# hyperplane-lab/RGBManip

Measured on AMD Instinct MI355X. Metric: adapose_poses_per_sec_batch256, higher is better.
Workload: dtype bf16

## Files before the change

### include/rgbm.h

```cpp
#ifndef RGBM_H_
#define RGBM_H_
#include <stddef.h>
#include <stdint.h>

#ifdef __cplusplus
extern "C" {
#endif

#define RGBM_VERSION 100
#define RGBM_F32 0
#define RGBM_BF16 1
#define RGBM_F16 2
#define RGBM_BF16X3 3

int rgbm_version(void);
const char* rgbm_last_error(void);

typedef struct rgbm_weight_desc {
  const char* name;
  const float* data;
  int ndim;
  const int64_t* shape;
} rgbm_weight_desc;

// ... 67 lines not shown
int rgbm_depth_fusion(const float* depth, const float* conf, const uint8_t* mask, const double* Kcrop, const double* E, int n, int V, int S,
                      double px_max, double rel_max, float conf_min, int n_min, float* fused, uint8_t* keep, uint8_t* nviews, uint16_t* agree,
                      void* stream);
int rgbm_cloud_pack_views(const float* fused, const uint8_t* keep, const double* Kcrop, const double* E, int n, int V, int S, int cap,
                          float* cloud, int32_t* index, int32_t* count, void* stream);
int rgbm_cloud_gather_views(const float* maps, const int32_t* index, int n, int V, int S2, int C, int cap, float* out, void* stream);

int rgbm_adapose_postprocess(int B, int P, int img_size, const float* nocs1, const float* depth1, const float* r1,
                             const int32_t* choose1, const double* Kcrop, const double* E1, double* bbox_world, double* ts,
                             int32_t* valid, void* stream);
int rgbm_adapose_postprocess_scratch_bytes(int B, size_t* bytes);
int rgbm_adapose_postprocess_ws(int B, int P, int img_size, const float* nocs1, const float* depth1, const float* r1,
                                const int32_t* choose1, const double* Kcrop, const double* E1, double* bbox_world, double* ts,
                                int32_t* valid, void* scratch, size_t scratch_bytes, void* stream);

int rgbm_adapose_postprocess_regressed(int B, int P, const float* nocs1, const float* r1, const float* t1, const float* s1,
                                       const double* E1, double* bbox_world, double* ts, int32_t* valid, void* stream);

int rgbm_adapose_postprocess_ransac(int B, int P, int img_size, uint32_t seed, const float* nocs1, const float* depth1,
                                    const int32_t* choose1, const double* Kcrop, const double* E1, double* bbox_world, double* srt,
                                    int32_t* valid, void* stream);
int rgbm_adapose_postprocess_pnp(int B, int P, uint32_t seed, const float* nocs1, const float* pts2d1, const float* nocs2,
                                 const float* pts2d2, const double* K, const double* E1, const double* E2, double* bbox_out,
                                 double* srt_out, int32_t* info_out, int32_t* valid_out, void* stream);

int rgbm_prepare_inputs(const float* rgb_dev, const uint8_t* mask_dev, const double* K_dev, int N, int H, int W, int S, int P,
                        uint32_t seed, float* img_out, int32_t* choose_out, float* pts2d_out, double* Kcrop_out,
                        int32_t* window_out, int32_t* valid_out, uint8_t* scratch, void* stream);

int rgbm_prepare_inputs_indexed(const float* rgb_dev, const uint8_t* mask_dev, const double* K_dev, const int32_t* frame_map_dev,
                                int N, int H, int W, int S, int P, uint32_t seed, float* img_out, int32_t* choose_out,
                                float* pts2d_out, double* Kcrop_out, int32_t* window_out, int32_t* valid_out, uint8_t* scratch,
                                void* stream);
int rgbm_prepare_inputs_ex(const float* rgb_dev, const uint8_t* mask_dev, const double* K_dev, const int32_t* frame_map_dev,
                           int frame0, int N, int H, int W, int S, int P, uint32_t seed, float* img_out, int32_t* choose_out,
                           float* pts2d_out, double* Kcrop_out, int32_t* window_out, int32_t* valid_out, uint8_t* scratch,
                           void* stream);
int rgbm_prepare_inputs_u8(const uint8_t* rgb_dev, const uint8_t* mask_dev, const double* K_dev, const int32_t* frame_map_dev,
                           int frame0, int N, int H, int W, int S, int P, uint32_t seed, float* img_out, int32_t* choose_out,
                           float* pts2d_out, double* Kcrop_out, int32_t* window_out, int32_t* valid_out, uint8_t* scratch,
                           void* stream);
int rgbm_prepare_inputs_opt(const void* rgb_dev, int pixel_type, int normalize, const uint8_t* mask_dev, const double* K_dev,
                            const int32_t* frame_map_dev, int frame0, int N, int H, int W, int S, int P, uint32_t seed, float* img_out,
                            int32_t* choose_out, float* pts2d_out, double* Kcrop_out, int32_t* window_out, int32_t* valid_out,
                            uint8_t* scratch, void* stream);
int rgbm_prepare_inputs_windows(const void* pix_dev, int pixel_type, int normalize, const uint8_t* mask_pix_dev, const int64_t* offset_dev,
                                const int32_t* window_dev, const int32_t* valid_in_dev, const double* K_dev, int frame0, int N, int H, int W,
                                int S, int P, uint32_t seed, float* img_out, int32_t* choose_out, float* pts2d_out, double* Kcrop_out,
                                int32_t* valid_out, uint8_t* scratch, void* stream);
int rgbm_quantize_frames(const float* src_dev, uint8_t* dst_dev, size_t n, void* stream);

int rgbm_projection(const double* Kcrop_dev, const double* E_dev, float* P_dev, int N, void* stream);
int rgbm_mask_extent(const uint8_t* mask_dev, int N, int H, int W, int32_t* ext_out, int32_t* count_out, void* stream);

int rgbm_lookat_quat(const double* dir_dev, int N, int batch_zero, double* quat_dev, void* stream);
int rgbm_control_action_to_pose(const float* action_dev, int lda, const double* pose_mid, const double* pose_min,
                                const double* pose_max, int N, double* pose_dev, void* stream);
typedef struct rgbm_control_reward_args {
  const float* action;
  const double* cam_pose;
  const double* target;
  const float* move_success;
  const double* bbox;
  const double* avail;
  const double* gt_bbox;
  const double* pred_bbox;
  const double* pose_cur;
  const double* pose_prev;
  const double* robot_pose;
  const double* success;
  double* reward;
  double* terms;
  double coef[14];
  double proper_pos[3];
  double precision2;
  int N, T, lda, pots, first;
  int pad_;
} rgbm_control_reward_args;
int rgbm_control_reward(const rgbm_control_reward_args* args, void* stream);
int rgbm_control_grasp_frame(const double* est_dev, int N, double* center_dev, double* direction_dev, void* stream);

typedef struct rgbm_synth_scene {
  const double* cam_pose;
  const double* robot_pose;
  const double* box;
  double fx, fy, cx, cy;
  int N, H, W, env0;
} rgbm_synth_scene;
int rgbm_synth_camera(const rgbm_synth_scene* scene, double* K_dev, double* E_dev, double* rays_dev, void* stream);
int rgbm_synth_render(const rgbm_synth_scene* scene, const double* rays_dev, float* color_dev, uint8_t* mask_dev, void* stream);
int rgbm_synth_render_u8(const rgbm_synth_scene* scene, const double* rays_dev, uint8_t* color_dev, uint8_t* mask_dev,
                         int32_t* extent_dev, int32_t* count_dev, void* stream);

int rgbm_gae(int T, int N, const float* rewards, const uint8_t* dones, const float* values, const float* last_values,
             float gamma, float lam, float* returns, float* adv, double* sums, void* stream);
int rgbm_adv_normalise(int64_t n_local, float* adv, const double* sums, double count_total, void* stream);

typedef struct rgbm_policy_layout {
  int dims[5];
  int log_std;
  int w[2][4];
  int b[2][4];
  int total;
} rgbm_policy_layout;
int rgbm_policy_forward(const float* params, const rgbm_policy_layout* L, int n, int mode, const float* obs, const float* noise,
                        float* actions, float* logp, float* value, float* mu, void* stream);
int rgbm_ppo_partial_floats(const rgbm_policy_layout* L, int n, size_t* count);
int rgbm_ppo_minibatch_fwd_bwd(const float* params, const rgbm_policy_layout* L, int n, const float* obs, const float* actions,
                               const float* old_logp, const float* adv, const float* returns, const float* old_values,
                               const float* old_mu, const float* old_log_std, float clip, float vcoef, float ecoef,
                               float* partial_scratch, float* grads_flat, void* stream);
int rgbm_ppo_clip_adam(float* params, const float* grads_flat, float* exp_avg, float* exp_avg_sq, void* opt_state,
                       const rgbm_policy_layout* L, float inv_world, float max_norm, float desired_kl, float lr_min,
                       float lr_max, int adaptive, void* stream);

#define RGBM_POLICY_MAX_HIDDEN 6
#define RGBM_POLICY_MAX_WIDTH 512
#define RGBM_POLICY_MAX_ACT 32
#define RGBM_ACT_ELU 0
#define RGBM_ACT_SELU 1
#define RGBM_ACT_RELU 2
#define RGBM_ACT_LRELU 3
#define RGBM_ACT_TANH 4
#define RGBM_ACT_SIGMOID 5
typedef struct rgbm_policy_desc {
  int obs_dim, state_dim, act_dim;
  int activation;
  int asymmetric;
  int n_hidden[2];
  int hidden[2][RGBM_POLICY_MAX_HIDDEN];
  int w[2][RGBM_POLICY_MAX_HIDDEN + 1];
  int b[2][RGBM_POLICY_MAX_HIDDEN + 1];
  int log_std;
  int total;
} rgbm_policy_desc;
int rgbm_policy_forward_ex(const float* params, const rgbm_policy_desc* D, int n, int mode, const float* obs, const float* states,
                           const float* noise, float* actions, float* logp, float* value, float* mu, void* stream);
int rgbm_ppo_scratch_floats_ex(const rgbm_policy_desc* D, int n, int clipped_value_loss, size_t* count);
int rgbm_ppo_minibatch_fwd_bwd_ex(const float* params, const rgbm_policy_desc* D, int n, const float* obs, const float* states,
                                  const float* actions, const float* old_logp, const float* adv, const float* returns,
                                  const float* old_values, const float* old_mu, const float* old_log_std, float clip, float vcoef,
                                  float ecoef, int clipped_value_loss, float* scratch, float* grads_flat, void* stream);
int rgbm_ppo_clip_adam_ex(float* params, const float* grads_flat, float* exp_avg, float* exp_avg_sq, void* opt_state, int total,
                          float inv_world, float max_norm, float desired_kl, float lr_min, float lr_max, int adaptive, void* stream);

int rgbm_conv_nd(int dtype, const void* in_dev, int N, int D, int H, int W, int Cin, int Cin_pad, const float* w_host,
                 int Cout, int Cout_pad, int KD, int KH, int KW, int stride_d, int stride_hw, int pad_d, int pad_hw,
                 int dil_hw, int transposed, const float* bias_host, const float* bn_scale_host, const float* bn_shift_host,
                 const void* res_dev, int res_mode, int act, float slope, void* out_dev, void* stream);
#define RGBM_CONV_PLAN_INTS 9
int rgbm_conv_plan(int dtype, int N, int D, int H, int W, int Cin, int Cin_pad, int Cout, int Cout_pad, int KD, int KH, int KW,
                   int stride_d, int stride_hw, int pad_d, int pad_hw, int dil_hw, int transposed, int has_bias, int res_mode, int act,
                   int cls, int n_cu, int32_t* plan);
int rgbm_bn_per_sample_scratch_bytes(int V, size_t* bytes);
int rgbm_bn_per_sample(int dtype, void* y_dev, const void* res_dev, const float* gamma_dev, const float* beta_dev, void* scratch_dev,
                       int V, int64_t nvox, int C, int relu, void* stream);
int rgbm_conv3d_tile(int layer, int dtype, const void* in_dev, int N, int D, int H, int W, const float* w_host,
                     const float* bn_scale_host, const float* bn_shift_host, const void* res_dev, void* out_dev, void* stream);
int rgbm_upsample_conv3x3(int dtype, const void* in_dev, int V, int h, int w, int Cin, const float* w_host, int Cout,
                          const float* bias_host, int act, float slope, void* z_scratch_dev, void* out_dev, void* stream);
int rgbm_upsample_conv3x3_final(int dtype, const void* in_dev, int V, int h, int w, const float* w3_host, const float* b3_host,
                                float slope, const float* wf_host, const float* bf_host, void* out_dev, int out_f32, void* stream);
int rgbm_stem(int dtype, const float* img1_dev, const float* img2_dev, const float* w_host, void* out_dev, int B, int S, void* stream);
int rgbm_maxpool3x3s2(int dtype, const void* in_dev, void* out_dev, int V, int H, int W, int C, void* stream);
int rgbm_resize_bilinear_ac(int dtype, const void* in_dev, void* out_dev, int V, int Hs, int Ws, int C, int Ho, int Wo,
                            void* stream);
int rgbm_adaptive_avgpool(int dtype, const void* in_dev, void* out_dev, int V, int H, int W, int C, int S, void* stream);
int rgbm_build_volume(int dtype, const void* feat_dev, const float* P_views_dev, const float* depths_dev, float* homog_scratch,
                      void* vol_dev, int V, int B, int D, int H, int W, void* stream);
int rgbm_conv0_sweep(const void* feat_dev, const float* P_views_dev, const float* depths_dev, float* homog_scratch,
                     const float* w_host, const float* bn_scale_host, const float* bn_shift_host, void* out_dev,
                     int V, int B, int D, int H, int W, void* stream);
int rgbm_conv0_sweep_dt(int dtype, const void* feat_dev, const float* P_views_dev, const float* depths_dev, float* homog_scratch,
                        const float* w_host, const float* bn_scale_host, const float* bn_shift_host, void* out_dev,
                        int V, int B, int D, int H, int W, void* stream);
int rgbm_conv0_sweep_f16feat(const void* feat_f16_dev, const float* P_views_dev, const float* depths_dev, float* homog_scratch,
                             const float* w_host, const float* bn_scale_host, const float* bn_shift_host, void* out_bf16_dev,
                             int V, int B, int D, int H, int W, void* stream);
int rgbm_adapose_forward_ex(rgbm_adapose_t* h, int B, const float* img1, const float* img2, const int32_t* choose1,
                            const int32_t* choose2, const float* P1, const float* P2, const float* depths, void* workspace,
                            size_t workspace_bytes, const rgbm_adapose_out* out, int stop_after, void* stream);
int rgbm_adapose_forward_graph(rgbm_adapose_t* h, int B, const float* img1, const float* img2, const int32_t* choose1,
                               const int32_t* choose2, const float* P1, const float* P2, const float* depths, void* workspace,
                               size_t workspace_bytes, const rgbm_adapose_out* out, void* stream, int32_t* n_nodes, int32_t* captured);
int rgbm_adapose_graph_clear(rgbm_adapose_t* h);
int rgbm_adapose_feature_bytes(rgbm_adapose_t* h, size_t* bytes);
int rgbm_adapose_features_workspace_bytes(rgbm_adapose_t* h, int V, size_t* bytes);
int rgbm_adapose_features(rgbm_adapose_t* h, int V, const float* img, const int32_t* slots_dev, void* pool, int pool_records,
                          void* workspace, size_t workspace_bytes, void* stream);
int rgbm_adapose_forward_cached(rgbm_adapose_t* h, int B, const void* pool, int pool_records, const int32_t* slot1_dev,
                                const int32_t* slot2_dev, const int32_t* choose1, const int32_t* choose2, const float* P1, const float* P2,
                                const float* depths, void* workspace, size_t workspace_bytes, const rgbm_adapose_out* out, void* stream);
int rgbm_adapose_fetch(rgbm_adapose_t* h, int B, void* workspace, const char* name, float* out_dev, size_t capacity,
                       size_t* n_elems, void* stream);
int rgbm_crop_fingerprint(const float* img, int V, int n_words, uint64_t* keys_out, void* stream);

#define RGBM_PROF_ROWS 42
int rgbm_debug_flags(int flags);
int rgbm_set_tuning(const char* key, long long value);
int rgbm_microbench_mfma_scratch_floats(int* n);
int rgbm_microbench_mfma(float* scratch, int iters, int random_operands, double* flops, void* stream);
int rgbm_microbench_copy(const void* src, void* dst, size_t bytes, void* stream);
int rgbm_prof_rows(void);
int rgbm_prof_start(void);
int rgbm_prof_stop(double* stats);
int rgbm_prof_select(int row);

#ifdef __cplusplus
}
#endif
#endif
```

### rgbmanip_amd/_lib.py

```python
from __future__ import annotations

import ctypes as C
import os

_HERE = os.path.dirname(os.path.abspath(__file__))
LIB_PATH = os.environ.get("RGBM_HIP_LIB") or os.path.join(_HERE, "librgbm_hip.so")

F32, BF16, F16, BF16X3 = 0, 1, 2, 3
ACT_NONE, ACT_RELU, ACT_PRELU, ACT_TANH = 0, 1, 2, 3
RES_NONE, RES_PRE_ACT, RES_POST_ACT = 0, 1, 2


PROF_ROWS = 42
PROF_KERNELS = [
    ("conv_igemm_glds_kernel<float, 16, 256>", "fp32"), ("conv_igemm_glds_kernel<float, 32, 256>", "fp32"),
    ("conv_igemm_glds_kernel<float, 64, 256>", "fp32"), ("conv_igemm_glds_kernel<float, 128, 128>", "fp32"),
    ("conv_igemm_glds_kernel<unsigned short, 16, 256>", "bf16"), ("conv_igemm_glds_kernel<unsigned short, 32, 256>", "bf16"),
    ("conv_igemm_glds_kernel<unsigned short, 64, 256>", "bf16"), ("conv_igemm_glds_kernel<unsigned short, 128, 128>", "bf16"),
    ("conv3d_tile_kernel<float, ...> (conv1..conv11)", "fp32"), ("conv3d_tile_kernel<unsigned short, ...> (conv1..conv11)", "bf16"),
    ("conv3d_tile_kernel<float, 32, 16, 4, 8, 8, 1, false, true> (conv0 + fused plane sweep)", "fp32"),
    ("conv3d_tile_kernel<unsigned short, 32, 16, 4, 8, 8, 1, false, true> (conv0 + fused plane sweep)", "bf16"),
    ("conv_igemm_ws_kernel<float, ...>", "fp32"), ("conv_igemm_ws_kernel<unsigned short, false, false> (128 channels x 256 pixels)", "bf16"),
    ("conv0_sweep_persistent_kernel<unsigned short> (conv0 + fused plane sweep of bf16 nets; sweep_f16 = 0 / fp16 nets: conv0_sweep_kernel)", "bf16"), ("conv_igemm_ws64_kernel", "bf16"),
    ("conv3d_tile_kernel<unsigned short, 32, 16, 6, 8, 8, 1, false, false> (conv0 on a materialised volume)", "bf16"),
    ("conv3d_tile_kernel<unsigned short, 8, 16, 2, 8, 8, 2, false, false> (conv1)", "bf16"),
    ("conv3d_tile_kernel<unsigned short, 16, 16, 4, 8, 8, 1, false, false> (conv2)", "bf16"),
    ("conv3d_tile_kernel<unsigned short, 16, 32, 2, 8, 8, 2, false, false> (conv3)", "bf16"),
    ("conv3d_tile_kernel<unsigned short, 32, 32, 2, 8, 8, 1, false, false> (conv4)", "bf16"),
    ("conv3d_tile_kernel<unsigned short, 32, 64, 1, 8, 8, 2, false, false> (conv5)", "bf16"),
    ("conv3d_tile_kernel<unsigned short, 64, 64, 1, 8, 8, 1, false, false> (conv6)", "bf16"),
    ("conv3d_tile_kernel<unsigned short, 64, 32, 1, 8, 8, 1, true, false> (conv7)", "bf16"),
    ("conv3d_tile_kernel<unsigned short, 32, 16, 2, 8, 8, 1, true, false> (conv9)", "bf16"),
    ("conv3d_tile_kernel<unsigned short, 16, 16, 4, 8, 8, 1, true, false> (conv11)", "bf16"),
] + [("conv_igemm_glds_kernel<bx3_t, ...> (all channel tiles)", "bf16x3"), ("conv3d_tile_kernel<bx3_t, ...> (conv1..conv11)", "bf16x3"),
     ("conv0 + fused plane sweep <bx3_t>", "bf16x3"), ("conv_igemm_ws_kernel<rgbm::bx3_t, false, false> (128 channels x 256 pixels)", "bf16x3"),
     ("pose_mlp1_kernel (pose_mlp1.0 + pose_mlp1.2 of a bf16 net in one launch)", "bf16"),
     ("conv_igemm_m32_kernel<unsigned short, 256, 256> (256 channels x 256 pixels, 32x32x16 MFMAs; gemm_kernel = 0: conv_igemm_ws_kernel<unsigned short, true, false>, 256 x 128)", "bf16"),
     ("pose_mlp2_kernel (pose_mlp2.0 + pose_mlp2.2 + the sum over points of a bf16 net in one launch)", "bf16"),
     ("conv_igemm_m32_kernel<rgbm::bx3_t, 256, 256> (256 channels x 256 pixels, 32x32x16 MFMAs; gemm_kernel = 0: conv_igemm_ws_kernel<rgbm::bx3_t, true, false>, 256 x 128)", "bf16x3"),
     ("conv_igemm_ws_kernel<rgbm::bx3_t, false, false, true> (64 channels x 256 pixels, four multiply waves)", "bf16x3"),
     ("conv_igemm_ws_kernel<unsigned short, false, false, true> (64 channels x 256 pixels, four multiply waves)", "bf16"),
     ("conv_igemm_ws_kernel<float, false, false, true> (64 channels x 256 pixels, four multiply waves)", "fp32"),
     ("upconv_combine_kernel<16-bit> (PSPUpsample tap combination)", "bf16"), ("upconv_combine_kernel<4-byte> (PSPUpsample tap combination)", "bf16x3"),
     ("upconv_final_kernel (up_3 + final in one kernel; either storage width)", "bf16"),
     ("conv_igemm_m32_kernel<unsigned short, 128, 64 / 128 / 256> (128-pixel tiles: tail and small-batch launches of the 256-channel GEMM)", "bf16"),
     ("conv_igemm_m32_kernel<rgbm::bx3_t, 128, 64 / 128 / 256> (128-pixel tiles: tail and small-batch launches of the 256-channel GEMM)", "bf16x3")]
assert len(PROF_KERNELS) == PROF_ROWS


class RgbmError(RuntimeError):
    pass


class WeightDesc(C.Structure):
    _fields_ = [("name", C.c_char_p), ("data", C.c_void_p), ("ndim", C.c_int), ("shape", C.POINTER(C.c_int64))]


class PolicyLayout(C.Structure):
    _fields_ = [("dims", C.c_int * 5), ("log_std", C.c_int), ("w", (C.c_int * 4) * 2), ("b", (C.c_int * 4) * 2), ("total", C.c_int)]


POLICY_MAX_HIDDEN, POLICY_MAX_WIDTH, POLICY_MAX_ACT = 6, 512, 32
POLICY_ACTIVATIONS = {"elu": 0, "selu": 1, "relu": 2, "crelu": 2, "lrelu": 3, "tanh": 4, "sigmoid": 5}


class PolicyDesc(C.Structure):
    _fields_ = [("obs_dim", C.c_int), ("state_dim", C.c_int), ("act_dim", C.c_int), ("activation", C.c_int), ("asymmetric", C.c_int),
                ("n_hidden", C.c_int * 2), ("hidden", (C.c_int * POLICY_MAX_HIDDEN) * 2),
                ("w", (C.c_int * (POLICY_MAX_HIDDEN + 1)) * 2), ("b", (C.c_int * (POLICY_MAX_HIDDEN + 1)) * 2),
                ("log_std", C.c_int), ("total", C.c_int)]


class AdaposeOut(C.Structure):
    _fields_ = [(n, C.c_void_p) for n in ("view1_nocs", "view2_nocs", "view1_depth", "view2_depth", "view1_r", "view2_r",
                                           "view1_t", "view2_t", "view1_s", "view2_s")]


class ControlRewardArgs(C.Structure):
    _fields_ = [(n, C.c_void_p) for n in ("action", "cam_pose", "target", "move_success", "bbox", "avail", "gt_bbox", "pred_bbox",
                                           "pose_cur", "pose_prev", "robot_pose", "success", "reward", "terms")] + [
        ("coef", C.c_double * 14), ("proper_pos", C.c_double * 3), ("precision2", C.c_double),
        ("N", C.c_int), ("T", C.c_int), ("lda", C.c_int), ("pots", C.c_int), ("first", C.c_int), ("pad_", C.c_int)]


class SynthScene(C.Structure):
    _fields_ = [("cam_pose", C.c_void_p), ("robot_pose", C.c_void_p), ("box", C.c_void_p),
                ("fx", C.c_double), ("fy", C.c_double), ("cx", C.c_double), ("cy", C.c_double),
                ("N", C.c_int), ("H", C.c_int), ("W", C.c_int), ("env0", C.c_int)]


_vp, _i, _f, _d, _sz, _i64 = C.c_void_p, C.c_int, C.c_float, C.c_double, C.c_size_t, C.c_int64

SIGNATURES = {
    "rgbm_version": (_i, []),
    "rgbm_last_error": (C.c_char_p, []),
    "rgbm_adapose_create": (_i, [C.POINTER(_vp), _i, C.POINTER(WeightDesc), _i, _i, _i]),
    "rgbm_adapose_create_baseline": (_i, [C.POINTER(_vp), _i, C.POINTER(WeightDesc), _i, _i, _i]),
    "rgbm_view_fusion": (_i, [_vp, _vp, _vp, _i, _i, _vp, _vp, _vp, _sz, _vp]),
    "rgbm_view_fusion_scratch_bytes": (_i, [_i, _i, C.POINTER(_sz)]),
    "rgbm_depth_head": (_i, [_vp, _vp, _i64, _vp, _vp]),
    "rgbm_adapose_destroy": (_i, [_vp]),
    "rgbm_adapose_set_chunk": (_i, [_vp, _i]),
    "rgbm_adapose_set_option": (_i, [_vp, C.c_char_p, _i]),
    "rgbm_adapose_workspace_bytes": (_i, [_vp, _i, C.POINTER(_sz)]),
    "rgbm_adapose_set_dropout": (_i, [_vp, _f, C.c_uint64]),
    "rgbm_adapose_dropout_masks": (_i, [_vp, _i, _vp]),
    "rgbm_adapose_set_dropout_masks": (_i, [_vp, _i, _vp]),
    "rgbm_adapose_forward": (_i, [_vp, _i, _vp, _vp, _vp, _vp, _vp, _vp, _vp, _vp, _sz, C.POINTER(AdaposeOut), _vp]),
    "rgbm_adapose_forward_ex": (_i, [_vp, _i, _vp, _vp, _vp, _vp, _vp, _vp, _vp, _vp, _sz, C.POINTER(AdaposeOut), _i, _vp]),
    "rgbm_adapose_forward_graph": (_i, [_vp, _i, _vp, _vp, _vp, _vp, _vp, _vp, _vp, _vp, _sz, C.POINTER(AdaposeOut), _vp, C.POINTER(C.c_int32),
                                        C.POINTER(C.c_int32)]),
    "rgbm_adapose_samples_workspace_bytes": (_i, [_vp, _i, _i, C.POINTER(_sz)]),
    "rgbm_adapose_forward_samples": (_i, [_vp, _i, _i, _vp, _vp, _vp, _vp, _vp, _vp, _vp, _vp, _sz, C.POINTER(AdaposeOut), _vp]),
    "rgbm_sample_box_stats": (_i, [_vp, _vp, _i, _i, _vp, _vp, _vp, _vp, _vp, _vp, _vp, _vp, _vp]),
    "rgbm_sample_point_stats": (_i, [_vp, _i, _i, _i64, _vp, _vp, _vp]),
    "rgbm_box_agreement": (_i, [_vp, _vp, _vp, _vp, _i] + [_vp] * 14),
    "rgbm_box_iou_matrix": (_i, [_vp, _vp, _vp, _vp, _i, _i, _i, _vp, _vp]),
    "rgbm_adapose_dense_workspace_bytes": (_i, [_vp, _i, C.POINTER(_sz)]),
    "rgbm_adapose_forward_dense": (_i, [_vp, _i, _vp, _vp, _vp, _vp, _vp, _vp, _vp, _vp, _sz, C.POINTER(AdaposeOut), _vp, _vp, _vp]),
    "rgbm_adapose_forward_maps": (_i, [_vp, _i, _vp, _vp, _vp, _vp, _vp, _vp, _vp, _vp, _sz, C.POINTER(AdaposeOut), _vp, _vp, _vp, _vp]),
    "rgbm_nocs_map": (_i, [_vp, _vp, _i, _i, _vp, _vp]),
    "rgbm_cloud_gather": (_i, [_vp, _vp, _vp, _i, _i, _i, _i, _vp, _vp]),
    "rgbm_cloud_similarity_scratch_bytes": (_i, [_i, _i, C.POINTER(_sz)]),
    "rgbm_cloud_similarity": (_i, [_vp, _vp, _vp, _i, _i, C.c_uint32, _vp, _vp, _vp, _vp, _vp, _sz, _vp]),
    "rgbm_depth_to_points": (_i, [_vp, _vp, _vp, _i, _i, _vp, _vp]),
    "rgbm_depth_consistency": (_i, [_vp, _vp, _vp, _vp, _vp, _vp, _vp, _vp, _i, _i, _d, _d, _f, _vp, _vp, _vp, _vp, _vp]),
    "rgbm_cloud_pack": (_i, [_vp, _vp, _vp, _vp, _vp, _vp, _vp, _vp, _i, _i, _i, _vp, _vp, _vp, _vp]),
    "rgbm_depth_fusion": (_i, [_vp, _vp, _vp, _vp, _vp, _i, _i, _i, _d, _d, _f, _i, _vp, _vp, _vp, _vp, _vp]),
    "rgbm_cloud_pack_views": (_i, [_vp, _vp, _vp, _vp, _i, _i, _i, _i, _vp, _vp, _vp, _vp]),
    "rgbm_cloud_gather_views": (_i, [_vp, _vp, _i, _i, _i, _i, _i, _vp, _vp]),
    "rgbm_adapose_graph_clear": (_i, [_vp]),
    "rgbm_adapose_feature_bytes": (_i, [_vp, C.POINTER(_sz)]),
    "rgbm_adapose_features_workspace_bytes": (_i, [_vp, _i, C.POINTER(_sz)]),
    "rgbm_adapose_features": (_i, [_vp, _i, _vp, _vp, _vp, _i, _vp, _sz, _vp]),
    "rgbm_adapose_forward_cached": (_i, [_vp, _i, _vp, _i, _vp, _vp, _vp, _vp, _vp, _vp, _vp, _vp, _sz, C.POINTER(AdaposeOut), _vp]),
    "rgbm_crop_fingerprint": (_i, [_vp, _i, _i, _vp, _vp]),
    "rgbm_adapose_fetch": (_i, [_vp, _i, _vp, C.c_char_p, _vp, _sz, C.POINTER(_sz), _vp]),
    "rgbm_adapose_postprocess": (_i, [_i, _i, _i, _vp, _vp, _vp, _vp, _vp, _vp, _vp, _vp, _vp, _vp]),
    "rgbm_adapose_postprocess_scratch_bytes": (_i, [_i, C.POINTER(_sz)]),
    "rgbm_adapose_postprocess_ws": (_i, [_i, _i, _i, _vp, _vp, _vp, _vp, _vp, _vp, _vp, _vp, _vp, _vp, _sz, _vp]),
    "rgbm_adapose_postprocess_regressed": (_i, [_i, _i, _vp, _vp, _vp, _vp, _vp, _vp, _vp, _vp, _vp]),
    "rgbm_adapose_postprocess_ransac": (_i, [_i, _i, _i, C.c_uint32, _vp, _vp, _vp, _vp, _vp, _vp, _vp, _vp, _vp]),
    "rgbm_adapose_postprocess_pnp": (_i, [_i, _i, C.c_uint32, _vp, _vp, _vp, _vp, _vp, _vp, _vp, _vp, _vp, _vp, _vp, _vp]),
    "rgbm_gae": (_i, [_i, _i, _vp, _vp, _vp, _vp, _f, _f, _vp, _vp, _vp, _vp]),
    "rgbm_adv_normalise": (_i, [_i64, _vp, _vp, _d, _vp]),
    "rgbm_policy_forward": (_i, [_vp, _vp, _i, _i, _vp, _vp, _vp, _vp, _vp, _vp, _vp]),
    "rgbm_ppo_partial_floats": (_i, [_vp, _i, C.POINTER(_sz)]),
    "rgbm_ppo_minibatch_fwd_bwd": (_i, [_vp, _vp, _i, _vp, _vp, _vp, _vp, _vp, _vp, _vp, _vp, _f, _f, _f, _vp, _vp, _vp]),
    "rgbm_ppo_clip_adam": (_i, [_vp, _vp, _vp, _vp, _vp, _vp, _f, _f, _f, _f, _f, _i, _vp]),
    "rgbm_policy_forward_ex": (_i, [_vp, _vp, _i, _i, _vp, _vp, _vp, _vp, _vp, _vp, _vp, _vp]),
    "rgbm_ppo_scratch_floats_ex": (_i, [_vp, _i, _i, C.POINTER(_sz)]),
    "rgbm_ppo_minibatch_fwd_bwd_ex": (_i, [_vp, _vp, _i, _vp, _vp, _vp, _vp, _vp, _vp, _vp, _vp, _vp, _f, _f, _f, _i, _vp, _vp, _vp]),
    "rgbm_ppo_clip_adam_ex": (_i, [_vp, _vp, _vp, _vp, _vp, _i, _f, _f, _f, _f, _f, _i, _vp]),
    "rgbm_conv_nd": (_i, [_i, _vp, _i, _i, _i, _i, _i, _i, _vp, _i, _i, _i, _i, _i, _i, _i, _i, _i, _i, _i, _vp, _vp, _vp,
                          _vp, _i, _i, _f, _vp, _vp]),
    "rgbm_conv_plan": (_i, [_i] * 23 + [C.POINTER(C.c_int32)]),
    "rgbm_bn_per_sample_scratch_bytes": (_i, [_i, C.POINTER(_sz)]),
    "rgbm_bn_per_sample": (_i, [_i, _vp, _vp, _vp, _vp, _vp, _i, _i64, _i, _i, _vp]),
    "rgbm_conv3d_tile": (_i, [_i, _i, _vp, _i, _i, _i, _i, _vp, _vp, _vp, _vp, _vp, _vp]),
    "rgbm_upsample_conv3x3": (_i, [_i, _vp, _i, _i, _i, _i, _vp, _i, _vp, _i, _f, _vp, _vp, _vp]),
    "rgbm_upsample_conv3x3_final": (_i, [_i, _vp, _i, _i, _i, _vp, _vp, _f, _vp, _vp, _vp, _i, _vp]),
    "rgbm_stem": (_i, [_i, _vp, _vp, _vp, _vp, _i, _i, _vp]),
    "rgbm_maxpool3x3s2": (_i, [_i, _vp, _vp, _i, _i, _i, _i, _vp]),
    "rgbm_resize_bilinear_ac": (_i, [_i, _vp, _vp, _i, _i, _i, _i, _i, _i, _vp]),
    "rgbm_adaptive_avgpool": (_i, [_i, _vp, _vp, _i, _i, _i, _i, _i, _vp]),
    "rgbm_build_volume": (_i, [_i, _vp, _vp, _vp, _vp, _vp, _i, _i, _i, _i, _i, _vp]),
    "rgbm_conv0_sweep": (_i, [_vp, _vp, _vp, _vp, _vp, _vp, _vp, _vp, _i, _i, _i, _i, _i, _vp]),
    "rgbm_conv0_sweep_dt": (_i, [_i, _vp, _vp, _vp, _vp, _vp, _vp, _vp, _vp, _i, _i, _i, _i, _i, _vp]),
    "rgbm_conv0_sweep_f16feat": (_i, [_vp, _vp, _vp, _vp, _vp, _vp, _vp, _vp, _i, _i, _i, _i, _i, _vp]),
    "rgbm_prepare_inputs": (_i, [_vp, _vp, _vp, _i, _i, _i, _i, _i, C.c_uint32, _vp, _vp, _vp, _vp, _vp, _vp, _vp, _vp]),
    "rgbm_prepare_inputs_indexed": (_i, [_vp, _vp, _vp, _vp, _i, _i, _i, _i, _i, C.c_uint32, _vp, _vp, _vp, _vp, _vp, _vp, _vp, _vp]),
    "rgbm_prepare_inputs_ex": (_i, [_vp, _vp, _vp, _vp, _i, _i, _i, _i, _i, _i, C.c_uint32, _vp, _vp, _vp, _vp, _vp, _vp, _vp, _vp]),
    "rgbm_prepare_inputs_u8": (_i, [_vp, _vp, _vp, _vp, _i, _i, _i, _i, _i, _i, C.c_uint32, _vp, _vp, _vp, _vp, _vp, _vp, _vp, _vp]),
    "rgbm_prepare_inputs_opt": (_i, [_vp, _i, _i, _vp, _vp, _vp, _i, _i, _i, _i, _i, _i, C.c_uint32, _vp, _vp, _vp, _vp, _vp, _vp, _vp, _vp]),
    "rgbm_prepare_inputs_windows": (_i, [_vp, _i, _i, _vp, _vp, _vp, _vp, _vp, _i, _i, _i, _i, _i, _i, C.c_uint32, _vp, _vp, _vp, _vp, _vp, _vp, _vp]),
    "rgbm_quantize_frames": (_i, [_vp, _vp, C.c_size_t, _vp]),
    "rgbm_projection": (_i, [_vp, _vp, _vp, _i, _vp]),
    "rgbm_mask_extent": (_i, [_vp, _i, _i, _i, _vp, _vp, _vp]),
    "rgbm_lookat_quat": (_i, [_vp, _i, _i, _vp, _vp]),
    "rgbm_control_action_to_pose": (_i, [_vp, _i, C.POINTER(C.c_double), C.POINTER(C.c_double), C.POINTER(C.c_double), _i, _vp, _vp]),
    "rgbm_control_reward": (_i, [C.POINTER(ControlRewardArgs), _vp]),
    "rgbm_control_grasp_frame": (_i, [_vp, _i, _vp, _vp, _vp]),
    "rgbm_synth_camera": (_i, [C.POINTER(SynthScene), _vp, _vp, _vp, _vp]),
    "rgbm_synth_render": (_i, [C.POINTER(SynthScene), _vp, _vp, _vp, _vp]),
    "rgbm_synth_render_u8": (_i, [C.POINTER(SynthScene), _vp, _vp, _vp, _vp, _vp, _vp]),
    "rgbm_debug_flags": (_i, [_i]),
    "rgbm_set_tuning": (_i, [C.c_char_p, _i64]),
    "rgbm_prof_rows": (_i, []),
    "rgbm_microbench_mfma_scratch_floats": (_i, [C.POINTER(C.c_int)]),
    "rgbm_microbench_mfma": (_i, [_vp, _i, _i, C.POINTER(C.c_double), _vp]),
    "rgbm_microbench_copy": (_i, [_vp, _vp, C.c_size_t, _vp]),
    "rgbm_prof_start": (_i, []),
    "rgbm_prof_select": (_i, [_i]),
    "rgbm_prof_stop": (_i, [C.POINTER(C.c_double)]),
}

_lib = None


def load():
    global _lib
    if _lib is not None:
        return _lib
    if not os.path.exists(LIB_PATH):
        raise RgbmError(f"{LIB_PATH} not found: build it with rgbmanip_amd/csrc/build.sh "
                        f"(or `python -c 'import __graft_entry__ as g; g.build()'`). There is no CPU fallback.")
    lib = C.CDLL(LIB_PATH)
    for name, (res, args) in SIGNATURES.items():
        fn = getattr(lib, name)
        fn.restype = res
        fn.argtypes = args
    if lib.rgbm_prof_rows() != PROF_ROWS:
        raise RgbmError(f"{LIB_PATH}: rgbm_prof_rows() = {lib.rgbm_prof_rows()}, this binding expects {PROF_ROWS} (stale build?)")
    _lib = lib
    return lib


def check(rc: int, what: str = ""):
    if rc != 0:
        msg = load().rgbm_last_error()
        raise RgbmError(f"{what} failed (code {rc}): {msg.decode() if msg else ''}")


def stream_ptr(stream=None):
    import torch
    s = stream if stream is not None else torch.cuda.current_stream()
    return C.c_void_p(s.cuda_stream)


def ptr(t):
    return C.c_void_p(t.data_ptr()) if t is not None else C.c_void_p(0)
```

### rgbmanip_amd/csrc/capi.cpp

```cpp
#include "../../include/rgbm.h"

#include <string.h>

#include <algorithm>
#include <initializer_list>
#include <memory>
#include <string>
#include <utility>
#include <vector>

#include "adapose.h"
#include "box_overlap.h"
#include "control.h"
#include "cost3d.h"
#include "conv_plan.h"
#include "prof.h"
#include "sample_stats.h"
#include "view_fusion.h"

using namespace rgbm;

struct ForwardGraph {
  int B = 0;
  hipStream_t stream = nullptr;
// ... 439 lines not shown
    if (call.dropout == AdaPose::Dropout::Draw) warm.dropout = AdaPose::Dropout::DrawNoAdvance;
    if (int rw = forward(warm)) return rw;
    ForwardGraph g;
    g.B = B; g.stream = s; memcpy(g.in, in, sizeof(in)); g.ws = workspace; g.ws_bytes = workspace_bytes; g.out = *out;
    g.opt_version = h->opt_version; g.tuning_version = g_tuning_version;
    RGBM_CHECK_HIP(hipStreamBeginCapture(s, hipStreamCaptureModeThreadLocal));
    const int rc = forward(call);
    const hipError_t ee = hipStreamEndCapture(s, &g.graph);
    if (rc) { if (g.graph) (void)hipGraphDestroy(g.graph); return rc; }
    if (ee != hipSuccess || !g.graph) { set_error(std::string("hipStreamEndCapture: ") + hipGetErrorString(ee)); return -2; }
    if (hipGraphGetNodes(g.graph, nullptr, &g.nodes) != hipSuccess) g.nodes = 0;
    const hipError_t ei = hipGraphInstantiate(&g.exec, g.graph, nullptr, nullptr, 0);
    if (ei != hipSuccess) { (void)hipGraphDestroy(g.graph); set_error(std::string("hipGraphInstantiate: ") + hipGetErrorString(ei)); return -2; }
    if (h->graphs.size() >= kMaxGraphs) {
      size_t lru = 0;
      for (size_t i = 1; i < h->graphs.size(); ++i) if (h->graphs[i].last_use < h->graphs[lru].last_use) lru = i;
      drop_graph(h->graphs[lru]);
      h->graphs.erase(h->graphs.begin() + lru);
    }
    h->graphs.push_back(g);
    hit = &h->graphs.back();
    if (captured) *captured = 1;
  }
  hit->last_use = ++h->tick;
  if (n_nodes) *n_nodes = (int32_t)hit->nodes;
  RGBM_CHECK_HIP(hipGraphLaunch(hit->exec, s));
  return finish_call(h, B, call, 0);
}

int rgbm_adapose_fetch(rgbm_adapose_t* h, int B, void* workspace, const char* name, float* out_dev, size_t capacity,
                       size_t* n_elems, void* stream) {
  RGBM_REQUIRE(h && workspace && name && out_dev && n_elems, "fetch arguments");
  const AdaPose& n = h->net;
  Arena A(workspace, 0);
  AdaPose::Buffers bf;
  n.plan(B, A, bf);
  const size_t V = 2 * (size_t)B, S = n.img, P = n.n_pts, D = n.n_depth;
  const size_t Vc = n.chunk_views((int)V);
  const std::string nm = name;
  const void* src = nullptr; size_t cnt = 0; int dt = n.dtype;
  if (nm == "imgpad") { src = bf.imgpad; cnt = V * S * S * n.img_cpad; }
  else if (nm == "conv1") { src = bf.c1; cnt = V * (S / 2) * (S / 2) * 64; }
  else if (nm == "layer4") { src = bf.lb[n.layer4_index()]; cnt = V * (S / 8) * (S / 8) * 512; }
  else if (nm == "cat") { src = bf.cat; cnt = V * (S / 8) * (S / 8) * 1024; }
  else if (nm == "u1") { src = bf.u1; cnt = V * (S / 4) * (S / 4) * 256; }
  else if (nm == "u2") { src = bf.u2; cnt = V * (S / 2) * (S / 2) * 64; }
  else if (nm == "u3") { src = bf.u3; cnt = V * S * S * 64; }
  else if (nm == "feat") { src = bf.feat; cnt = V * S * S * 32; if (n.feat_f32_only()) { src = bf.featf; dt = F32; } else if (n.feat_f16()) dt = F16; }
  else if (nm == "vol") { src = bf.vol; cnt = Vc * D * S * S * 32; }
  else if (nm == "homog") { src = bf.homog; cnt = V * 12; dt = F32; }
  else if (nm == "prob") { src = bf.prob; cnt = V * P * D; dt = F32; }
  else if (nm == "pf96") { src = bf.PF96; cnt = V * P * 96; dt = n.pose_dtype() == BF16X3 ? BF16X3 : F32; }
  else if (nm == "pf2") { src = bf.pf2; cnt = V * 256; dt = F32; }
  else if (nm == "r6") { src = bf.r6; cnt = V * 6; dt = F32; }
  else if (nm == "fused1" && bf.fused) { src = bf.fused; cnt = (size_t)B * P * 32; dt = F32; }
  else if (nm == "fused2" && bf.fused) { src = bf.fused + (size_t)B * P * 32; cnt = (size_t)B * P * 32; dt = F32; }
  static const struct { const char* name; int row; } taps3d[] = {{"c0", 0}, {"c2", 2}, {"c4", 4}, {"c6", 6}, {"u7", 7}, {"u9", 8}, {"u11", 9}};
  int row3d = -1;
  for (const auto& t : taps3d)
    if (nm == t.name) { row3d = t.row; src = bf.c3[row3d]; cnt = cost3d_out_elems(row3d, (int)Vc, (int)D, (int)S); }
  if (is_baseline(h))
    RGBM_REQUIRE(nm == "feat" || nm == "fused1" || nm == "fused2" || nm == "pf96" || nm == "pf2" || nm == "r6" || nm == "layer4" || nm == "cat" ||
                 nm == "u1" || nm == "u2", "tap '" + nm + "' does not exist in the baseline network");
  RGBM_REQUIRE(src != nullptr, "unknown intermediate name: " + nm);
  const bool tap3d = row3d >= 0 && row3d < 9;
  RGBM_REQUIRE(!(tap3d && n.sparse_active()), "tap '" + nm + "' needs a dense cost regularisation: set option sparse_dec = 0 before the forward "
               "(the default computes it only inside the chosen pixels' dependency cones)");
  *n_elems = cnt;
  RGBM_REQUIRE(cnt <= capacity, "fetch capacity too small");
  return launch_to_f32(dt, src, out_dev, (long long)cnt, (hipStream_t)stream);
}

int rgbm_adapose_postprocess(int B, int P, int img_size, const float* nocs1, const float* depth1, const float* r1,
                             const int32_t* choose1, const double* Kcrop, const double* E1, double* bbox_world, double* ts,
                             int32_t* valid, void* stream) {
  RGBM_REQUIRE(B > 0 && nocs1 && depth1 && r1 && choose1 && Kcrop && E1 && bbox_world && ts && valid, "postprocess arguments");
  return launch_postprocess(nocs1, depth1, r1, choose1, Kcrop, E1, bbox_world, ts, valid, B, P, img_size, (hipStream_t)stream);
}

int rgbm_adapose_postprocess_scratch_bytes(int B, size_t* bytes) {
  RGBM_REQUIRE(B > 0 && bytes, "postprocess_scratch_bytes arguments");
  *bytes = postprocess_slices(B) > 1 ? postprocess_scratch_bytes(B) : 0;
  return 0;
}

int rgbm_adapose_postprocess_ws(int B, int P, int img_size, const float* nocs1, const float* depth1, const float* r1,
                                const int32_t* choose1, const double* Kcrop, const double* E1, double* bbox_world, double* ts,
                                int32_t* valid, void* scratch, size_t scratch_bytes, void* stream) {
  RGBM_REQUIRE(B > 0 && nocs1 && depth1 && r1 && choose1 && Kcrop && E1 && bbox_world && ts && valid, "postprocess arguments");
  return launch_postprocess(nocs1, depth1, r1, choose1, Kcrop, E1, bbox_world, ts, valid, B, P, img_size, (hipStream_t)stream,
                            scratch, scratch_bytes);
}

int rgbm_adapose_postprocess_ransac(int B, int P, int img_size, uint32_t seed, const float* nocs1, const float* depth1,
                                    const int32_t* choose1, const double* Kcrop, const double* E1, double* bbox_world, double* srt,
                                    int32_t* valid, void* stream) {
  return launch_umeyama_ransac(nocs1, depth1, choose1, Kcrop, E1, bbox_world, srt, valid, B, P, img_size, seed, (hipStream_t)stream);
}

int rgbm_gae(int T, int N, const float* rewards, const uint8_t* dones, const float* values, const float* last_values,
             float gamma, float lam, float* returns, float* adv, double* sums, void* stream) {
  RGBM_REQUIRE(rewards && dones && values && last_values && returns && adv && sums, "gae arguments");
  return launch_gae(T, N, rewards, dones, values, last_values, gamma, lam, returns, adv, sums, (hipStream_t)stream);
}

int rgbm_adv_normalise(int64_t n_local, float* adv, const double* sums, double count_total, void* stream) {
  RGBM_REQUIRE(adv && sums && n_local > 0 && count_total > 1.0, "adv_normalise arguments");
  return launch_adv_normalise(n_local, adv, sums, count_total, (hipStream_t)stream);
}

static ConvGeom conv_nd_geom(int Cin, int Cout, int KD, int KH, int KW, int stride_d, int stride_hw, int pad_d, int pad_hw, int dil_hw,
                             int transposed, int act, float slope) {
  ConvGeom g;
  g.Cin = Cin; g.Cout = Cout; g.KD = KD; g.KH = KH; g.KW = KW;
  g.sd = stride_d; g.sh = g.sw = stride_hw; g.pd = pad_d; g.ph = g.pw = pad_hw;
  g.dild = 1; g.dilh = g.dilw = dil_hw; g.transposed = transposed != 0; g.act = act; g.slope = slope;
  return g;
}

int rgbm_conv_nd(int dtype, const void* in_dev, int N, int D, int H, int W, int Cin, int Cin_pad, const float* w_host,
                 int Cout, int Cout_pad, int KD, int KH, int KW, int stride_d, int stride_hw, int pad_d, int pad_hw,
                 int dil_hw, int transposed, const float* bias_host, const float* bn_scale_host, const float* bn_shift_host,
                 const void* res_dev, int res_mode, int act, float slope, void* out_dev, void* stream) {
  RGBM_REQUIRE(in_dev && w_host && out_dev, "conv arguments");
  const ConvGeom g = conv_nd_geom(Cin, Cout, KD, KH, KW, stride_d, stride_hw, pad_d, pad_hw, dil_hw, transposed, act, slope);
  ConvLayer L;
  if (int rc = L.init(dtype, g, w_host, bias_host, bn_scale_host, bn_shift_host, Cin_pad, Cout_pad)) return rc;
  return finish_one_shot(L.run(in_dev, out_dev, N, D, H, W, Cout_pad, res_dev, res_mode, nullptr, 0, (hipStream_t)stream), stream);
}

int rgbm_conv_plan(int dtype, int N, int D, int H, int W, int Cin, int Cin_pad, int Cout, int Cout_pad, int KD, int KH, int KW,
                   int stride_d, int stride_hw, int pad_d, int pad_hw, int dil_hw, int transposed, int has_bias, int res_mode, int act,
                   int cls, int n_cu, int32_t* plan) {
  RGBM_REQUIRE(plan && n_cu >= 0 && dtype >= F32 && dtype <= BF16X3 && N > 0 && D > 0 && H > 0 && W > 0, "conv_plan arguments");
  const ConvGeom g = conv_nd_geom(Cin, Cout, KD, KH, KW, stride_d, stride_hw, pad_d, pad_hw, dil_hw, transposed, act, 0.f);
  PackedConv pc;
  if (int rc = conv_pack_geom(g, dtype, Cin_pad, Cout_pad, cls, &pc)) return rc;
  ConvDesc d;
  conv_desc_geom(d, g, pc, Cin_pad, Cout_pad, N, D, H, W, Cout_pad, cls);
  alignas(16) static const float buffer[4] = {};
  d.in = d.wgt = buffer; d.out = const_cast<float*>(buffer);
  d.bias = has_bias ? buffer : nullptr;
  d.res = res_mode != RES_NONE ? buffer : nullptr;
  d.res_mode = res_mode;
  ConvTuning t;
  ConvPlan p;
  if (int rc = conv_tuning(n_cu, &t)) return rc;
  if (int rc = plan_conv(d, dtype, t, &p)) return rc;
  const int32_t v[RGBM_CONV_PLAN_INTS] = {p.kernel, p.bch, p.bpix, p.ksplit, (int32_t)p.main_rows, p.tail_bch, p.identity_residual, (int32_t)d.M, d.KT};
  memcpy(plan, v, sizeof(v));
  return 0;
}

int rgbm_upsample_conv3x3(int dtype, const void* in_dev, int V, int h, int w, int Cin, const float* w_host, int Cout,
                          const float* bias_host, int act, float slope, void* z_scratch_dev, void* out_dev, void* stream) {
  RGBM_REQUIRE(in_dev && w_host && z_scratch_dev && out_dev, "upsample_conv3x3 arguments");
  UpConvLayer L;
  if (int rc = L.init(dtype, Cin, Cout, w_host, bias_host, act, slope)) return rc;
  return finish_one_shot(L.run(in_dev, z_scratch_dev, out_dev, V, h, w, Cout, (hipStream_t)stream), stream);
}

int rgbm_upsample_conv3x3_final(int dtype, const void* in_dev, int V, int h, int w, const float* w3_host, const float* b3_host,
                                float slope, const float* wf_host, const float* bf_host, void* out_dev, int out_f32, void* stream) {
  RGBM_REQUIRE(in_dev && w3_host && b3_host && wf_host && bf_host && out_dev, "upsample_conv3x3_final arguments");
  UpConvFinal L;
  if (int rc = L.init(dtype, w3_host, b3_host, slope, wf_host, bf_host)) return rc;
  return finish_one_shot(L.run(in_dev, out_dev, out_f32, V, h, w, (hipStream_t)stream), stream);
}

int rgbm_stem(int dtype, const float* img1_dev, const float* img2_dev, const float* w_host, void* out_dev, int B, int S, void* stream) {
  RGBM_REQUIRE(img1_dev && img2_dev && w_host && out_dev && B > 0, "stem arguments");
  std::vector<float> pk;
  stem_pack(w_host, pk);
  DevBuf wd;
  if (int rc = upload_packed(pk, dtype, wd)) return rc;
  return finish_one_shot(launch_stem(dtype, img1_dev, img2_dev, wd.get(), out_dev, B, 2 * B, S, (hipStream_t)stream), stream);
}

int rgbm_bn_per_sample_scratch_bytes(int V, size_t* bytes) {
  RGBM_REQUIRE(V > 0 && bytes, "bn_per_sample_scratch_bytes arguments");
  *bytes = bn_scratch_bytes(V);
  return 0;
}
int rgbm_bn_per_sample(int dtype, void* y_dev, const void* res_dev, const float* gamma_dev, const float* beta_dev, void* scratch_dev,
                       int V, int64_t nvox, int C, int relu, void* stream) {
  RGBM_REQUIRE(y_dev && gamma_dev && beta_dev && scratch_dev, "bn_per_sample arguments");
  return launch_bn_per_sample(dtype, y_dev, res_dev, gamma_dev, beta_dev, scratch_dev, V, (long long)nvox, C, relu, (hipStream_t)stream);
}
int rgbm_maxpool3x3s2(int dtype, const void* in_dev, void* out_dev, int V, int H, int W, int C, void* stream) {
  return launch_maxpool3x3s2(dtype, in_dev, out_dev, V, H, W, C, (hipStream_t)stream);
}
int rgbm_resize_bilinear_ac(int dtype, const void* in_dev, void* out_dev, int V, int Hs, int Ws, int C, int Ho, int Wo,
                            void* stream) {
  return launch_resize_bilinear_ac(dtype, in_dev, out_dev, V, Hs, Ws, C, Ho, Wo, C, 0, (hipStream_t)stream);
}
int rgbm_adaptive_avgpool(int dtype, const void* in_dev, void* out_dev, int V, int H, int W, int C, int S, void* stream) {
  return launch_adaptive_avgpool(dtype, in_dev, out_dev, V, H, W, C, S, (hipStream_t)stream);
}
int rgbm_build_volume(int dtype, const void* feat_dev, const float* P_views_dev, const float* depths_dev, float* homog_scratch,
                      void* vol_dev, int V, int B, int D, int H, int W, void* stream) {
  if (int rc = launch_homography(P_views_dev, homog_scratch, V, B, (hipStream_t)stream)) return rc;
  return launch_build_volume(dtype, feat_dev, homog_scratch, depths_dev, vol_dev, 0, V, V, B, D, H, W, (hipStream_t)stream);
}

}

#include "prof.h"
extern "C" {
int rgbm_prof_rows(void) { return rgbm::kProfVariants; }
int rgbm_microbench_mfma_scratch_floats(int* n) {
  RGBM_REQUIRE(n, "microbench_mfma_scratch_floats arguments");
  return rgbm::microbench_mfma_scratch_floats(n);
}
int rgbm_microbench_mfma(float* scratch, int iters, int random_operands, double* flops, void* stream) {
  return rgbm::launch_microbench_mfma(scratch, iters, random_operands, flops, (hipStream_t)stream);
}
int rgbm_microbench_copy(const void* src, void* dst, size_t bytes, void* stream) {
  return rgbm::launch_microbench_copy(src, dst, bytes, (hipStream_t)stream);
}
int rgbm_prof_start(void) { return rgbm::prof_start(); }
int rgbm_prof_select(int row) {
  RGBM_REQUIRE(row >= -1 && row < rgbm::kProfVariants, "prof_select: row out of range");
  return rgbm::prof_select(row);
}
int rgbm_prof_stop(double* stats) {
  RGBM_REQUIRE(stats != nullptr, "prof_stop arguments");
  return rgbm::prof_stop(stats, rgbm::kProfVariants);
}
}

extern "C" int rgbm_conv3d_tile(int layer, int dtype, const void* in_dev, int N, int D, int H, int W, const float* w_host,
                                const float* bn_scale_host, const float* bn_shift_host, const void* res_dev, void* out_dev,
                                void* stream) {
  RGBM_REQUIRE(layer >= 0 && layer < kCost3dLayers && in_dev && w_host && bn_scale_host && bn_shift_host && out_dev, "conv3d_tile arguments");
  const Cost3dLayer& L = kCost3d[layer];
  const int coutp = cost3d_coutp(layer);
  std::vector<float> packed;
  conv3d_tile_pack(w_host, bn_scale_host, L.cin, L.cout, coutp, L.transposed, dtype, packed);
  DevBuf wdev, bdev;
  if (upload_packed(packed, dtype, wdev)) return -2;
  std::vector<float> bpad(coutp, 0.f);
  for (int o = 0; o < L.cout; ++o) bpad[o] = bn_shift_host[o];
  if (upload_f32(bpad.data(), bpad.size(), bdev)) return -2;
  Conv3dTileDesc d;
  memset(&d, 0, sizeof(d));
  d.in = in_dev; d.wgt = wdev.get(); d.out = out_dev; d.bias = bdev.get<float>(); d.res = res_dev;
  d.N = N; d.Di = D; d.Hi = H; d.Wi = W;
  if (L.transposed) { d.Do = 2 * D; d.Ho = 2 * H; d.Wo = 2 * W; d.Dq = D; d.Hq = H; d.Wq = W; }
  else {
    const int s = L.stride;
    d.Do = (D + 2 - 3) / s + 1; d.Ho = (H + 2 - 3) / s + 1; d.Wo = (W + 2 - 3) / s + 1;
    d.Dq = d.Do; d.Hq = d.Ho; d.Wq = d.Wo;
  }
  d.Cout = L.cout; d.relu = 1; d.prof_variant = -1;
  return finish_one_shot(launch_conv3d_tile(layer, dtype, d, (hipStream_t)stream), stream);
}

static int conv0_sweep_entry(int dtype, int feat_f16, const void* feat_dev, const float* P_views_dev, const float* depths_dev,
                             float* homog_scratch, const float* w_host, const float* bn_scale_host, const float* bn_shift_host,
                             void* out_dev, int V, int B, int D, int H, int W, void* stream) {
  RGBM_REQUIRE(feat_dev && P_views_dev && depths_dev && homog_scratch && w_host && bn_scale_host && bn_shift_host && out_dev,
               "conv0_sweep arguments");
  RGBM_REQUIRE(dtype == BF16 || dtype == F16 || dtype == BF16X3, "conv0_sweep: 16-bit storage types or bf16x3 (fp32 features in, split-pair c0 out)");
  if (int rc = launch_homography(P_views_dev, homog_scratch, V, B, (hipStream_t)stream)) return rc;
  std::vector<float> packed;
  conv0_sweep_pack(w_host, bn_scale_host, packed);
  DevBuf wdev, bdev;
  if (dtype == BF16X3) { if (conv0_sweep_x3_upload(packed, wdev.out())) return -2; }
  else if (upload_packed(packed, feat_f16 ? (int)F16 : dtype, wdev)) return -2;
  std::vector<float> bpad(cost3d_coutp(0), 0.f);
  for (int o = 0; o < kCost3d[0].cout; ++o) bpad[o] = bn_shift_host[o];
  if (upload_f32(bpad.data(), bpad.size(), bdev)) return -2;
  Conv3dTileDesc d;
  memset(&d, 0, sizeof(d));
  d.wgt = wdev.get(); d.out = out_dev; d.bias = bdev.get<float>();
  d.N = V; d.Di = D; d.Hi = H; d.Wi = W; d.Do = D; d.Ho = H; d.Wo = W; d.Dq = D; d.Hq = H; d.Wq = W;
  d.Cout = kCost3d[0].cout; d.relu = 1; d.prof_variant = -1;
  d.feat = feat_dev; d.homog = homog_scratch; d.depths = depths_dev; d.v0 = 0; d.V = V; d.B = B;
  d.feat_f16 = feat_f16;
  return finish_one_shot(dtype == BF16X3 ? launch_conv0_sweep_x3(d, (hipStream_t)stream) : launch_conv0_sweep(d, dtype, (hipStream_t)stream), stream);
}

extern "C" int rgbm_conv0_sweep_dt(int dtype, const void* feat_dev, const float* P_views_dev, const float* depths_dev,
                                   float* homog_scratch, const float* w_host, const float* bn_scale_host, const float* bn_shift_host,
                                   void* out_dev, int V, int B, int D, int H, int W, void* stream) {
  return conv0_sweep_entry(dtype, 0, feat_dev, P_views_dev, depths_dev, homog_scratch, w_host, bn_scale_host, bn_shift_host, out_dev, V, B, D,
                           H, W, stream);
}

extern "C" int rgbm_conv0_sweep_f16feat(const void* feat_f16_dev, const float* P_views_dev, const float* depths_dev,
                                        float* homog_scratch, const float* w_host, const float* bn_scale_host,
                                        const float* bn_shift_host, void* out_bf16_dev, int V, int B, int D, int H, int W, void* stream) {
  return conv0_sweep_entry(BF16, 1, feat_f16_dev, P_views_dev, depths_dev, homog_scratch, w_host, bn_scale_host, bn_shift_host, out_bf16_dev,
                           V, B, D, H, W, stream);
}

extern "C" int rgbm_conv0_sweep(const void* feat_dev, const float* P_views_dev, const float* depths_dev, float* homog_scratch,
                                const float* w_host, const float* bn_scale_host, const float* bn_shift_host, void* out_dev,
                                int V, int B, int D, int H, int W, void* stream) {
  return rgbm_conv0_sweep_dt(BF16, feat_dev, P_views_dev, depths_dev, homog_scratch, w_host, bn_scale_host, bn_shift_host, out_dev,
                             V, B, D, H, W, stream);
}

extern "C" int rgbm_prepare_inputs(const float* rgb_dev, const uint8_t* mask_dev, const double* K_dev, int N, int H, int W, int S,
                                   int P, uint32_t seed, float* img_out, int32_t* choose_out, float* pts2d_out, double* Kcrop_out,
                                   int32_t* window_out, int32_t* valid_out, uint8_t* scratch, void* stream) {
// ... 185 lines not shown
```

### rgbmanip_amd/csrc/common.h

```cpp
#pragma once
#include <hip/hip_runtime.h>
#include <stdint.h>
#include <stdio.h>
#include <string>

namespace rgbm {

enum DType { F32 = 0, BF16 = 1, F16 = 2, BF16X3 = 3 };
enum Act { ACT_NONE = 0, ACT_RELU = 1, ACT_PRELU = 2, ACT_TANH = 3 };
enum ResMode { RES_NONE = 0, RES_PRE_ACT = 1, RES_POST_ACT = 2 };

typedef __attribute__((ext_vector_type(8))) __bf16 bf16x8;
typedef _Float16 f16_t;
typedef __attribute__((ext_vector_type(8))) _Float16 f16x8;
typedef __attribute__((ext_vector_type(4))) _Float16 f16x4;
typedef __attribute__((ext_vector_type(8))) float f32x8;
typedef __attribute__((ext_vector_type(4))) float f32x4;

void set_error(const std::string& s);
int fail(const char* what, const char* file, int line);

#define RGBM_CHECK_HIP(expr)                                                             \
  do {                                                                                   \
    hipError_t _e = (expr);                                                              \
// ... 62 lines not shown
  o.w = pack2_bf16(c - __uint_as_float(o.y << 16), d - __uint_as_float(o.y & 0xffff0000u));
  return o;
}
__device__ __forceinline__ void bx3_join4(const uint4& c, float* v) {
  v[0] = __uint_as_float(c.x << 16) + __uint_as_float(c.z << 16);
  v[1] = __uint_as_float(c.x & 0xffff0000u) + __uint_as_float(c.z & 0xffff0000u);
  v[2] = __uint_as_float(c.y << 16) + __uint_as_float(c.w << 16);
  v[3] = __uint_as_float(c.y & 0xffff0000u) + __uint_as_float(c.w & 0xffff0000u);
}
template <> struct Elem<bx3_t> {
  static constexpr int kPerChunk = 4;
  __device__ static __forceinline__ float ld(const bx3_t* p) {
    const unsigned long long a = (unsigned long long)p;
    const unsigned short* ch = reinterpret_cast<const unsigned short*>(a & ~15ull);
    const int e = (int)((a >> 2) & 3);
    return bf16_to_f32(ch[e]) + bf16_to_f32(ch[4 + e]);
  }
  __device__ static __forceinline__ void st(bx3_t* p, float v) {
    const unsigned long long a = (unsigned long long)p;
    unsigned short* ch = reinterpret_cast<unsigned short*>(a & ~15ull);
    const int e = (int)((a >> 2) & 3);
    const unsigned short h = f32_to_bf16(v);
    ch[e] = h;
    ch[4 + e] = f32_to_bf16(v - bf16_to_f32(h));
  }
};

__device__ __forceinline__ float sat_f16(float v) { return v != v ? v : fminf(fmaxf(v, -65504.f), 65504.f); }

__device__ __forceinline__ void load4(const float* p, float v[4]) {
  float4 t = *reinterpret_cast<const float4*>(p);
  v[0] = t.x; v[1] = t.y; v[2] = t.z; v[3] = t.w;
}
__device__ __forceinline__ void load4(const unsigned short* p, float v[4]) {
  uint2 t = *reinterpret_cast<const uint2*>(p);
  v[0] = __uint_as_float(t.x << 16); v[1] = __uint_as_float(t.x & 0xffff0000u);
  v[2] = __uint_as_float(t.y << 16); v[3] = __uint_as_float(t.y & 0xffff0000u);
}
__device__ __forceinline__ void load4(const f16_t* p, float v[4]) {
  const f16x4 t = *reinterpret_cast<const f16x4*>(p);
  v[0] = (float)t[0]; v[1] = (float)t[1]; v[2] = (float)t[2]; v[3] = (float)t[3];
}
__device__ __forceinline__ void store4(f16_t* p, const float v[4]) {
  f16x4 t;
  t[0] = (f16_t)sat_f16(v[0]); t[1] = (f16_t)sat_f16(v[1]); t[2] = (f16_t)sat_f16(v[2]); t[3] = (f16_t)sat_f16(v[3]);
  *reinterpret_cast<f16x4*>(p) = t;
}
__device__ __forceinline__ void store4(float* p, const float v[4]) {
  *reinterpret_cast<float4*>(p) = make_float4(v[0], v[1], v[2], v[3]);
}
__device__ __forceinline__ void store4(unsigned short* p, const float v[4]) {
  uint2 t;
  t.x = pack2_bf16(v[0], v[1]);
  t.y = pack2_bf16(v[2], v[3]);
  *reinterpret_cast<uint2*>(p) = t;
}
__device__ __forceinline__ void load4(const bx3_t* p, float v[4]) { bx3_join4(*reinterpret_cast<const uint4*>(p), v); }
__device__ __forceinline__ void store4(bx3_t* p, const float v[4]) { *reinterpret_cast<uint4*>(p) = bx3_split4(v[0], v[1], v[2], v[3]); }
__device__ __forceinline__ void unpack_chunk(const uint4& c, float* v, bx3_t ) { bx3_join4(c, v); }
__device__ __forceinline__ uint4 pack_chunk(const float* v, bx3_t ) { return bx3_split4(v[0], v[1], v[2], v[3]); }
__device__ __forceinline__ void unpack_chunk(const uint4& c, float* v, float ) {
  v[0] = __uint_as_float(c.x); v[1] = __uint_as_float(c.y); v[2] = __uint_as_float(c.z); v[3] = __uint_as_float(c.w);
}
__device__ __forceinline__ void unpack_chunk(const uint4& c, float* v, unsigned short ) {
  v[0] = __uint_as_float(c.x << 16); v[1] = __uint_as_float(c.x & 0xffff0000u);
  v[2] = __uint_as_float(c.y << 16); v[3] = __uint_as_float(c.y & 0xffff0000u);
  v[4] = __uint_as_float(c.z << 16); v[5] = __uint_as_float(c.z & 0xffff0000u);
  v[6] = __uint_as_float(c.w << 16); v[7] = __uint_as_float(c.w & 0xffff0000u);
}
__device__ __forceinline__ void unpack_chunk(const uint4& c, float* v, f16_t ) {
  const f16x8 h = __builtin_bit_cast(f16x8, c);
#pragma unroll
  for (int e = 0; e < 8; ++e) v[e] = (float)h[e];
}
__device__ __forceinline__ uint4 pack_chunk(const float* v, f16_t ) {
  f16x8 h;
#pragma unroll
  for (int e = 0; e < 8; ++e) h[e] = (f16_t)sat_f16(v[e]);
  return __builtin_bit_cast(uint4, h);
}
__device__ __forceinline__ uint4 pack_chunk(const float* v, float ) {
  return make_uint4(__float_as_uint(v[0]), __float_as_uint(v[1]), __float_as_uint(v[2]), __float_as_uint(v[3]));
}
__device__ __forceinline__ uint4 pack_chunk(const float* v, unsigned short ) {
  uint4 c;
  c.x = pack2_bf16(v[0], v[1]);
  c.y = pack2_bf16(v[2], v[3]);
  c.z = pack2_bf16(v[4], v[5]);
  c.w = pack2_bf16(v[6], v[7]);
  return c;
}

typedef __attribute__((ext_vector_type(4))) short rgbm_s16x4;
__device__ __forceinline__ f32x4 mma_bx3_k16(const uint4& a, const uint4& b, f32x4 c) {
  const rgbm_s16x4 ah = __builtin_bit_cast(rgbm_s16x4, make_uint2(a.x, a.y)), al = __builtin_bit_cast(rgbm_s16x4, make_uint2(a.z, a.w));
  const rgbm_s16x4 bh = __builtin_bit_cast(rgbm_s16x4, make_uint2(b.x, b.y)), bl = __builtin_bit_cast(rgbm_s16x4, make_uint2(b.z, b.w));
  c = __builtin_amdgcn_mfma_f32_16x16x16bf16_1k(al, bh, c, 0, 0, 0);
  c = __builtin_amdgcn_mfma_f32_16x16x16bf16_1k(ah, bl, c, 0, 0, 0);
  c = __builtin_amdgcn_mfma_f32_16x16x16bf16_1k(ah, bh, c, 0, 0, 0);
  return c;
}
__device__ __forceinline__ void bx3_pair(const uint4& c0, const uint4& c1, uint4& hi, uint4& lo) {
  hi = make_uint4(c0.x, c0.y, c1.x, c1.y);
  lo = make_uint4(c0.z, c0.w, c1.z, c1.w);
}

__host__ __device__ inline unsigned mix32(unsigned seed, unsigned frame, unsigned idx) {
  unsigned h = seed ^ (frame * 0x9E3779B9u) ^ (idx * 0x85EBCA6Bu);
  h ^= h >> 16; h *= 0x85EBCA6Bu; h ^= h >> 13; h *= 0xC2B2AE35u; h ^= h >> 16;
  return h;
}

template <int THREADS, class Op> __device__ inline double block_reduce(double v, double* red, Op op) {
  const int t = threadIdx.x;
  red[t] = v;
  __syncthreads();
  for (int s = THREADS / 2; s > 0; s >>= 1) {
    if (t < s) red[t] = op(red[t], red[t + s]);
    __syncthreads();
  }
  const double r = red[0];
  __syncthreads();
  return r;
}
template <int THREADS> __device__ inline double block_sum(double v, double* red) {
  return block_reduce<THREADS>(v, red, [](double a, double b) { return a + b; });
}
template <int THREADS> __device__ inline double block_max(double v, double* red) {
  return block_reduce<THREADS>(v, red, [](double a, double b) { return fmax(a, b); });
}

struct ConvDesc {
  const void* in; const void* wgt; void* out; const float* bias; const void* res;
  int N, Di, Hi, Wi, Cin, lcin;
  int Dq, Hq, Wq;
  int sd, sh, sw, pd, ph, pw;
  int KD, KH, KW, dild, dilh, dilw;
  int ntaps, KT, Kpad;
  int Cout, ldo;
  int Do, Ho, Wo;
  int osd, osh, osw, opd, oph, opw;
  int act; float slope; int res_mode; int bias_stride;
  long long M;
  int n_pix_tiles, n_ch_tiles;
  int n_tiles; unsigned fd_m[3]; int fd_s[3];
  int korder;
  int buf_ok;
  const void* ident;
  long long m0;
  const void* w2; const float* bias2; void* out2; int ldo2, cout2, kpad2, act2; float slope2;
  double algo_flops, algo_bytes;
  int out_f32;
  int ksplit; float* kscratch; unsigned* kcount;
};

int launch_conv(const ConvDesc& d, int dtype, hipStream_t s);
bool conv_ws64_eligible(const ConvDesc& d, int dtype);
int conv_ch_tile(int Cout);
int conv_bk(int dtype);

}
```

### rgbmanip_amd/csrc/conv_igemm_glds.hip

```cpp
#include <map>
#include <mutex>
#include <type_traits>
#include <vector>
#include "common.h"
#include "conv_plan.h"
#include "kernels.h"
#include "prof.h"

#ifndef WS_BUF
#define WS_BUF 1
#endif

namespace rgbm {

int g_gemm_kernel = 2;
__device__ uint4 g_zero_page[4];

typedef __attribute__((address_space(3))) void* lds_ptr_t;
typedef const __attribute__((address_space(1))) void* gbl_ptr_t;

__device__ __forceinline__ void glds16(const void* gsrc, unsigned lds_off) {
  asm volatile("s_mov_b32 m0, %1\n\ts_nop 0\n\tglobal_load_lds_dwordx4 %0, off" :: "v"(gsrc), "s"(lds_off) : "memory");
}
__device__ __forceinline__ void blds16(unsigned voff, const __amdgpu_buffer_rsrc_t& rsrc, unsigned soff, unsigned lds_off) {
  asm volatile("s_mov_b32 m0, %3\n\ts_nop 0\n\tbuffer_load_dwordx4 %0, %1, %2 offen lds" :: "v"(voff), "s"(rsrc), "s"(soff), "s"(lds_off) : "memory");
}
__device__ __forceinline__ unsigned lds_addr(const void* p) {
  return (unsigned)(unsigned long long)(__attribute__((address_space(3))) const void*)p;
}

#define RGBM_BARRIER() do { asm volatile("" ::: "memory"); __builtin_amdgcn_s_barrier(); asm volatile("" ::: "memory"); } while (0)

template <typename T> struct MmaG;
template <> struct MmaG<unsigned short> {
  __device__ static __forceinline__ void run(const uint4& a, const uint4& b, f32x4& c) {
    c = __builtin_amdgcn_mfma_f32_16x16x32_bf16(__builtin_bit_cast(bf16x8, a), __builtin_bit_cast(bf16x8, b), c, 0, 0, 0);
  }
  __device__ static __forceinline__ f32x4 run2(const uint4& a, const uint4& b, const f32x4& c) {
    return __builtin_amdgcn_mfma_f32_16x16x32_bf16(__builtin_bit_cast(bf16x8, a), __builtin_bit_cast(bf16x8, b), c, 0, 0, 0);
  }
};
template <> struct MmaG<f16_t> {
  __device__ static __forceinline__ void run(const uint4& a, const uint4& b, f32x4& c) {
    c = __builtin_amdgcn_mfma_f32_16x16x32_f16(__builtin_bit_cast(f16x8, a), __builtin_bit_cast(f16x8, b), c, 0, 0, 0);
  }
  __device__ static __forceinline__ f32x4 run2(const uint4& a, const uint4& b, const f32x4& c) {
    return __builtin_amdgcn_mfma_f32_16x16x32_f16(__builtin_bit_cast(f16x8, a), __builtin_bit_cast(f16x8, b), c, 0, 0, 0);
  }
};
template <> struct MmaG<float> {
  __device__ static __forceinline__ void run(const uint4& a, const uint4& b, f32x4& c) {
    c = __builtin_amdgcn_mfma_f32_16x16x4f32(__uint_as_float(a.x), __uint_as_float(b.x), c, 0, 0, 0);
    c = __builtin_amdgcn_mfma_f32_16x16x4f32(__uint_as_float(a.y), __uint_as_float(b.y), c, 0, 0, 0);
    c = __builtin_amdgcn_mfma_f32_16x16x4f32(__uint_as_float(a.z), __uint_as_float(b.z), c, 0, 0, 0);
    c = __builtin_amdgcn_mfma_f32_16x16x4f32(__uint_as_float(a.w), __uint_as_float(b.w), c, 0, 0, 0);
  }
};

template <> struct MmaG<bx3_t> {
  __device__ static __forceinline__ void run(const uint4& a, const uint4& b, f32x4& c) { c = mma_bx3_k16(a, b, c); }
};
template <typename T> constexpr int prof_row_generic(int bch) {
  return std::is_same<T, bx3_t>::value ? 26 : (sizeof(T) == 2 ? 4 : 0) + (bch == 16 ? 0 : bch == 32 ? 1 : bch == 64 ? 2 : 3);
}
template <typename T> constexpr int prof_row_ws() { return std::is_same<T, bx3_t>::value ? 29 : sizeof(T) == 2 ? 13 : 12; }

template <int FM, int FN>
__device__ __forceinline__ void mma_bx3_tile(const uint4 (&a0)[FM], const uint4 (&a1)[FM], const uint4 (&b0)[FN], const uint4 (&b1)[FN],
                                             f32x4 (&acc)[FM][FN]) {
  uint4 ah[FM], al[FM], bh[FN], bl[FN];
#pragma unroll
  for (int a = 0; a < FM; ++a) bx3_pair(a0[a], a1[a], ah[a], al[a]);
#pragma unroll
  for (int b = 0; b < FN; ++b) bx3_pair(b0[b], b1[b], bh[b], bl[b]);
#pragma unroll
  for (int a = 0; a < FM; ++a)
#pragma unroll
    for (int b = 0; b < FN; ++b) MmaG<unsigned short>::run(al[a], bh[b], acc[a][b]);
#pragma unroll
  for (int a = 0; a < FM; ++a)
#pragma unroll
    for (int b = 0; b < FN; ++b) MmaG<unsigned short>::run(ah[a], bl[b], acc[a][b]);
#pragma unroll
  for (int a = 0; a < FM; ++a)
#pragma unroll
    for (int b = 0; b < FN; ++b) MmaG<unsigned short>::run(ah[a], bh[b], acc[a][b]);
}

template <int OFF>
__device__ __forceinline__ void lds_rd8(uint2& dst, unsigned addr) {
  asm volatile("ds_read_b64 %0, %1 offset:%2" : "=v"(dst) : "v"(addr), "n"(OFF) : "memory");
}

template <int FM, int FN>
__device__ __forceinline__ void mma_bx3_ops(const uint4 (&ah)[FM], const uint4 (&al)[FM], const uint4 (&bh)[FN], const uint4 (&bl)[FN],
                                            f32x4 (&acc)[FM][FN]) {
#pragma unroll
  for (int a = 0; a < FM; ++a)
#pragma unroll
    for (int b = 0; b < FN; ++b) MmaG<unsigned short>::run(al[a], bh[b], acc[a][b]);
#pragma unroll
  for (int a = 0; a < FM; ++a)
#pragma unroll
    for (int b = 0; b < FN; ++b) MmaG<unsigned short>::run(ah[a], bl[b], acc[a][b]);
#pragma unroll
  for (int a = 0; a < FM; ++a)
#pragma unroll
    for (int b = 0; b < FN; ++b) MmaG<unsigned short>::run(ah[a], bh[b], acc[a][b]);
}

template <int N> struct IC { static constexpr int value = N; };

__device__ __forceinline__ float apply_act_g(float v, int act, float slope) {
  if (act == ACT_RELU) return v < 0.f ? 0.f : v;
  if (act == ACT_PRELU) return v < 0.f ? v * slope : v;
  if (act == ACT_TANH) return tanhf(v);
  return v;
}

template <typename T, int BCH, int BPIX, bool UNI>
__global__ __launch_bounds__(256, 2) void conv_igemm_glds_kernel(const ConvDesc d) {
  constexpr int E = 16 / sizeof(T);
  constexpr int BK = 8 * E;
  constexpr int XR = BPIX / 32;
  constexpr int WL = BCH >= 32 ? BCH / 32 : 1;
  constexpr int WCH = BCH < 64 ? BCH : 64;
  constexpr int FM = WCH / 16;
  constexpr int FN = 4;
  constexpr int STAGE = (BCH + BPIX) * 8;
  __shared__ uint4 lds[2 * STAGE];

  const int tid = threadIdx.x;
  const int lane = tid & 63;
  const int wave = __builtin_amdgcn_readfirstlane(tid >> 6);

  const int nblk = gridDim.x;
  const int bq = nblk >> 3, br = nblk & 7;
  const int xcd = blockIdx.x & 7, bidx = blockIdx.x >> 3;
  const int lid = (xcd < br ? xcd * (bq + 1) : br * (bq + 1) + (xcd - br) * bq) + bidx;
  const int pix_tile = lid / d.n_ch_tiles;
  const int ch_tile = lid - pix_tile * d.n_ch_tiles;

  const T* __restrict__ in = reinterpret_cast<const T*>(d.in);
  const T* __restrict__ wgt = reinterpret_cast<const T*>(d.wgt);

  const int j = tid & 7;
  const int r0 = tid >> 3;
  const int js = j ^ ((r0 >> 1) & 7);
  int xn[XR], xd0[XR], xh0[XR], xw0[XR];
  const char* rowp[XR];
  unsigned rmask[XR];
#pragma unroll
// ... 1600 lines not shown
```

### rgbmanip_amd/csrc/conv_igemm_m32.inc

```
#ifndef M32_SHIFT
#define M32_SHIFT 1
#endif
#ifndef M32_RACE_PROBE
#define M32_RACE_PROBE 0
#endif
typedef __attribute__((ext_vector_type(16))) float f32x16;

template <typename T> struct Mma32;
template <> struct Mma32<unsigned short> {
  __device__ static __forceinline__ void run(const uint4& a, const uint4& b, f32x16& c) {
    c = __builtin_amdgcn_mfma_f32_32x32x16_bf16(__builtin_bit_cast(bf16x8, a), __builtin_bit_cast(bf16x8, b), c, 0, 0, 0);
  }
};
template <> struct Mma32<f16_t> {
  __device__ static __forceinline__ void run(const uint4& a, const uint4& b, f32x16& c) {
    c = __builtin_amdgcn_mfma_f32_32x32x16_f16(__builtin_bit_cast(f16x8, a), __builtin_bit_cast(f16x8, b), c, 0, 0, 0);
  }
};

template <> struct Mma32<bx3_t> {
  __device__ static __forceinline__ void run(const uint4&, const uint4&, f32x16&) {}
};

__device__ __forceinline__ int m32_row_channel(int i) { return ((i >> 2) & 1) * 16 + (i & 3) + 4 * (i >> 3); }

template <typename T, int BPIX, int BCH = 256>
__global__ __launch_bounds__(BPIX == 256 ? 768 : 512) void conv_igemm_m32_kernel(const ConvDesc d) {
  constexpr bool BIG = BPIX == 256;
  constexpr bool STAGED = BIG && BCH == 256;
  constexpr bool X3 = std::is_same<T, bx3_t>::value;
  constexpr int NMW = BIG ? 8 : 4;
  constexpr int NTH = (NMW + 4) * 64;
  constexpr int NST = BIG ? 2 : 3;
  static_assert(BCH == 256 || BCH == 128 || BCH == 64, "channel tiles of 256 / 128 / 64");
  constexpr int E = 16 / sizeof(T);
  constexpr int BK = 8 * E;
  constexpr int XR = BPIX / 32;
  constexpr int WL = BCH / 32;
  constexpr int NP = XR + WL;
  constexpr int FA = BCH / 64, FB = 2;
  constexpr int WCHW = FA * 32;
  constexpr int STAGE = (BCH + BPIX) * 8;
  extern __shared__ __attribute__((aligned(16))) uint4 lds3[];

  const int tid = threadIdx.x;
  const int lane = tid & 63;
  const int wave = __builtin_amdgcn_readfirstlane(tid >> 6);
  constexpr bool KSPLIT = !BIG && BCH <= 128;
  int KT = d.KT, kt0 = 0, part = 0, nsp = 1, vtile = -1;
  if constexpr (KSPLIT) {
    if (d.ksplit > 1) {
      nsp = d.ksplit;
      part = (int)blockIdx.x % nsp;
      vtile = (int)blockIdx.x / nsp;
      kt0 = (int)((long long)part * d.KT / nsp);
      KT = (int)((long long)(part + 1) * d.KT / nsp) - kt0;
    }
  }
  const bool res_in_acc = d.ident != nullptr && d.res_mode == RES_PRE_ACT;
  const int KR = (res_in_acc && part == nsp - 1) ? BCH / BK : 0;
  const int KTT = KT + KR;
  const int n_my = vtile >= 0 ? 1 : ((int)d.n_tiles - (int)blockIdx.x + (int)gridDim.x - 1) / (int)gridDim.x;
  const int total = n_my * KTT;
  auto tile_of = [&](int k, int& pix_tile, int& ch_tile) {
    const int v = vtile >= 0 ? vtile : (int)blockIdx.x + k * (int)gridDim.x;
    const int nblk = d.n_tiles, bq = nblk >> 3, br = nblk & 7, xcd = v & 7, bidx = v >> 3;
    const int lid = (xcd < br ? xcd * (bq + 1) : br * (bq + 1) + (xcd - br) * bq) + bidx;
    pix_tile = lid / d.n_ch_tiles;
    ch_tile = lid - pix_tile * d.n_ch_tiles;
  };

  float* lbias = reinterpret_cast<float*>(lds3 + NST * STAGE);
  const bool bias_lds = d.bias != nullptr && d.bias_stride == 0 && d.Cout <= 2560;
  if (bias_lds)
    for (int i = tid; i < d.Cout; i += NTH) lbias[i] = d.bias[i];
  __syncthreads();

  if (wave >= NMW) {
    const int pw = wave - NMW;
    const int tp = tid - NMW * 64;
    const int j = tp & 7;
    const int r0 = tp >> 3;
    const int js = j ^ ((r0 >> 1) & 7);
    unsigned rmask[XR], xoff[XR], woff[WL], roff[XR];
    int tkd = 0, tkh = 0, tkw = 0, tc = 0;
    unsigned wko = 0;
    const unsigned lds0 = __builtin_amdgcn_readfirstlane(lds_addr(lds3 + pw * 64));
    const long long xbias = ((long long)(d.pd * d.Hi + d.ph) * d.Wi + d.pw) * d.Cin * (long long)sizeof(T);
    const __amdgpu_buffer_rsrc_t rsrc_x = __builtin_amdgcn_make_buffer_rsrc(
        const_cast<char*>(reinterpret_cast<const char*>(d.in)) - xbias, 0,
        (int)(unsigned)((long long)d.N * d.Di * d.Hi * d.Wi * d.Cin * (long long)sizeof(T) + xbias), 0x00020000);
    const __amdgpu_buffer_rsrc_t rsrc_w = __builtin_amdgcn_make_buffer_rsrc(
        const_cast<char*>(reinterpret_cast<const char*>(d.wgt)), 0, (int)(unsigned)((long long)d.n_ch_tiles * BCH * d.Kpad * (long long)sizeof(T)), 0x00020000);

    const __amdgpu_buffer_rsrc_t rsrc_r = __builtin_amdgcn_make_buffer_rsrc(
        const_cast<char*>(reinterpret_cast<const char*>(d.res)), 0, (int)(unsigned)(d.M * d.ldo * (long long)sizeof(T)), 0x00020000);
    const __amdgpu_buffer_rsrc_t rsrc_i = __builtin_amdgcn_make_buffer_rsrc(
        const_cast<char*>(reinterpret_cast<const char*>(d.ident)), 0, (int)(unsigned)(256 * 256 * sizeof(T)), 0x00020000);
    long long mybase = 0;
    unsigned mymask = 0;
    int my_ch_tile = 0, my_pix_tile = 0;
    auto prepare_tile = [&](int k) {
      int pix_tile, ch_tile;
      tile_of(k, pix_tile, ch_tile);
      my_ch_tile = ch_tile;
      my_pix_tile = pix_tile;
      mybase = 0;
      mymask = 0;
      if (j < XR) {
        const long long m = d.m0 + (long long)pix_tile * BPIX + r0 + 32 * j;
        int xn = 0, xd0 = -(1 << 20), xh0 = 0, xw0 = 0;
        if (m < d.M) {
          unsigned n, qd, qh, qw;
          decode_row(d, (unsigned)m, n, qd, qh, qw);
          xn = (int)n * d.Di;
          xd0 = (int)qd * d.sd - d.pd;
          xh0 = (int)qh * d.sh - d.ph;
          xw0 = (int)qw * d.sw - d.pw;
        }
        for (int kk = 0; kk < d.KD; ++kk) mymask |= (unsigned)((unsigned)(xd0 + kk * d.dild) < (unsigned)d.Di) << kk;
        for (int kk = 0; kk < d.KH; ++kk) mymask |= (unsigned)((unsigned)(xh0 + kk * d.dilh) < (unsigned)d.Hi) << (8 + kk);
        for (int kk = 0; kk < d.KW; ++kk) mymask |= (unsigned)((unsigned)(xw0 + kk * d.dilw) < (unsigned)d.Wi) << (16 + kk);
        const long long pix0 = ((long long)(xn + xd0) * d.Hi + xh0) * d.Wi + xw0;
        mybase = pix0 * d.Cin * (long long)sizeof(T);
      }
    };
    auto enter_tile = [&]() {
      const int grp = (tp & 63) & 56;
#pragma unroll
      for (int i = 0; i < XR; ++i) {
        const long long b = __shfl(mybase, grp | i, 64);
        rmask[i] = (unsigned)__shfl((int)mymask, grp | i, 64);
        xoff[i] = (unsigned)(b + xbias + (long long)(js * E) * (long long)sizeof(T));
        if (KR) {
          const long long m = d.m0 + (long long)my_pix_tile * BPIX + r0 + 32 * i;
          roff[i] = m < d.M ? (unsigned)((m * d.ldo + my_ch_tile * BCH + js * E) * (long long)sizeof(T)) : 0xffffffffu;
        }
      }
#pragma unroll
      for (int i = 0; i < WL; ++i) {
        const int row = r0 + 32 * i;
        woff[i] = (unsigned)(((long long)(my_ch_tile * BCH + row) * d.Kpad + js * E) * (long long)sizeof(T));
      }
      tkd = tkh = tkw = tc = 0;
      wko = 0;
      if (kt0 > 0) {
        if (d.korder && d.lcin >= 0) {
          const int tap = kt0 % d.ntaps, cb = kt0 / d.ntaps;
          tkw = tap % d.KW; tkh = (tap / d.KW) % d.KH; tkd = tap / (d.KW * d.KH);
          tc = cb * BK;
          wko = (unsigned)(((long long)tap * d.Cin + tc) * (long long)sizeof(T));
        } else {
          wko = (unsigned)kt0 * (unsigned)(BK * sizeof(T));
          if (d.lcin >= 0) {
            const int cpt = d.Cin / BK, tap = kt0 / cpt;
            tc = (kt0 - tap * cpt) * BK;
            tkw = tap % d.KW; tkh = (tap / d.KW) % d.KH; tkd = tap / (d.KW * d.KH);
          } else {
            tc = kt0 * BK;
          }
        }
      }
    };

    int ikt = 0, itile = 0;
    auto issue = [&](int stage) {
      if (ikt == 0) enter_tile();
      const unsigned sbase = lds0 + (unsigned)stage * (STAGE * 16);
      const unsigned sel = (1u << tkd) | (256u << tkh) | (65536u << tkw);
      const unsigned soff = (unsigned)(((long long)((tkd * d.dild * d.Hi + tkh * d.dilh) * d.Wi + tkw * d.dilw) * d.Cin + tc) * (long long)sizeof(T));
      const bool cok = tkd < d.KD && tc + js * E < d.Cin;
      if (ikt >= KT) {
        const unsigned ro = (unsigned)(ikt - KT) * (unsigned)(BK * sizeof(T));
#pragma unroll
        for (int i = 0; i < XR; ++i) blds16(roff[i], rsrc_r, ro, sbase + (BCH * 8 + i * 256) * 16);
        if (!BIG) {
#pragma unroll
          for (int i = 0; i < WL; ++i) blds16((unsigned)(((r0 + 32 * i) * 256 + js * E) * (int)sizeof(T)), rsrc_i, ro, sbase + (i * 256) * 16);
        }
      } else {
#pragma unroll
        for (int i = 0; i < XR; ++i) {
          const bool ok = cok && (rmask[i] & sel) == sel;
          blds16(ok ? xoff[i] : 0xffffffffu, rsrc_x, soff, sbase + (BCH * 8 + i * 256) * 16);
        }
#pragma unroll
        for (int i = 0; i < WL; ++i) blds16(woff[i], rsrc_w, wko, sbase + (i * 256) * 16);
      }
      if (ikt >= KT) {
      } else if (d.korder && d.lcin >= 0) {
        wko += (unsigned)d.Cin * (unsigned)sizeof(T);
        if (++tkw == d.KW) { tkw = 0; if (++tkh == d.KH) { tkh = 0; if (++tkd == d.KD) { tkd = 0; tc += BK; wko = (unsigned)tc * (unsigned)sizeof(T); } } }
      } else {
        wko += BK * (unsigned)sizeof(T);
        tc += BK;
        if (d.lcin >= 0 && tc >= d.Cin) {
          tc = 0;
          if (++tkw == d.KW) { tkw = 0; if (++tkh == d.KH) { tkh = 0; ++tkd; } }
        }
      }
      if (++ikt == KTT) { ikt = 0; ++itile; if (itile < n_my) prepare_tile(itile); }
    };

    if (total > 0) prepare_tile(0);
    if (total > 0) issue(0);
    if (NST == 3 && total > 1) issue(1);
    int st = 0, gk = 0;
    for (int g = 0; g < total; ++g) {
      if (NST == 2 || g + 1 >= total) asm volatile("s_waitcnt vmcnt(0)" ::: "memory");
      else asm volatile("s_waitcnt vmcnt(%0)" :: "n"(NP) : "memory");
      RGBM_BARRIER();
      if (NST == 3) { if (g + 2 < total) issue(st == 0 ? 2 : st - 1); }
      else { if (g + 1 < total) issue(st ^ 1); }
      st = st == NST - 1 ? 0 : st + 1;
      if (STAGED) { if (++gk == KTT) { gk = 0; RGBM_BARRIER(); } }
    }
    return;
  }

  const int wch = BIG ? (wave >> 2) * WCHW : (wave >> 1) * WCHW;
  const int wpix = BIG ? (wave & 3) * 64 : (wave & 1) * 64;
  const int li = lane & 31, lh = lane >> 5;
  const int rowA = wch + m32_row_channel(li), rowB = wpix + li;
  const unsigned offA = (unsigned)(rowA * 8 + (lh ^ ((rowA >> 1) & 7))) * 16u;
  const unsigned offB = (unsigned)(BCH * 8 + rowB * 8 + (lh ^ ((rowB >> 1) & 7))) * 16u;
  const char* ldsc = reinterpret_cast<const char*>(lds3);
  f32x16 acc[FA][FB];
  auto ident_frag = [&](int sub) {
    int lq = lane;
    asm volatile("" : "+v"(lq));
    const int qi = lq & 31, qh = lq >> 5;
    const int id_s = (qi >> 2) & 1, id_c = (qi & 3) + 4 * (qi >> 3);
    const int lh = qh;
    const unsigned one = std::is_same<T, f16_t>::value ? 0x3c00u : 0x3f80u;
    const bool mine = sub == id_s && lh == (id_c >> 3);
    const unsigned w = mine ? one << (16 * (id_c & 1)) : 0u;
    const int q = (id_c & 7) >> 1;
    return make_uint4(q == 0 ? w : 0u, q == 1 ? w : 0u, q == 2 ? w : 0u, q == 3 ? w : 0u);
  };
  auto load_step = [&](int st, int s, uint4 (&af)[FA], uint4 (&bf)[FB]) {
    const char* base = ldsc + st * (STAGE * 16);
    const unsigned oa = offA ^ ((unsigned)s << 5), ob = offB ^ ((unsigned)s << 5);
#pragma unroll
    for (int b = 0; b < FB; ++b) bf[b] = *reinterpret_cast<const uint4*>(base + ob + b * 4096);
#pragma unroll
    for (int a = 0; a < FA; ++a) af[a] = *reinterpret_cast<const uint4*>(base + oa + a * 4096);
  };
  auto mma_step = [&](const uint4 (&af)[FA], const uint4 (&bf)[FB]) {
#pragma unroll
    for (int a = 0; a < FA; ++a)
#pragma unroll
      for (int b = 0; b < FB; ++b) {
        Mma32<T>::run(af[a], bf[b], acc[a][b]);
      }
  };
  T* __restrict__ out = reinterpret_cast<T*>(d.out);
  const T* __restrict__ res = reinterpret_cast<const T*>(d.res);
  auto tile_interior = [&](int pix_tile, int ch_tile) {
    return (d.bias == nullptr || bias_lds) && d.m0 + (long long)(pix_tile + 1) * BPIX <= d.M && (ch_tile + 1) * BCH <= d.Cout && d.act != ACT_TANH;
  };
  int st = 0;
  for (int k = 0; k < n_my; ++k) {
    {
      int pt, ct;
      tile_of(k, pt, ct);
      if (tile_interior(pt, ct) && d.bias && part == 0) {
        const float* bp = lbias + ct * BCH + wch + lh * 16;
#pragma unroll
        for (int a = 0; a < FA; ++a) {
          f32x16 b16;
#pragma unroll
          for (int q = 0; q < 4; ++q) {
            const f32x4 b4 = *reinterpret_cast<const f32x4*>(bp + a * 32 + q * 4);
            b16[q * 4 + 0] = b4[0]; b16[q * 4 + 1] = b4[1]; b16[q * 4 + 2] = b4[2]; b16[q * 4 + 3] = b4[3];
          }
#pragma unroll
          for (int b = 0; b < FB; ++b) acc[a][b] = b16;
        }
      } else {
#pragma unroll
        for (int a = 0; a < FA; ++a)
#pragma unroll
          for (int b = 0; b < FB; ++b)
#pragma unroll
            for (int e = 0; e < 16; ++e) acc[a][b][e] = 0.f;
      }
    }
    if constexpr (X3) {
      const int zA = (rowA >> 1) & 7, zB = (rowB >> 1) & 7;
      unsigned oA3 = (unsigned)(rowA * 128) + (unsigned)(((2 * lh) ^ zA) << 4);
      unsigned oB3 = (unsigned)(BCH * 128 + rowB * 128) + (unsigned)(((2 * lh) ^ zB) << 4);
      const char* sb = ldsc;
      auto rdp = [&](unsigned off, uint4& hi, uint4& lo) {
        const uint4 c0 = *reinterpret_cast<const uint4*>(sb + off), c1 = *reinterpret_cast<const uint4*>(sb + (off ^ 16u));
        hi = make_uint4(c0.x, c0.y, c1.x, c1.y);
        lo = make_uint4(c0.z, c0.w, c1.z, c1.w);
      };
      const int KTM = BIG ? KT : KTT;
      for (int kt = 0; kt < KTM; ++kt) {
        asm volatile("s_waitcnt lgkmcnt(0)" ::: "memory");
        RGBM_BARRIER();
        asm volatile("" : "+v"(oA3), "+v"(oB3));
        sb = ldsc + st * (STAGE * 16);
#pragma unroll
        for (int s = 0; s < 2; ++s) {
          uint4 Bh[FB], Bl[FB], Al, Ah, Aln, Ahn;
          const unsigned ob = oB3 ^ ((unsigned)s << 6), oa = oA3 ^ ((unsigned)s << 6);
#pragma unroll
          for (int b = 0; b < FB; ++b) rdp(ob + b * 4096, Bh[b], Bl[b]);
          rdp(oa, Ah, Al);
          __builtin_amdgcn_sched_barrier(0);
#pragma unroll
          for (int a = 0; a < FA; ++a) {
            if (a + 1 < FA) rdp(oa + (a + 1) * 4096, Ahn, Aln);
            __builtin_amdgcn_sched_barrier(0);
#pragma unroll
            for (int b = 0; b < FB; ++b) Mma32<unsigned short>::run(Al, Bh[b], acc[a][b]);
#pragma unroll
            for (int b = 0; b < FB; ++b) Mma32<unsigned short>::run(Ah, Bl[b], acc[a][b]);
#pragma unroll
            for (int b = 0; b < FB; ++b) Mma32<unsigned short>::run(Ah, Bh[b], acc[a][b]);
            __builtin_amdgcn_sched_barrier(0);
            if (a + 1 < FA) { Al = Aln; Ah = Ahn; }
          }
        }
        st = st == NST - 1 ? 0 : st + 1;
      }
      if constexpr (BIG) {
        if (KR) {
#pragma unroll
          for (int r = 0; r < BCH / BK; ++r) {
            asm volatile("s_waitcnt lgkmcnt(0)" ::: "memory");
            RGBM_BARRIER();
            if (wch == ((32 * r) / WCHW) * WCHW) {
              asm volatile("" : "+v"(oB3));
              sb = ldsc + st * (STAGE * 16);
#pragma unroll
              for (int s2 = 0; s2 < 2; ++s2) {
                uint4 Bh[FB], Bl[FB];
                const unsigned ob = oB3 ^ ((unsigned)s2 << 6);
#pragma unroll
                for (int b = 0; b < FB; ++b) rdp(ob + b * 4096, Bh[b], Bl[b]);
                const uint4 Aid = ident_frag(s2);
#pragma unroll
                for (int b = 0; b < FB; ++b) Mma32<unsigned short>::run(Aid, Bl[b], acc[((32 * r) % WCHW) / 32][b]);
#pragma unroll
                for (int b = 0; b < FB; ++b) Mma32<unsigned short>::run(Aid, Bh[b], acc[((32 * r) % WCHW) / 32][b]);
              }
            }
            st ^= 1;
          }
        }
      }
    } else if constexpr (BIG) {
      uint4 A[FA], B[FB], Bn[FB];
      unsigned oA = offA, oB = offB;
      auto ldA = [&](int s, int a) { A[a] = *reinterpret_cast<const uint4*>(ldsc + st * (STAGE * 16) + (oA ^ ((unsigned)s << 5)) + a * 4096); };
      auto ldB = [&](int s, uint4 (&bf)[FB]) {
#pragma unroll
        for (int b = 0; b < FB; ++b) bf[b] = *reinterpret_cast<const uint4*>(ldsc + st * (STAGE * 16) + (oB ^ ((unsigned)s << 5)) + b * 4096);
      };
      auto ldAs = [&](int stg, int s, int a) { A[a] = *reinterpret_cast<const uint4*>(ldsc + stg * (STAGE * 16) + (oA ^ ((unsigned)s << 5)) + a * 4096); };
      auto ldBs = [&](int stg, int s, uint4 (&bf)[FB]) {
#pragma unroll
        for (int b = 0; b < FB; ++b) bf[b] = *reinterpret_cast<const uint4*>(ldsc + stg * (STAGE * 16) + (oB ^ ((unsigned)s << 5)) + b * 4096);
      };
      auto first3 = [&]() {
#pragma unroll
        for (int s = 0; s < 3; ++s) {
          ldBs(st, s + 1, Bn);
          __builtin_amdgcn_sched_barrier(0);
#pragma unroll
          for (int a = 0; a < FA; ++a) {
            Mma32<T>::run(A[a], B[0], acc[a][0]);
            Mma32<T>::run(A[a], B[1], acc[a][1]);
            __builtin_amdgcn_sched_barrier(0);
            ldAs(st, s + 1, a);
            __builtin_amdgcn_sched_barrier(0);
          }
          B[0] = Bn[0]; B[1] = Bn[1];
        }
      };
      asm volatile("s_waitcnt lgkmcnt(0)" ::: "memory");
      RGBM_BARRIER();
      asm volatile("" : "+v"(oA), "+v"(oB));
      ldBs(st, 0, B);
#pragma unroll
      for (int a = 0; a < FA; ++a) ldAs(st, 0, a);
      __builtin_amdgcn_sched_barrier(0);
      for (int kt = 0; kt + 1 < KT; ++kt) {
        first3();
        if (M32_SHIFT) {
          asm volatile("s_waitcnt lgkmcnt(0)" ::: "memory");
          RGBM_BARRIER();
          asm volatile("" : "+v"(oA), "+v"(oB));
          ldBs(st ^ 1, 0, Bn);
          __builtin_amdgcn_sched_barrier(0);
#pragma unroll
          for (int a = 0; a < FA; ++a) {
            Mma32<T>::run(A[a], B[0], acc[a][0]);
            Mma32<T>::run(A[a], B[1], acc[a][1]);
            __builtin_amdgcn_sched_barrier(0);
            ldAs(st ^ 1, 0, a);
            __builtin_amdgcn_sched_barrier(0);
          }
          B[0] = Bn[0]; B[1] = Bn[1];
        } else {
#pragma unroll
          for (int a = 0; a < FA; ++a) {
            Mma32<T>::run(A[a], B[0], acc[a][0]);
            Mma32<T>::run(A[a], B[1], acc[a][1]);
            __builtin_amdgcn_sched_barrier(0);
          }
          asm volatile("s_waitcnt lgkmcnt(0)" ::: "memory");
          RGBM_BARRIER();
          asm volatile("" : "+v"(oA), "+v"(oB));
          ldBs(st ^ 1, 0, B);
#pragma unroll
          for (int a = 0; a < FA; ++a) ldAs(st ^ 1, 0, a);
          __builtin_amdgcn_sched_barrier(0);
        }
        st ^= 1;
      }
      first3();
#if M32_RACE_PROBE
      if (wave == 5 && !KR) { for (int q = 0; q < 32; ++q) __builtin_amdgcn_s_sleep(2); }
#endif
#pragma unroll
      for (int a = 0; a < FA; ++a) {
        Mma32<T>::run(A[a], B[0], acc[a][0]);
        Mma32<T>::run(A[a], B[1], acc[a][1]);
        __builtin_amdgcn_sched_barrier(0);
      }
      st ^= 1;
      if (KR) {
#pragma unroll
        for (int r = 0; r < BCH / BK; ++r) {
          asm volatile("s_waitcnt lgkmcnt(0)" ::: "memory");
          RGBM_BARRIER();
#if M32_RACE_PROBE
          if (wave == 5 && r == BCH / BK - 1) { for (int q = 0; q < 32; ++q) __builtin_amdgcn_s_sleep(2); }
#endif
          asm volatile("" : "+v"(oB));
#pragma unroll
          for (int s = 0; s < 4; ++s) {
            if (wch == ((64 * r + 16 * s) / WCHW) * WCHW) {
              ldB(s, B);
              const uint4 Aid = ident_frag(s & 1);
              Mma32<T>::run(Aid, B[0], acc[((64 * r + 16 * s) % WCHW) / 32][0]);
              Mma32<T>::run(Aid, B[1], acc[((64 * r + 16 * s) % WCHW) / 32][1]);
            }
          }
          st ^= 1;
        }
      }
    } else {
      uint4 A0[FA], B0[FB], A1[FA], B1[FB];
      for (int kt = 0; kt < KTT; ++kt) {
        asm volatile("s_waitcnt lgkmcnt(0)" ::: "memory");
        RGBM_BARRIER();
        load_step(st, 0, A0, B0);
        __builtin_amdgcn_sched_barrier(0);
        if (kt > 0) mma_step(A1, B1);
        __builtin_amdgcn_sched_barrier(0);
        load_step(st, 1, A1, B1);
        __builtin_amdgcn_sched_barrier(0);
        mma_step(A0, B0);
        __builtin_amdgcn_sched_barrier(0);
        load_step(st, 2, A0, B0);
        __builtin_amdgcn_sched_barrier(0);
        mma_step(A1, B1);
        __builtin_amdgcn_sched_barrier(0);
        load_step(st, 3, A1, B1);
        __builtin_amdgcn_sched_barrier(0);
        mma_step(A0, B0);
        __builtin_amdgcn_sched_barrier(0);
        st = st == 2 ? 0 : st + 1;
      }
      mma_step(A1, B1);
    }

    if constexpr (STAGED) {
      asm volatile("s_waitcnt lgkmcnt(0)" ::: "memory");
      RGBM_BARRIER();
    }
    if constexpr (KSPLIT) {
      if (nsp > 1) {
        constexpr int WFL = FA * FB * 64 * 16;
        float* sc = d.kscratch + (((long long)vtile * nsp + part) * NMW + wave) * WFL;
#pragma unroll
        for (int a = 0; a < FA; ++a)
#pragma unroll
          for (int b = 0; b < FB; ++b)
#pragma unroll
            for (int q = 0; q < 4; ++q)
            {
              const f32x4 v = f32x4{acc[a][b][4 * q], acc[a][b][4 * q + 1], acc[a][b][4 * q + 2], acc[a][b][4 * q + 3]};
              asm volatile("global_store_dwordx4 %0, %1, off sc1" :: "v"(sc + (((a * FB + b) * 4 + q) * 64 + lane) * 4), "v"(v) : "memory");
            }
        asm volatile("s_waitcnt vmcnt(0)" ::: "memory");
        unsigned arrived = 0;
        if (lane == 0) arrived = __hip_atomic_fetch_add(d.kcount + (long long)vtile * NMW + wave, 1u, __ATOMIC_RELAXED, __HIP_MEMORY_SCOPE_AGENT);
        arrived = (unsigned)__builtin_amdgcn_readfirstlane((int)arrived);
        if (arrived != (unsigned)(nsp - 1)) continue;
#pragma unroll
        for (int a = 0; a < FA; ++a)
#pragma unroll
          for (int b = 0; b < FB; ++b)
#pragma unroll
            for (int e = 0; e < 16; ++e) acc[a][b][e] = 0.f;
        for (int p = 0; p < nsp; ++p) {
          const float* sp = d.kscratch + (((long long)vtile * nsp + p) * NMW + wave) * WFL;
          f32x4 t[FA * FB * 4];
#pragma unroll
          for (int i = 0; i < FA * FB * 4; ++i)
            asm volatile("global_load_dwordx4 %0, %1, off sc1" : "=v"(t[i]) : "v"(sp + (i * 64 + lane) * 4) : "memory");
          asm volatile("s_waitcnt vmcnt(0)" ::: "memory");
#pragma unroll
          for (int i = 0; i < FA * FB * 4; ++i) asm volatile("" : "+v"(t[i]));
#pragma unroll
          for (int a = 0; a < FA; ++a)
#pragma unroll
            for (int b = 0; b < FB; ++b)
#pragma unroll
              for (int q = 0; q < 4; ++q)
#pragma unroll
                for (int e = 0; e < 4; ++e) acc[a][b][4 * q + e] += t[(a * FB + b) * 4 + q][e];
        }
        if (lane == 0) __hip_atomic_store(d.kcount + (long long)vtile * NMW + wave, 0u, __ATOMIC_RELAXED, __HIP_MEMORY_SCOPE_AGENT);
      }
    }
    int pix_tile, ch_tile;
    tile_of(k, pix_tile, ch_tile);
    const bool interior = tile_interior(pix_tile, ch_tile);
    long long obase[FB];
    int nn[FB];
    bool pok[FB];
    const bool dense_out = d.osd == 1 && d.osh == 1 && d.osw == 1 && d.opd == 0 && d.oph == 0 && d.opw == 0 && d.Dq == d.Do &&
                           d.Hq == d.Ho && d.Wq == d.Wo;
#pragma unroll
    for (int b = 0; b < FB; ++b) {
      const long long m = d.m0 + (long long)pix_tile * BPIX + wpix + b * 32 + li;
      pok[b] = m < d.M;
      if (dense_out && (interior || d.bias_stride == 0)) {
        nn[b] = 0;
        obase[b] = (pok[b] ? m : 0ll) * d.ldo;
        continue;
      }
      unsigned n, qd, qh, qw;
      decode_row(d, pok[b] ? (unsigned)m : 0u, n, qd, qh, qw);
      nn[b] = (int)n;
      obase[b] = ((((long long)n * d.Do + (qd * d.osd + d.opd)) * d.Ho + (qh * d.osh + d.oph)) * d.Wo + (qw * d.osw + d.opw)) * d.ldo;
    }
    constexpr int CHK = 16 / (int)sizeof(T);
    constexpr int NQ = 16 / CHK;
    if (interior) {
      const float nslope = d.act == ACT_RELU ? 0.f : d.act == ACT_PRELU ? d.slope : 1.f;
      auto fast = [&](auto resc) {
        constexpr int RES = decltype(resc)::value;
        constexpr int NF = FA * FB;
        constexpr int AR = FA < (X3 ? 2 : 4) ? FA : (X3 ? 2 : 4);
        static_assert(FA % AR == 0, "whole store rounds");
        uint4 pk[AR][NQ];
        uint4 rr[4][NQ];
        const long long mrow = d.m0 + (long long)pix_tile * BPIX + wpix;
        const int ch0 = ch_tile * BCH + wch;
        unsigned lofs_c = (unsigned)((li * d.ldo + lh * 16) * (int)sizeof(T));
        asm volatile("" : "+v"(lofs_c));
        auto rd = [&](int i) {
          const int b = i / FA, a = i % FA;
          const char* ub = reinterpret_cast<const char*>(res + (mrow + b * 32) * d.ldo + ch0 + a * 32);
#pragma unroll
          for (int q = 0; q < NQ; ++q) rr[i & 3][q] = *reinterpret_cast<const uint4*>(ub + lofs_c + q * 16);
        };
        auto make = [&](int i) {
          const int b = i / FA, a = i % FA;
#pragma unroll
          for (int q = 0; q < NQ; ++q) {
            float v[CHK], rv[CHK];
#pragma unroll
            for (int e = 0; e < CHK; ++e) v[e] = acc[a][b][q * CHK + e];
            if (RES != RES_NONE) unpack_chunk(rr[i & 3][q], rv, T());
            if (RES == RES_PRE_ACT) {
#pragma unroll
              for (int e = 0; e < CHK; ++e) v[e] += rv[e];
            }
#pragma unroll
            for (int e = 0; e < CHK; ++e) v[e] = v[e] < 0.f ? __builtin_fmaxf(v[e], -3.402823466e38f) * nslope : v[e];
            if (RES == RES_POST_ACT) {
#pragma unroll
              for (int e = 0; e < CHK; ++e) v[e] += rv[e];
            }
            pk[a % AR][q] = pack_chunk(v, T());
          }
        };
        auto store_round = [&](int b, int ar) {
          if constexpr (STAGED) {
            char* stg = const_cast<char*>(ldsc) + (st ^ 1) * (STAGE * 16) + wave * 8192;
            unsigned wofs = (unsigned)(li * 256 + (((lh * NQ) ^ (li & 15)) << 4));
            unsigned rofs = (unsigned)((lane >> 4) * 256 + (((lane & 15) ^ (lane >> 4)) << 4));
            unsigned gofs = (unsigned)(((lane >> 4) * d.ldo + (lane & 15) * CHK) * (int)sizeof(T));
            asm volatile("" : "+v"(wofs), "+v"(rofs), "+v"(gofs));
#pragma unroll
            for (int a = 0; a < AR; ++a)
#pragma unroll
              for (int q = 0; q < NQ; ++q)
                *reinterpret_cast<uint4*>(stg + (wofs ^ (unsigned)((a * 2 * NQ + q) << 4))) = pk[a][q];
            char* ob = reinterpret_cast<char*>(out + (mrow + b * 32) * d.ldo + ch0 + ar * AR * 32);
#pragma unroll
            for (int t = 0; t < 8; ++t) {
              const uint4 v = *reinterpret_cast<const uint4*>(stg + t * 1024 + (rofs ^ (unsigned)(((4 * t) & 15) << 4)));
              *reinterpret_cast<uint4*>(ob + (long long)(4 * t) * d.ldo * (long long)sizeof(T) + gofs) = v;
            }
          } else {
#pragma unroll
            for (int a = 0; a < AR; ++a)
#pragma unroll
              for (int q = 0; q < NQ; ++q)
                *reinterpret_cast<uint4*>(reinterpret_cast<char*>(out + (mrow + b * 32) * d.ldo + ch0 + (ar * AR + a) * 32) + lofs_c + q * 16) = pk[a][q];
          }
        };
        if (RES != RES_NONE) { rd(0); rd(1); __builtin_amdgcn_sched_barrier(0); }
#pragma unroll
        for (int i = 0; i < NF; ++i) {
          make(i);
          __builtin_amdgcn_sched_barrier(0);
          if (RES != RES_NONE) {
            if (i < FA - 1) rd(i + 2);
            else if (i == FA - 1) {
#pragma unroll
              for (int k = FA + 1; k < NF; ++k) rd(k);
            }
            __builtin_amdgcn_sched_barrier(0);
          }
          if (i % AR == AR - 1) { store_round(i / FA, (i % FA) / AR); __builtin_amdgcn_sched_barrier(0); }
        }
      };
      if (BIG || res_in_acc) fast(IC<RES_NONE>{});
      else if (d.res_mode == RES_NONE) fast(IC<RES_NONE>{});
      else if (d.res_mode == RES_PRE_ACT) fast(IC<RES_PRE_ACT>{});
      else fast(IC<RES_POST_ACT>{});
      continue;
    }
    if constexpr (BIG) continue;
#pragma unroll
    for (int a = 0; a < FA; ++a) {
      const int chL = ch_tile * BCH + wch + a * 32 + lh * 16;
#pragma unroll
      for (int b = 0; b < FB; ++b) {
#pragma unroll
        for (int q = 0; q < NQ; ++q) {
          const int c = chL + q * CHK;
          if (!pok[b] || c >= d.Cout) continue;
          const bool whole = c + CHK <= d.Cout;
          float v[CHK], rv[CHK];
#pragma unroll
          for (int e = 0; e < CHK; ++e) v[e] = acc[a][b][q * CHK + e];
          if (d.bias) {
            const float* bp = d.bias + (long long)nn[b] * d.bias_stride + c;
#pragma unroll
            for (int e = 0; e < CHK; ++e) if (e < 4 || whole) v[e] += bp[e];
          }
#pragma unroll
          for (int e = 0; e < CHK; ++e) rv[e] = 0.f;
          if (d.res_mode != RES_NONE && !res_in_acc) {
            if (whole) unpack_chunk(*reinterpret_cast<const uint4*>(res + obase[b] + c), rv, T());
            else load4(res + obase[b] + c, rv);
          }
          if (d.res_mode == RES_PRE_ACT && !res_in_acc) {
#pragma unroll
            for (int e = 0; e < CHK; ++e) v[e] += rv[e];
          }
#pragma unroll
          for (int e = 0; e < CHK; ++e) v[e] = apply_act_g(v[e], d.act, d.slope);
          if (d.res_mode == RES_POST_ACT) {
#pragma unroll
            for (int e = 0; e < CHK; ++e) v[e] += rv[e];
          }
          if (whole) *reinterpret_cast<uint4*>(out + obase[b] + c) = pack_chunk(v, T());
          else store4(out + obase[b] + c, v);
        }
      }
    }
  }
}

template <typename T, int BPIX, int BCH = 256>
static int launch_m32_range(ConvDesc d, hipStream_t s) {
  constexpr int NST = BPIX == 256 ? 2 : 3;
  constexpr size_t LDS = ((size_t)NST * (BCH + BPIX) * 8) * sizeof(uint4) + 2560 * sizeof(float);
  d.n_pix_tiles = (int)((d.M - d.m0 + BPIX - 1) / BPIX);
  d.n_ch_tiles = (d.Cout + BCH - 1) / BCH;
  const long long ntiles = (long long)d.n_pix_tiles * d.n_ch_tiles;
  RGBM_REQUIRE(ntiles > 0 && ntiles < (1ll << 31) && d.M < (1ll << 31), "conv grid out of range");
  d.n_tiles = (int)ntiles;
  make_fastdiv(d.Wq, d.fd_m[0], d.fd_s[0]);
  make_fastdiv(d.Hq, d.fd_m[1], d.fd_s[1]);
  make_fastdiv(d.Dq, d.fd_m[2], d.fd_s[2]);
  if (int rc = ensure_dynamic_lds(reinterpret_cast<const void*>(conv_igemm_m32_kernel<T, BPIX, BCH>), (int)LDS)) return rc;
  int n_cu = 0;
  if (int rc = persistent_grid_cus(&n_cu)) return rc;
  RGBM_REQUIRE(d.ksplit <= 1 || (BPIX == 128 && BCH <= 128 && ntiles * d.ksplit <= 4096 && d.kscratch && d.kcount), "K split: 64 / 128-channel x 128-pixel tiles, one workgroup per (tile, part)");
  const int grid = d.ksplit > 1 ? (int)(ntiles * d.ksplit) : ntiles < n_cu ? (int)ntiles : n_cu;
  prof_begin_launch(s, BPIX == 256 && BCH == 256 ? (std::is_same<T, bx3_t>::value ? 33 : 31) : (std::is_same<T, bx3_t>::value ? 41 : 40), d.algo_flops, d.algo_bytes);
  hipLaunchKernelGGL((conv_igemm_m32_kernel<T, BPIX, BCH>), dim3((unsigned)grid), dim3(BPIX == 256 ? 768 : 512), LDS, s, d);
  prof_end_launch(s);
  RGBM_CHECK_HIP(hipGetLastError());
  return 0;
}

template <typename T>
static int m32_identity(const void** out) {
  static std::mutex mu;
  static std::map<int, void*> per_dev;
  int dev = 0;
  RGBM_CHECK_HIP(hipGetDevice(&dev));
  std::lock_guard<std::mutex> lock(mu);
  void*& p = per_dev[dev];
  if (!p) {
    if (std::is_same<T, bx3_t>::value) {
      std::vector<unsigned short> h(256 * 256 * 2, 0);
      for (int i = 0; i < 256; ++i) h[(i * 256 + (i & ~3)) * 2 + (i & 3)] = 0x3f80;
      RGBM_CHECK_HIP(hipMalloc(&p, h.size() * 2));
      RGBM_CHECK_HIP(hipMemcpy(p, h.data(), h.size() * 2, hipMemcpyHostToDevice));
    } else {
      std::vector<unsigned short> h(256 * 256, 0);
      const unsigned short one = std::is_same<T, f16_t>::value ? 0x3c00 : 0x3f80;
      for (int i = 0; i < 256; ++i) h[i * 256 + i] = one;
      RGBM_CHECK_HIP(hipMalloc(&p, h.size() * 2));
      RGBM_CHECK_HIP(hipMemcpy(p, h.data(), h.size() * 2, hipMemcpyHostToDevice));
    }
  }
  *out = p;
  return 0;
}

static int m32_ksplit_buffers(hipStream_t s, float** scratch, unsigned** count) {
  static std::mutex mu;
  static std::map<std::pair<int, hipStream_t>, std::pair<float*, unsigned*>> per_stream;
  int dev = 0;
  RGBM_CHECK_HIP(hipGetDevice(&dev));
  std::lock_guard<std::mutex> lock(mu);
  auto& e = per_stream[std::make_pair(dev, s)];
  if (!e.first) {
    hipStreamCaptureStatus cs = hipStreamCaptureStatusNone;
    if (hipStreamIsCapturing(s, &cs) == hipSuccess && cs != hipStreamCaptureStatusNone) { *scratch = nullptr; *count = nullptr; return 0; }
    float* sc = nullptr; unsigned* cn = nullptr;
    RGBM_CHECK_HIP(hipMalloc(&sc, kM32SplitFloats * sizeof(float)));
    RGBM_CHECK_HIP(hipMalloc(&cn, kM32SplitCounters * sizeof(unsigned)));
    RGBM_CHECK_HIP(hipMemsetAsync(cn, 0, kM32SplitCounters * sizeof(unsigned), s));
    e.first = sc; e.second = cn;
  }
  *scratch = e.first; *count = e.second;
  return 0;
}

template <typename T>
static int m32_setup(ConvDesc& d, const ConvPlan& p, hipStream_t s) {
  d.m0 = 0;
  d.ident = nullptr;
  d.korder = p.korder;
  d.ksplit = 1; d.kscratch = nullptr; d.kcount = nullptr;
  if (p.ksplit > 1) {
    if (int rc = m32_ksplit_buffers(s, &d.kscratch, &d.kcount)) return rc;
    if (d.kscratch) d.ksplit = p.ksplit;
  }
  return p.identity_residual ? m32_identity<T>(&d.ident) : 0;
}

template <typename T>
static int launch_m32_tiles128(const ConvDesc& d, int bch, hipStream_t s) {
  return bch == 64 ? launch_m32_range<T, 128, 64>(d, s) : bch == 128 ? launch_m32_range<T, 128, 128>(d, s) : launch_m32_range<T, 128, 256>(d, s);
}

template <typename T>
static int launch_m32_small(ConvDesc d, const ConvPlan& p, hipStream_t s) {
  if (int rc = m32_setup<T>(d, p, s)) return rc;
  return launch_m32_tiles128<T>(d, p.bch, s);
}

template <typename T>
static int launch_m32(ConvDesc d, const ConvPlan& p, hipStream_t s) {
  if (int rc = m32_setup<T>(d, p, s)) return rc;
  if (p.main_rows > 0) {
    ConvDesc m = d;
    m.M = p.main_rows;
    const double frac = (double)m.M / (double)d.M;
    m.algo_flops = d.algo_flops * frac; m.algo_bytes = d.algo_bytes * frac;
    if (int rc = launch_m32_range<T, 256, 256>(m, s)) return rc;
    d.m0 = m.M;
    d.algo_flops *= 1.0 - frac; d.algo_bytes *= 1.0 - frac;
  }
  return p.tail_bch ? launch_m32_tiles128<T>(d, p.tail_bch, s) : 0;
}
```

### rgbmanip_amd/csrc/conv_plan.cpp

```cpp
#include "conv_plan.h"

#include "kernels.h"

namespace rgbm {

#ifndef M32_KSPLIT_MAX
#define M32_KSPLIT_MAX 4
#endif
#ifndef M32_KSPLIT_MINSTEPS
#define M32_KSPLIT_MINSTEPS 8
#endif

namespace {

bool uniform_taps(const ConvDesc& d, int bk) {
  if (d.KD > 8 || d.KH > 8 || d.KW > 8) return false;
  if (d.lcin < 0) return d.ntaps == 1;
  return d.Cin % bk == 0;
}

bool buffer_offsets_ok(const ConvDesc& d, int bch, long long esz) {
  const long long xbytes = ((long long)d.N * d.Di * d.Hi * d.Wi + (long long)(d.pd * d.Hi + d.ph) * d.Wi + d.pw) * d.Cin * esz;
  const long long wbytes = (long long)((d.Cout + bch - 1) / bch) * bch * d.Kpad * esz;
  return xbytes < (1ll << 32) - 65536 && wbytes < (1ll << 32) - 65536 && d.pd >= 0 && d.ph >= 0 && d.pw >= 0;
}

bool rowhalo_ok(const ConvDesc& d) {
  return d.KD == 1 && d.KH == 3 && d.KW == 3 && d.sd == 1 && d.sh == 1 && d.sw == 1 && d.Dq == 1 && d.Di == 1 &&
         d.dilh == d.dilw && d.dilw >= 1 && d.dilw <= 4 && d.ph == d.dilh && d.pw == d.dilw && d.pd == 0 &&
         d.lcin >= 6 && d.Hq == d.Hi && d.Wq == d.Wi && d.Wi > 2 * d.dilw && d.osh == 1 && d.osw == 1;
}

int m32_small_choice(const ConvDesc& d, int n_cu, bool slim_ok) {
  const long long p128 = (d.M + 127) / 128, p256 = (d.M + 255) / 256;
  auto cost = [&](long long tiles, int kb) { return (double)((tiles + n_cu - 1) / n_cu) * (double)(kb + 8); };
  double best = slim_ok ? cost(p256 * (d.Cout / 64), 40) : 1e30;
  int pick = 0;
  const int bch[3] = {64, 128, 256}, kb[3] = {24, 32, 48};
  for (int i = 0; i < 3; ++i) {
    if (d.Cout % bch[i]) continue;
    const double c = cost(p128 * (d.Cout / bch[i]), kb[i]);
    if (c < best * 0.999) { best = c; pick = bch[i]; }
  }
  return pick;
}

int m32_ksplit_choice(const ConvDesc& d, int flags, long long tiles, int n_cu, int bch, int n_waves) {
  if ((flags & DBG_NO_KSPLIT) || tiles <= 0 || bch > 128) return 1;
  int n = (int)(n_cu / tiles);
  if (n > M32_KSPLIT_MAX) n = M32_KSPLIT_MAX;
  while (n > 1 && d.KT / n < M32_KSPLIT_MINSTEPS) --n;
  if (n < 2) return 1;
  if ((size_t)tiles * n * bch * 128 > kM32SplitFloats || (size_t)tiles * n_waves > kM32SplitCounters) return 1;
  return n;
}

}

int plan_conv(const ConvDesc& d, int dtype, const ConvTuning& t, ConvPlan* out) {
  RGBM_REQUIRE(d.M > 0 && d.M < (1ll << 31), "conv M out of range");
  RGBM_REQUIRE(d.Cout % 4 == 0 && d.ldo % 4 == 0, "conv Cout/ldo must be multiples of 4");
  RGBM_REQUIRE(d.KT > 0 && d.Kpad == d.KT * conv_bk(dtype), "conv K padding mismatch");
  RGBM_REQUIRE(d.Cin % dtype_chunk(dtype) == 0, "conv Cin must be a multiple of the 16-byte chunk");
  if (d.lcin >= 0) {
    RGBM_REQUIRE((1 << d.lcin) == d.Cin, "conv lcin mismatch");
  } else {
    RGBM_REQUIRE(d.ntaps == 1, "linear-K mode needs a single tap");
  }
  const int f = t.flags, n_cu = t.n_cu;
  const long long esz = (long long)dtype_size(dtype);
  const bool bits16 = esz == 2, mfma32 = dtype != F32;
  const int ch_tile = conv_ch_tile(d.Cout);
  const bool uni = uniform_taps(d, conv_bk(dtype)) && !(f & DBG_NONUNIFORM_TAPS);
  const bool out16 = (((unsigned long long)d.out | (unsigned long long)(d.ldo * esz)) & 15ull) == 0ull;
  const bool rows16 = out16 && ((unsigned long long)d.res & 15ull) == 0ull;
  const bool dense_out = d.osd == 1 && d.osh == 1 && d.osw == 1 && d.opd == 0 && d.oph == 0 && d.opw == 0 && d.Dq == d.Do && d.Hq == d.Ho && d.Wq == d.Wo;
  const bool ident_ok = dense_out && d.res_mode == RES_PRE_ACT && d.res != nullptr && d.M * d.ldo * esz < (1ll << 32) - 65536;
  const bool ws_rows = d.M >= (t.ws_min_rows > 0 ? t.ws_min_rows : 1024);

  ConvPlan p = {};
  p.uniform_taps = uni;
  p.ksplit = 1;
  p.korder = (f & DBG_KORDER_TAPS_OUTER) ? 0 : 1;
  auto pick = [&](int kernel, int bch, int bpix) {
    p.kernel = kernel; p.bch = bch; p.bpix = bpix;
    p.buf_ok = buffer_offsets_ok(d, bch, esz) && !(f & DBG_GLOBAL_ADDR);
    *out = p;
    return 0;
  };
  auto generic = [&]() { return pick(CONV_GENERIC, ch_tile, ch_tile == 128 ? 128 : 256); };
  auto small = [&](int bch) {
    p.ksplit = m32_ksplit_choice(d, f, ((d.M + 127) / 128) * ((d.Cout + bch - 1) / bch), n_cu, bch, 4);
    p.identity_residual = ident_ok && d.Cout % 256 == 0;
    return pick(CONV_M32_SMALL, bch, 128);
  };

  if (d.out_f32) {
    RGBM_REQUIRE(dtype == BF16X3 && d.w2 == nullptr, "out_f32 is a bf16x3 option of the generic kernel");
    return generic();
  }
  if (ch_tile == 128 && !(f & DBG_NO_WS) && ws_rows) {
    if (!uni || (f & DBG_V3_FOR_WS) || !rows16) return pick(CONV_V3, 128, 256);
    if (!(f & DBG_NO_SLIM_SMALL) && d.Cout % 64 == 0) {
      const long long slim_tiles = ((d.M + 255) / 256) * (d.Cout / 64);
      if (mfma32) {
        if (d.Cout % 256 == 0 && ((d.M + 255) / 256) * (d.Cout / 256) < n_cu && t.gemm_kernel >= 1 && !(f & (DBG_M32_TAILS_R5 | DBG_WS_128x256)) &&
            buffer_offsets_ok(d, 256, esz)) {
          const int bch = t.gemm_kernel == 1 ? 256 : m32_small_choice(d, n_cu, slim_tiles <= n_cu);
          if (bch) return small(bch);
        }
        if (d.Cout == 128 && ((d.M + 127) / 128) * 2 * 2 <= n_cu && t.gemm_kernel == 2 &&
            !(f & (DBG_M32_TAILS_R5 | DBG_WS_128x256 | DBG_NO_KSPLIT | DBG_L2_SLIM_TILE)) && d.w2 == nullptr && buffer_offsets_ok(d, 64, esz))
          return small(64);
      }
      if (slim_tiles <= n_cu) return pick(CONV_WS_SLIM, 64, 256);
    }
    if (d.Cout % 256 == 0 && !(f & DBG_WS_128x256)) {
      if (!(mfma32 && buffer_offsets_ok(d, 256, esz) && t.gemm_kernel >= 1)) return pick(CONV_WS_WIDE, 256, 128);
      const bool big_ok = dense_out && (d.bias == nullptr || (d.bias_stride == 0 && d.Cout <= 2560)) && d.act != ACT_TANH &&
                          (d.res_mode == RES_NONE || (d.res_mode == RES_PRE_ACT && d.res != nullptr)) && d.M * d.ldo * esz < (1ll << 32) - 65536;
      const long long P = d.M / 256, n_ch = d.Cout / 256, tiles = P * n_ch;
      long long Pm = 0;
      if (t.gemm_kernel != 1 && big_ok && tiles >= n_cu) {
        const long long rem = tiles % n_cu;
        Pm = (rem == 0 || rem * 10 >= (long long)n_cu * 6) ? P : (tiles - rem) / n_ch;
      }
      p.main_rows = Pm * 256;
      p.identity_residual = ident_ok;
      p.tail_bch = p.main_rows == d.M ? 0 : 256;
      const long long pt = (d.M - p.main_rows + 127) / 128;
      if (p.tail_bch && t.gemm_kernel != 1 && !(f & DBG_M32_TAILS_R5)) {
        if (pt * (d.Cout / 64) <= n_cu) p.tail_bch = 64;
        else if (pt * (d.Cout / 128) <= n_cu) p.tail_bch = 128;
      }
      return pick(CONV_M32, 256, 256);
    }
    return pick(CONV_WS, 128, 256);
  }
  if (bits16 && uni && !(f & DBG_NO_WS64) && ch_tile == 64 && d.res_mode == RES_NONE && d.KT >= 2 && ws_rows &&
      (d.w2 ? d.Cout == 64 && d.kpad2 == 64 && (d.cout2 == 16 || d.cout2 == 32) && d.ldo2 % 4 == 0 : out16))
    return rowhalo_ok(d) && !(f & DBG_NO_ROWHALO) ? pick(CONV_WS64_ROWHALO, 64, 256) : pick(CONV_WS64, 64, 256);
  RGBM_REQUIRE(d.w2 == nullptr, "a fused 1x1 needs the ws64 kernel (check conv_ws64_eligible first)");
  if (ch_tile == 64 && uni && ws_rows && !(f & (DBG_NO_WS | DBG_V3_FOR_WS | DBG_NO_SLIM64)) && rows16) return pick(CONV_WS_SLIM, 64, 256);
  return generic();
}

}
```

### rgbmanip_amd/csrc/conv_plan.h

```cpp
#pragma once
#include "common.h"

namespace rgbm {

struct ConvTuning {
  int flags;
  int gemm_kernel;
  long long ws_min_rows;
  int n_cu;
};

enum ConvKernel {
  CONV_GENERIC = 0,
  CONV_V3 = 1,
  CONV_WS = 2,
  CONV_WS_WIDE = 3,
  CONV_WS_SLIM = 4,
  CONV_WS64 = 5,
  CONV_WS64_ROWHALO = 6,
  CONV_M32 = 7,
  CONV_M32_SMALL = 8,
};

struct ConvPlan {
  int kernel;
  int bch, bpix;
  bool uniform_taps;
  long long main_rows;
  int tail_bch;
  int ksplit;
  bool identity_residual;
  int korder, buf_ok;
};

constexpr size_t kM32SplitFloats = 8u << 20, kM32SplitCounters = 16384;

int plan_conv(const ConvDesc& d, int dtype, const ConvTuning& t, ConvPlan* out);
int conv_tuning(int n_cu, ConvTuning* t);

}
```

### rgbmanip_amd/csrc/kernels.h

```cpp
#pragma once
#include <vector>

#include "common.h"

namespace rgbm {

int launch_nchw_to_nhwc_pad(int dtype, const float* in, void* out, int V, int C, int H, int W, int Cp, hipStream_t s);
int launch_maxpool3x3s2(int dtype, const void* in, void* out, int V, int H, int W, int C, hipStream_t s);
int launch_resize_bilinear_ac(int dtype, const void* in, void* out, int V, int Hs, int Ws, int C, int Ho, int Wo, int ldo,
                              int ch_off, hipStream_t s);
int launch_copy_channels(int dtype, const void* in, void* out, long long npix, int C, int ldo, int ch_off, hipStream_t s);
int launch_adaptive_avgpool(int dtype, const void* in, void* out, int V, int H, int W, int C, int S, hipStream_t s);
int launch_adaptive_avgpool_multi(int dtype, const void* in, void* const* outs, const int* bins, int nb, int V, int H, int W, int C,
                                  hipStream_t s);
int launch_psp_pool_conv(int dtype, const void* in, int ldi, const void* const* w, void* const* outs, const int* bins, int V, int H, int W,
                         int act, float slope, hipStream_t s);
int launch_psp_resize_cat(int dtype, const void* f, const void* const* stages, const int* bins, void* out, int V, int Ho, int Wo, hipStream_t s);
int launch_homography(const float* P_views, float* out, int V, int B, hipStream_t s);
int launch_build_volume(int dtype, const void* feat, const float* homog, const float* depths, void* vol, int v0, int Vc, int V,
                        int B, int D, int H, int W, hipStream_t s);

int launch_upconv_combine(int dtype, const void* z, const float* bias, void* out, int V, int h, int w, int Co, int ldo, int act,
                          float slope, hipStream_t s, const float* drop = nullptr);
int launch_upconv_final(int dtype, const void* x, const void* wz, const float* bias, float slope, const void* wf, const float* biasf,
                        void* out, int out_f32, int V, int h, int w, hipStream_t s, const void* wf_f16 = nullptr);

constexpr int kDropoutPerView = 256 + 64;
unsigned dropout_threshold(float p);
float dropout_scale(float p);
int launch_dropout_masks(float* masks, unsigned long long* state, int B, float p, unsigned long long seed, int advance, hipStream_t s);

size_t bn_scratch_bytes(int V);
int launch_bn_per_sample(int dtype, void* y, const void* res, const float* gamma, const float* beta, void* scratch, int V,
                         long long nvox, int C, int relu, hipStream_t s);

int launch_to_f32(int dtype, const void* in, float* out, long long n, hipStream_t s);

int launch_gather_points(int dtype, const void* feat, const int* choose, float* out, int V, int P, int HW, int C, hipStream_t s);
int launch_prob_softmax_depth(int dtype, const void* u11, const float* wprob, const int* choose, const float* depths,
                              float* prob, float* depth_out, int v0, int Vc, int B, int P, int D, int H, int W, int classmajor,
                              hipStream_t s);
int launch_dense_depth(int dtype, const void* u11, const float* wprob, const float* depths, float* depth_map, float* conf_map,
                       int v0, int Vc, int B, int D, int H, int W, int classmajor, hipStream_t s);
int launch_depth_to_points(const float* depth, const double* Kc, const double* E, int n, int S, float* points, hipStream_t s);
int launch_depth_consistency(const float* depth_a, const float* conf_a, const unsigned char* mask_a, const double* Ka, const double* Ea,
                             const float* depth_b, const double* Kb, const double* Eb, int n, int S, double px_max, double rel_max,
                             float conf_min, float* fused, float* reproj, float* rel, unsigned char* keep, hipStream_t s);
int launch_cloud_pack(const float* fused1, const unsigned char* keep1, const double* K1, const double* E1, const float* fused2,
                      const unsigned char* keep2, const double* K2, const double* E2, int n, int S, int cap, float* cloud, int* index,
                      int* count, hipStream_t s);
int launch_depth_fusion(const float* depth, const float* conf, const unsigned char* mask, const double* Kc, const double* E, int n, int V,
                        int S, double px_max, double rel_max, float conf_min, int n_min, float* fused, unsigned char* keep,
                        unsigned char* nviews, unsigned short* agree, hipStream_t s);
int launch_cloud_pack_views(const float* fused, const unsigned char* keep, const double* Kc, const double* E, int n, int V, int S, int cap,
                            float* cloud, int* index, int* count, hipStream_t s);
int launch_cloud_gather_views(const float* maps, const int* index, int n, int V, int S2, int C, int cap, float* out, hipStream_t s);
int launch_fuse_points(int dtype, const void* feat, const float* homog, const float* depths, const int* choose,
                       const float* prob, float* out, int V, int B, int P, int D, int H, int W, int ldo, int ch_off,
                       hipStream_t s, int Vn = -1);
int launch_mean_points(int dtype, const void* in, float* out, float* scratch, int V, int P, int C, hipStream_t s);
int launch_f32_to_f16(const float* in, void* out, long long n, hipStream_t s);
void stem_pack(const float* w, std::vector<float>& packed);
int launch_stem(int dtype, const float* img1, const float* img2, const void* wpk, void* out, int B, int V, int S, hipStream_t s);
int launch_stem_views(int dtype, const float* img, const void* wpk, void* out, int V, int S, hipStream_t s);
int launch_feature_store(const void* src, void* pool, const int* slots, int V, int pool_records, size_t part_off, size_t part_bytes,
                         size_t record_bytes, hipStream_t s);
int launch_feature_gather(const void* pool, void* dst, const int* slot1, const int* slot2, int B, int pool_records, size_t part_off,
                          size_t part_bytes, size_t record_bytes, hipStream_t s);
int launch_feature_bad_slot_nan(const int* slot1, const int* slot2, int B, int pool_records, float* const out[10], const int per_pose[10],
                                hipStream_t s);
int launch_crop_fingerprint(const float* img, int V, int n_words, unsigned long long* keys_out, hipStream_t s);
int launch_f32_to_bx3(const float* in, void* out, long long n, hipStream_t s);
int launch_view_linear(const float* x, const float* W, const float* bias, float* out, int V, int I, int O, int ldw, int i0,
                       int relu, hipStream_t s);
struct PointMlpDesc {
  const float* table;
  const void* feat;
  const int* choose;
  float* nocs4;
  float* pf;
  int ldpf, P, HW;
  long long N;
};
int point_mlp_table_floats();
void point_mlp_pack(const float* const w[6], const float* const b[6], float* table);
int launch_point_mlp(int feat_dtype, const PointMlpDesc& d, hipStream_t s);
int launch_dense_nocs(int feat_dtype, const float* table, const void* feat, float* out, long long N, hipStream_t s);
int launch_ortho6d(const float* r6, float* R, int V, hipStream_t s);
int launch_mean_points_partial(int dtype, const void* in, float* scratch, int V, int P, int C, hipStream_t s);
int launch_view_linear_mean(const float* partial, int P, float* mean_out, const float* W, const float* bias, float* out, int V, int I, int O,
                            int ldw, int i0, int relu, hipStream_t s);
int launch_pose_heads_mean(const float* partial, int P, float* mean_out, float* R, float* const w[3][3], float* const b[3][3],
                           float* const out[3], const int odim[3], int V, hipStream_t s);
constexpr int kMeanSplit = 8;
constexpr int kPoseMlpSlab = 128;
struct PoseMlpDesc {
  const float* pf96;
  const void* w[4];
  int ldw[4];
  const float* bias[4];
  const float* vbias;
  void* q128;
  float* part128;
  float* part256;
  int V, P;
};
bool pose_mlp_fits(int P);
int launch_pose_mlp1(const PoseMlpDesc& d, hipStream_t s);
int launch_pose_mlp2(const PoseMlpDesc& d, hipStream_t s);
int launch_pose_heads(const float* pf2, float* const w[3][3], float* const b[3][3], float* const out[3], const int odim[3], int V,
                      hipStream_t s);
int launch_stage_in(const float* P1, const float* P2, const int* c1, const int* c2, float* Pviews, int* choose, int B, int P, hipStream_t s);
int launch_stage_out(const float* nocs4, const float* depth, const float* R, const float* tv, const float* sv, float* const nocs[2],
                     float* const dep[2], float* const r[2], float* const t[2], float* const sz[2], int B, int P, int view2, hipStream_t s);
int launch_copy_cols(const float* in, float* out, long long rows, int ldi, int ldo, int n, hipStream_t s);

struct Conv3dTileDesc {
  const void* in; const void* wgt; void* out; const float* bias; const void* res;
  int N, Di, Hi, Wi;
  int Do, Ho, Wo;
  int Dq, Hq, Wq;
  int ntd, nth, ntw;
  int Cout, relu;
  const void* feat; const float* homog; const float* depths; int v0, V, B;
  int prof_variant; double algo_flops, algo_bytes;
  int out_classmajor;
  int feat_f16;
  const int* tile_list; const int* tile_count;
  int tile_mask_stride;
  const unsigned char* tile_mask;
};
enum DebugFlag {
  DBG_NO_WS = 8, DBG_NONUNIFORM_TAPS = 16, DBG_V3_FOR_WS = 64, DBG_NO_WS64 = 128, DBG_NO_ROWHALO = 256, DBG_GENERIC_RESIZE = 512,
  DBG_PSP_STAGE_R5 = 1024, DBG_POINT_MLP_R5 = 2048, DBG_TILE_CONV0 = 4096, DBG_NO_KSPLIT = 16384, DBG_L2_SLIM_TILE = 32768,
  DBG_WS_128x256 = 65536, DBG_NO_SLIM64 = 262144, DBG_KORDER_TAPS_OUTER = 1 << 20, DBG_SWEEP_ALT_BLEND = 1 << 21, DBG_SWEEP_DOT2 = 1 << 22,
  DBG_PP_ONE_KERNEL = 1 << 23, DBG_NO_SLIM_SMALL = 1 << 24, DBG_PP_GENERIC_SELECT = 1 << 25, DBG_PP_GUARD = 1 << 26, DBG_GLOBAL_ADDR = 1 << 27,
  DBG_SWEEP_PER_TILE = 1 << 28, DBG_SPARSE_TAIL_R5 = 1 << 29, DBG_M32_TAILS_R5 = 1 << 30, DBG_POSE_MLP_R6 = 1 << 19,
};
extern int g_debug_flags;
extern long long g_ws_min_rows;
extern int g_tuning_version;
extern int g_gemm_kernel;
void conv3d_tile_pack(const float* w, const float* scale, int Cin, int Cout, int coutp, bool transposed, int dtype,
                      std::vector<float>& packed);
int launch_conv3d_tile(int layer, int dtype, const Conv3dTileDesc& d, hipStream_t s);
int sparse_mask_bytes_per_view(int S);
int sparse_mask_offset(int S, int layer);
int launch_sparse_masks(const int* choose, int v0, int Vc, int P, int S, unsigned char* masks, int* sweep_list, int* sweep_count,
                        hipStream_t s);
int conv3d_tile_dims(int layer, int dtype, int* TD, int* TH, int* TW);

void conv0_sweep_pack(const float* w, const float* scale, std::vector<float>& packed);
int launch_conv0_sweep(const Conv3dTileDesc& d, int dtype, hipStream_t s);

int conv0_sweep_x3_upload(const std::vector<float>& packed, void** dev);
int launch_conv0_sweep_x3(const Conv3dTileDesc& d, hipStream_t s);
int launch_bx3_to_f32(const void* in, float* out, long long n, hipStream_t s);

int launch_prob_sparse(const void* u9, const void* c0, const void* w11_packed, const float* bias11, const float* wprob,
                       const int* choose, const float* depths, float* prob, float* depth_out, int v0, int Vc, int B, int P,
                       int D, int H, int W, int dtype, hipStream_t s, const void* w11_taps = nullptr);
void prob_sparse_pack(const float* w, const float* scale, std::vector<float>& packed);

int launch_prepare_inputs(const float* rgb, const unsigned char* mask, const double* K, const int* frame_map, int N, int H, int W, int S, int P,
                          unsigned seed, float* img, int* choose, float* pts2d, double* Kcrop, int* window, int* valid,
                          unsigned char* small_scratch, hipStream_t s, int frame0 = 0);
int launch_prepare_inputs_u8(const unsigned char* rgb, const unsigned char* mask, const double* K, const int* frame_map, int N, int H, int W,
                             int S, int P, unsigned seed, float* img, int* choose, float* pts2d, double* Kcrop, int* window, int* valid,
                             unsigned char* small_scratch, hipStream_t s, int frame0 = 0);
int launch_prepare_inputs_opt(const void* rgb, int pixel_type, int normalize, const unsigned char* mask, const double* K, const int* frame_map,
                              int N, int H, int W, int S, int P, unsigned seed, float* img, int* choose, float* pts2d, double* Kcrop,
                              int* window, int* valid, unsigned char* small_scratch, hipStream_t s, int frame0 = 0);
int launch_prepare_inputs_windows(const void* pix, int pixel_type, int normalize, const unsigned char* mask_pix, const long long* offset,
                                  const int* window, const int* valid_in, const double* K, int frame0, int N, int H, int W, int S, int P,
                                  unsigned seed, float* img, int* choose, float* pts2d, double* Kcrop, int* valid, unsigned char* small_scratch,
                                  hipStream_t s);
int launch_quantize_frames(const float* src, unsigned char* dst, size_t n, hipStream_t s);

int launch_umeyama_ransac(const float* nocs, const float* depth, const int* choose, const double* Kc, const double* E1,
                          double* bbox, double* srt, int* valid, int B, int P, int img, unsigned seed, hipStream_t s);

int launch_cloud_gather(const float* map1, const float* map2, const int* index, int n, int S2, int C, int cap, float* out, hipStream_t s);
size_t cloud_similarity_scratch_bytes(int n, int cap);
int launch_cloud_similarity(const float* nocs, const float* cloud, const int* count, int n, int cap, unsigned seed, double* bbox, double* srt,
                            int* info, int* valid, void* scratch, size_t scratch_bytes, hipStream_t s);

int launch_projection(const double* Kc, const double* E, float* P, int n, hipStream_t s);
int launch_pnp_ransac(const float* nocs1, const float* pts1, const float* nocs2, const float* pts2, const double* K, const double* E1,
                      const double* E2, double* bbox, double* srt, int* info, int* valid, int B, int P, unsigned seed, hipStream_t s);

int launch_mask_extent(const unsigned char* mask, int N, int H, int W, int* ext, int* count, hipStream_t s);

int launch_postprocess(const float* nocs, const float* depth, const float* rot, const int* choose, const double* Kc,
                       const double* E1, double* bbox, double* ts_out, int* valid, int B, int P, int img, hipStream_t s,
                       void* scratch = nullptr, size_t scratch_bytes = 0);
int launch_postprocess_regressed(const float* nocs, const float* rot, const float* tr, const float* sv, const double* E1, double* bbox,
                                 double* ts_out, int* valid, int B, int P, hipStream_t s);
int launch_microbench_mfma(float* scratch, int iters, int random_operands, double* flops, hipStream_t s);
int microbench_mfma_scratch_floats(int* n);
int launch_microbench_copy(const void* src, void* dst, size_t bytes, hipStream_t s);
size_t postprocess_scratch_bytes(int B);
int postprocess_slices(int B);

int launch_gae(int T, int N, const float* rewards, const unsigned char* dones, const float* values, const float* last_values,
               float gamma, float lam, float* returns, float* adv, double* sums, hipStream_t s);
int launch_adv_normalise(long long n_local, float* adv, const double* sums, double count_total, hipStream_t s);

struct PolicyLayout { int dims[5]; int log_std; int w[2][4]; int b[2][4]; int total; };
struct PolicyOptState { int t; int n_updates; float lr; float last_kl; float last_norm; float pad_; double sum_surr; double sum_vloss; };
int launch_policy_forward(const float* params, const PolicyLayout& L, int n, int mode, const float* obs, const float* noise,
                          float* actions, float* logp, float* value, float* mu, hipStream_t s);
int policy_partial_floats(const PolicyLayout& L, int n);
int launch_ppo_minibatch(const float* params, const PolicyLayout& L, int n, const float* obs, const float* actions,
                         const float* old_logp, const float* adv, const float* returns, const float* old_values,
                         const float* old_mu, const float* old_sigma, float clip, float vcoef, float ecoef, float* partial,
                         float* grads, hipStream_t s);
constexpr int POLICY_MAX_HIDDEN = 6, POLICY_MAX_WIDTH = 512, POLICY_MAX_ACT = 32;
enum { PACT_ELU = 0, PACT_SELU = 1, PACT_RELU = 2, PACT_LRELU = 3, PACT_TANH = 4, PACT_SIGMOID = 5 };
struct PolicyDesc {
  int obs_dim, state_dim, act_dim, activation, asymmetric;
  int n_hidden[2];
  int hidden[2][POLICY_MAX_HIDDEN];
  int w[2][POLICY_MAX_HIDDEN + 1];
  int b[2][POLICY_MAX_HIDDEN + 1];
  int log_std, total;
};
int launch_policy_forward_ex(const float* params, const PolicyDesc& D, int n, int mode, const float* obs, const float* states,
                             const float* noise, float* actions, float* logp, float* value, float* mu, hipStream_t s);
int ppo_scratch_floats_ex(const PolicyDesc& D, int n, int clipped_vloss, size_t* count);
int launch_ppo_minibatch_ex(const float* params, const PolicyDesc& D, int n, const float* obs, const float* states,
                            const float* actions, const float* old_logp, const float* adv, const float* returns,
                            const float* old_values, const float* old_mu, const float* old_sigma, float clip, float vcoef, float ecoef,
                            int clipped_vloss, float* scratch, float* grads, hipStream_t s);
int launch_ppo_adam(float* params, const float* grads, float* m, float* v, PolicyOptState* st, int total, float inv_world,
                    float max_norm, float desired_kl, float lr_min, float lr_max, int adaptive, hipStream_t s);

}
```

### rgbmanip_amd/csrc/layers.cpp

```cpp
#include "layers.h"
#include "kernels.h"

#include <string.h>

#include <map>
#include <mutex>
#include <utility>
#include <vector>

namespace rgbm {

static thread_local std::string g_err;
void set_error(const std::string& s) { g_err = s; }
const char* last_error_cstr() { return g_err.c_str(); }

static inline unsigned short host_f32_to_bf16(float f) {
  unsigned u;
  memcpy(&u, &f, 4);
  if ((u & 0x7fffffffu) > 0x7f800000u) return (unsigned short)((u >> 16) | 0x40);
  u += 0x7fffu + ((u >> 16) & 1u);
  return (unsigned short)(u >> 16);
}

int ensure_dynamic_lds(const void* fn, int bytes) {
  static std::mutex mu;
  static std::map<std::pair<int, const void*>, int> set_for;
  int dev = 0;
  RGBM_CHECK_HIP(hipGetDevice(&dev));
  std::lock_guard<std::mutex> lock(mu);
  int& have = set_for[std::make_pair(dev, fn)];
  if (bytes > have) {
    RGBM_CHECK_HIP(hipFuncSetAttribute(fn, hipFuncAttributeMaxDynamicSharedMemorySize, bytes));
    have = bytes;
  }
  return 0;
}

int persistent_grid_cus(int* n_cu) {
  static std::mutex mu;
  static std::map<int, int> per_dev;
  int dev = 0;
  RGBM_CHECK_HIP(hipGetDevice(&dev));
  std::lock_guard<std::mutex> lock(mu);
  int& n = per_dev[dev];
  if (n == 0) {
    RGBM_CHECK_HIP(hipDeviceGetAttribute(&n, hipDeviceAttributeMultiprocessorCount, dev));
    n = n / 8 * 8;
    if (n < 8) n = 8;
  }
  *n_cu = n;
  return 0;
}

static int upload_bytes(const void* host, size_t bytes, DevBuf& dev) {
  RGBM_CHECK_HIP(hipMalloc(dev.out(), bytes));
  RGBM_CHECK_HIP(hipMemcpy(dev.get(), host, bytes, hipMemcpyHostToDevice));
  return 0;
}

int upload_f32(const float* host, size_t n, DevBuf& dev) { return upload_bytes(host, n * sizeof(float), dev); }

static inline unsigned short host_f32_to_f16(float f) {
  const _Float16 h = (_Float16)(f > 65504.f ? 65504.f : (f < -65504.f ? -65504.f : f));
  unsigned short u;
  memcpy(&u, &h, 2);
  return u;
}

bool weights_fit_f16(const std::vector<float>& w) {
  double total = 0.0, small = 0.0;
  for (float v : w) {
    const float a = v < 0.f ? -v : v;
    if (!(a < 65504.f)) return false;
    total += a;
    if (a != 0.f && a < 6.103515625e-05f) small += a;
  }
  return small <= 1e-3 * total;
}

int upload_packed(const std::vector<float>& w, int dtype, DevBuf& dev) {
  if (dtype == BF16 || dtype == F16) {
    std::vector<unsigned short> h(w.size());
    for (size_t i = 0; i < w.size(); ++i) h[i] = dtype == BF16 ? host_f32_to_bf16(w[i]) : host_f32_to_f16(w[i]);
    return upload_bytes(h.data(), h.size() * 2, dev);
  }
  if (dtype == BF16X3) {
    RGBM_REQUIRE(w.size() % 4 == 0, "bf16x3 weights: element count must be a multiple of 4");
    std::vector<unsigned> h(w.size());
    for (size_t i = 0; i < w.size(); i += 4) {
      unsigned short hi[4], lo[4];
      for (int e = 0; e < 4; ++e) {
        hi[e] = host_f32_to_bf16(w[i + e]);
        unsigned u = (unsigned)hi[e] << 16;
        float hf;
        memcpy(&hf, &u, 4);
        lo[e] = host_f32_to_bf16(w[i + e] - hf);
      }
      h[i] = hi[0] | ((unsigned)hi[1] << 16); h[i + 1] = hi[2] | ((unsigned)hi[3] << 16);
      h[i + 2] = lo[0] | ((unsigned)lo[1] << 16); h[i + 3] = lo[2] | ((unsigned)lo[3] << 16);
    }
    return upload_bytes(h.data(), h.size() * 4, dev);
  }
  return upload_bytes(w.data(), w.size() * 4, dev);
}

int conv_pack_geom(const ConvGeom& g, int dtype, int Cin_pad, int Cout_pad, int cls, PackedConv* pc) {
  const int BK = conv_bk(dtype);
  RGBM_REQUIRE(Cin_pad % dtype_chunk(dtype) == 0 && Cin_pad >= g.Cin, "Cin_pad");
  RGBM_REQUIRE(Cout_pad % 4 == 0 && Cout_pad >= g.Cout, "Cout_pad");
  *pc = PackedConv();
  if (!g.transposed) {
    pc->KD = g.KD; pc->KH = g.KH; pc->KW = g.KW;
  } else {
    RGBM_REQUIRE(g.KD == 3 && g.KH == 3 && g.KW == 3 && g.sd == 2 && g.sh == 2 && g.sw == 2, "transposed conv geometry");
    RGBM_REQUIRE(cls >= 0 && cls < 8, "sub-pixel class");
    pc->KD = 1 + ((cls >> 2) & 1); pc->KH = 1 + ((cls >> 1) & 1); pc->KW = 1 + (cls & 1);
  }
  pc->ntaps = pc->KD * pc->KH * pc->KW;
  if (pc->ntaps > 1 || g.transposed) RGBM_REQUIRE(is_pow2(Cin_pad), "multi-tap / transposed conv needs power-of-two Cin_pad");
  const int K = pc->ntaps * Cin_pad;
  pc->Kpad = (K + BK - 1) / BK * BK;
  pc->KT = pc->Kpad / BK;
  return 0;
}

int ConvLayer::init(int dtype_, const ConvGeom& g_, const float* w, const float* bias_h, const float* bn_scale,
                    const float* bn_shift, int Cin_pad_, int Cout_pad_) {
  g = g_;
  dtype = dtype_;
  Cin_pad = Cin_pad_;
  Cout_pad = Cout_pad_;
  PackedConv pc;
  if (int rc = conv_pack_geom(g, dtype, Cin_pad, Cout_pad, 0, &pc)) return rc;
  const int bch = conv_ch_tile(Cout_pad);
  const int rows = (Cout_pad + bch - 1) / bch * bch;

  if (bias_h || bn_shift) {
    std::vector<float> b(Cout_pad, 0.f);
    for (int o = 0; o < g.Cout; ++o) {
      float v = bias_h ? bias_h[o] : 0.f;
      if (bn_scale) v *= bn_scale[o];
      if (bn_shift) v += bn_shift[o];
      b[o] = v;
    }
    if (upload_f32(b.data(), b.size(), bias)) return -2;
  }

  auto finish = [&](PackedConv& pc, std::vector<float>& packed) -> int {
    if (upload_packed(packed, dtype, pc.w)) return -2;
    packs.push_back(std::move(pc));
    return 0;
  };

  if (!g.transposed) {
    std::vector<float> packed((size_t)rows * pc.Kpad, 0.f);
    const long long kvol = (long long)g.KD * g.KH * g.KW;
    for (int o = 0; o < g.Cout; ++o) {
      const float sc = bn_scale ? bn_scale[o] : 1.f;
      for (int c = 0; c < g.Cin; ++c)
        for (int t = 0; t < pc.ntaps; ++t)
          packed[(size_t)o * pc.Kpad + (size_t)t * Cin_pad + c] = w[((long long)o * g.Cin + c) * kvol + t] * sc;
    }
    return finish(pc, packed);
  }

  for (int cls = 0; cls < 8; ++cls) {
    const int pd_ = (cls >> 2) & 1, ph_ = (cls >> 1) & 1, pw_ = cls & 1;
    if (int rc = conv_pack_geom(g, dtype, Cin_pad, Cout_pad, cls, &pc)) return rc;
    std::vector<float> packed((size_t)rows * pc.Kpad, 0.f);
    auto kidx = [](int p, int delta) { return p == 0 ? 1 : (delta == 0 ? 2 : 0); };
    for (int o = 0; o < g.Cout; ++o) {
      const float sc = bn_scale ? bn_scale[o] : 1.f;
      for (int c = 0; c < g.Cin; ++c)
        for (int dd = 0; dd < pc.KD; ++dd)
          for (int dh = 0; dh < pc.KH; ++dh)
            for (int dw = 0; dw < pc.KW; ++dw) {
              const int t = (dd * pc.KH + dh) * pc.KW + dw;
              const int kd = kidx(pd_, dd), kh = kidx(ph_, dh), kw = kidx(pw_, dw);
              packed[(size_t)o * pc.Kpad + (size_t)t * Cin_pad + c] =
                  w[(((long long)c * g.Cout + o) * 3 + kd) * 9 + kh * 3 + kw] * sc;
            }
    }
    if (finish(pc, packed)) return -2;
  }
  return 0;
}

void conv_out_dims(const ConvGeom& g, int Di, int Hi, int Wi, int& Do, int& Ho, int& Wo) {
  if (g.transposed) { Do = 2 * Di; Ho = 2 * Hi; Wo = 2 * Wi; return; }
  Do = (Di + 2 * g.pd - g.dild * (g.KD - 1) - 1) / g.sd + 1;
  Ho = (Hi + 2 * g.ph - g.dilh * (g.KH - 1) - 1) / g.sh + 1;
  Wo = (Wi + 2 * g.pw - g.dilw * (g.KW - 1) - 1) / g.sw + 1;
}

void ConvLayer::out_dims(int Di, int Hi, int Wi, int& Do, int& Ho, int& Wo) const { conv_out_dims(g, Di, Hi, Wi, Do, Ho, Wo); }

void conv_desc_geom(ConvDesc& d, const ConvGeom& g, const PackedConv& pc, int Cin_pad, int Cout_pad, int N, int Di, int Hi, int Wi,
                    int ldo, int cls) {
  memset(&d, 0, sizeof(d));
  conv_out_dims(g, Di, Hi, Wi, d.Do, d.Ho, d.Wo);
  d.N = N; d.Di = Di; d.Hi = Hi; d.Wi = Wi;
  d.Cin = Cin_pad;
  d.Cout = Cout_pad; d.ldo = ldo;
  d.act = g.act; d.slope = g.slope;
  d.KD = pc.KD; d.KH = pc.KH; d.KW = pc.KW;
  d.ntaps = pc.ntaps; d.KT = pc.KT; d.Kpad = pc.Kpad;
  d.lcin = (pc.ntaps > 1 || is_pow2(Cin_pad)) ? ilog2(Cin_pad) : -1;
  if (g.transposed) {
    d.Dq = Di; d.Hq = Hi; d.Wq = Wi;
    d.sd = d.sh = d.sw = 1; d.pd = d.ph = d.pw = 0;
    d.dild = d.dilh = d.dilw = 1;
    d.osd = d.osh = d.osw = 2;
    d.opd = (cls >> 2) & 1; d.oph = (cls >> 1) & 1; d.opw = cls & 1;
  } else {
    d.Dq = d.Do; d.Hq = d.Ho; d.Wq = d.Wo;
    d.sd = g.sd; d.sh = g.sh; d.sw = g.sw; d.pd = g.pd; d.ph = g.ph; d.pw = g.pw;
    d.dild = g.dild; d.dilh = g.dilh; d.dilw = g.dilw;
    d.osd = d.osh = d.osw = 1;
    d.opd = d.oph = d.opw = 0;
  }
  d.M = (long long)N * d.Dq * d.Hq * d.Wq;
}

int ConvLayer::build_desc(ConvDesc& d, const void* in, void* out, int N, int Di, int Hi, int Wi, int ldo, const void* res,
                          int res_mode, const float* bias_override, int bias_stride, int cls, bool out_plain_f32) const {
  RGBM_REQUIRE(!packs.empty(), "conv layer not initialised");
  const PackedConv& pc = packs[cls];
  conv_desc_geom(d, g, pc, Cin_pad, Cout_pad, N, Di, Hi, Wi, ldo, cls);
  d.in = in; d.out = out; d.res = res; d.wgt = pc.w.get();
  d.bias = bias_override ? bias_override : bias.get<float>();
  d.bias_stride = bias_override ? bias_stride : 0;
  d.res_mode = res ? res_mode : RES_NONE;
  d.out_f32 = (out_plain_f32 && dtype == BF16X3) ? 1 : 0;
  d.algo_flops = 2.0 * (double)d.M * g.Cout * (double)pc.ntaps * g.Cin;
  d.algo_bytes = ((double)d.M * g.Cout + (cls == 0 ? (double)N * Di * Hi * Wi * g.Cin : 0.0) +
                  (res ? (double)d.M * g.Cout : 0.0)) * (double)dtype_size(dtype) +
                 (double)g.Cout * pc.ntaps * g.Cin * (double)dtype_size(dtype);
  return 0;
}

int ConvLayer::run(const void* in, void* out, int N, int Di, int Hi, int Wi, int ldo, const void* res, int res_mode,
                   const float* bias_override, int bias_stride, hipStream_t s, bool out_plain_f32) const {
  const int nclass = g.transposed ? 8 : 1;
  for (int cls = 0; cls < nclass; ++cls) {
    ConvDesc d;
    if (int rc = build_desc(d, in, out, N, Di, Hi, Wi, ldo, res, res_mode, bias_override, bias_stride, cls, out_plain_f32)) return rc;
    if (int rc = launch_conv(d, dtype, s)) return rc;
  }
  return 0;
}

int ConvLayer::run_then_1x1(const ConvLayer& next, const void* in, void* mid, int ldmid, void* out2, int ldo2, int N, int Di, int Hi,
                            int Wi, bool allow_fuse, bool* fused, hipStream_t s, bool out2_plain_f32) const {
  if (fused) *fused = false;
  const ConvGeom& ng = next.g;
  const bool is1x1 = !ng.transposed && ng.KD == 1 && ng.KH == 1 && ng.KW == 1 && ng.sd == 1 && ng.sh == 1 && ng.sw == 1 &&
                     ng.pd == 0 && ng.ph == 0 && ng.pw == 0 && next.packs.size() == 1;
  if (allow_fuse && is1x1 && !g.transposed && dtype_size(dtype) == 2 && next.dtype == dtype && next.Cin_pad == Cout_pad) {
    ConvDesc d;
    if (int rc = build_desc(d, in, mid, N, Di, Hi, Wi, ldmid, nullptr, RES_NONE, nullptr, 0, 0)) return rc;
    d.w2 = next.packs[0].w.get(); d.bias2 = next.bias.get<float>(); d.out2 = out2; d.ldo2 = ldo2; d.cout2 = next.Cout_pad;
    d.kpad2 = next.packs[0].Kpad; d.act2 = ng.act; d.slope2 = ng.slope;
    if (conv_ws64_eligible(d, dtype)) {
      d.algo_flops += 2.0 * (double)d.M * ng.Cout * ng.Cin;
      d.algo_bytes += ((double)d.M * ng.Cout - (double)d.M * g.Cout) * 2.0;
      if (int rc = launch_conv(d, dtype, s)) return rc;
      if (fused) *fused = true;
      return 0;
    }
  }
  if (int rc = run(in, mid, N, Di, Hi, Wi, ldmid, nullptr, RES_NONE, nullptr, 0, s)) return rc;
  int Do, Ho, Wo;
  out_dims(Di, Hi, Wi, Do, Ho, Wo);
  return next.run(mid, out2, N, Do, Ho, Wo, ldo2, nullptr, RES_NONE, nullptr, 0, s, out2_plain_f32);
}

int UpConvLayer::init(int dtype, int Cin, int Cout_, const float* w, const float* bias_h, int act_, float slope_) {
  Cout = Cout_; act = act_; slope = slope_;
  RGBM_REQUIRE(Cout % dtype_chunk(dtype) == 0, "upconv Cout must be a multiple of the 16-byte chunk");
  std::vector<float> wz((size_t)9 * Cout * Cin);
  for (int t = 0; t < 9; ++t)
    for (int o = 0; o < Cout; ++o)
      for (int c = 0; c < Cin; ++c) wz[((size_t)t * Cout + o) * Cin + c] = w[((size_t)o * Cin + c) * 9 + t];
  ConvGeom g;
  g.Cin = Cin; g.Cout = 9 * Cout; g.act = ACT_NONE;
  split = (dtype != F32 && 9 * Cout > 256 && (9 * Cout) % 256 != 0 && (9 * Cout) % 256 <= 64 && Cin % 64 == 0) ? (9 * Cout) / 256 * 256 : 0;
  if (split) {
    ConvGeom g1 = g, g2 = g;
    g1.Cout = split; g2.Cout = 9 * Cout - split;
    if (int rc = gemm.init(dtype, g1, wz.data(), nullptr, nullptr, nullptr, Cin, g1.Cout)) return rc;
    if (int rc = gemm2.init(dtype, g2, wz.data() + (size_t)split * Cin, nullptr, nullptr, nullptr, Cin, g2.Cout)) return rc;
  } else {
    if (int rc = gemm.init(dtype, g, wz.data(), nullptr, nullptr, nullptr, Cin, 9 * Cout)) return rc;
  }
  if (bias_h) { if (upload_f32(bias_h, Cout, bias)) return -2; }
  return 0;
}

int UpConvLayer::run_gemm(const void* in, void* z, int V, int h, int w, hipStream_t s) const {
  if (int rc = gemm.run(in, z, V, 1, h, w, 9 * Cout, nullptr, RES_NONE, nullptr, 0, s)) return rc;
  if (split)
    if (int rc = gemm2.run(in, reinterpret_cast<char*>(z) + (size_t)split * dtype_size(gemm.dtype), V, 1, h, w, 9 * Cout, nullptr, RES_NONE, nullptr, 0, s)) return rc;
  return 0;
}

int UpConvLayer::combine(const void* z, void* out, int V, int h, int w, int ldo, hipStream_t s, const float* drop) const {
  return launch_upconv_combine(gemm.dtype, z, bias.get<float>(), out, V, h, w, Cout, ldo, act, slope, s, drop);
}

int UpConvLayer::run(const void* in, void* z, void* out, int V, int h, int w, int ldo, hipStream_t s, const float* drop) const {
  if (int rc = run_gemm(in, z, V, h, w, s)) return rc;
  return combine(z, out, V, h, w, ldo, s, drop);
}

int UpConvFinal::init(int dtype_, const float* w3, const float* b3, float slope_, const float* wfin, const float* bfin) {
  RGBM_REQUIRE(dtype_ == BF16 || dtype_ == F16 || dtype_ == BF16X3, "upconv + final: 16-bit or split-pair storage");
  dtype = dtype_; slope = slope_;
  std::vector<float> z((size_t)9 * 64 * 64), f(wfin, wfin + 32 * 64);
  for (int t = 0; t < 9; ++t)
    for (int o = 0; o < 64; ++o)
      for (int c = 0; c < 64; ++c) z[((size_t)t * 64 + o) * 64 + c] = w3[((size_t)o * 64 + c) * 9 + t];
  if (int rc = upload_packed(z, dtype, wz)) return rc;
  if (int rc = upload_packed(f, dtype, wf)) return rc;
  if (dtype == BF16 && weights_fit_f16(f)) if (int rc = upload_packed(f, F16, wf_h)) return rc;
  if (upload_f32(b3, 64, bias) || upload_f32(bfin, 32, biasf)) return -2;
  return 0;
}

int UpConvFinal::run(const void* in, void* out, int out_kind, int V, int h, int w, hipStream_t s) const {
  return launch_upconv_final(dtype, in, wz.get(), bias.get<float>(), slope, wf.get(), biasf.get<float>(), out, out_kind, V, h, w, s, wf_h.get());
}

}
```

### rgbmanip_amd/csrc/layers.h

```cpp
#pragma once
#include <map>
#include <string>
#include <vector>

#include "common.h"

namespace rgbm {

struct HostTensor {
  const float* data = nullptr;
  std::vector<long long> shape;
  long long numel() const { long long n = 1; for (auto s : shape) n *= s; return n; }
};
typedef std::map<std::string, HostTensor> StateDict;

class DevBuf {
 public:
  DevBuf() = default;
  DevBuf(DevBuf&& o) noexcept : p_(o.p_) { o.p_ = nullptr; }
  DevBuf& operator=(DevBuf&& o) noexcept {
    if (this != &o) { reset(); p_ = o.p_; o.p_ = nullptr; }
    return *this;
  }
  DevBuf(const DevBuf&) = delete;
  DevBuf& operator=(const DevBuf&) = delete;
  ~DevBuf() { reset(); }
  void reset() {
    if (p_) (void)hipFree(p_);
    p_ = nullptr;
  }
  void** out() { reset(); return &p_; }
  template <class T = void> T* get() const { return static_cast<T*>(p_); }
  explicit operator bool() const { return p_ != nullptr; }

 private:
  void* p_ = nullptr;
};

struct ConvGeom {
  int Cin = 0, Cout = 0;
  int KD = 1, KH = 1, KW = 1;
  int sd = 1, sh = 1, sw = 1;
  int pd = 0, ph = 0, pw = 0;
  int dild = 1, dilh = 1, dilw = 1;
  bool transposed = false;
  int act = ACT_NONE;
  float slope = 0.f;
};

struct PackedConv {
  DevBuf w;
  int KD = 1, KH = 1, KW = 1, ntaps = 1, Kpad = 0, KT = 0;
};

int conv_pack_geom(const ConvGeom& g, int dtype, int Cin_pad, int Cout_pad, int cls, PackedConv* pc);
void conv_out_dims(const ConvGeom& g, int Di, int Hi, int Wi, int& Do, int& Ho, int& Wo);
void conv_desc_geom(ConvDesc& d, const ConvGeom& g, const PackedConv& pc, int Cin_pad, int Cout_pad, int N, int Di, int Hi, int Wi,
                    int ldo, int cls);

struct ConvLayer {
  ConvGeom g;
  int dtype = F32;
  int Cin_pad = 0;
  int Cout_pad = 0;
  DevBuf bias;
  std::vector<PackedConv> packs;

  int init(int dtype, const ConvGeom& g, const float* w, const float* bias, const float* bn_scale, const float* bn_shift,
           int Cin_pad, int Cout_pad);

  int run(const void* in, void* out, int N, int Di, int Hi, int Wi, int ldo, const void* res, int res_mode,
          const float* bias_override, int bias_stride, hipStream_t s, bool out_plain_f32 = false) const;
  void out_dims(int Di, int Hi, int Wi, int& Do, int& Ho, int& Wo) const;
  int run_then_1x1(const ConvLayer& next, const void* in, void* mid, int ldmid, void* out2, int ldo2, int N, int Di, int Hi, int Wi,
                   bool allow_fuse, bool* fused, hipStream_t s, bool out2_plain_f32 = false) const;
  int build_desc(ConvDesc& d, const void* in, void* out, int N, int Di, int Hi, int Wi, int ldo, const void* res, int res_mode,
                 const float* bias_override, int bias_stride, int cls, bool out_plain_f32 = false) const;
};

struct UpConvLayer {
  ConvLayer gemm;
  ConvLayer gemm2;
  int split = 0;
  DevBuf bias;
  int Cout = 0, act = ACT_NONE;
  float slope = 0.f;
  int init(int dtype, int Cin, int Cout, const float* w, const float* bias_h, int act, float slope);
  size_t scratch_elems(int V, int h, int w) const { return (size_t)V * h * w * 9 * Cout; }
  int run(const void* in, void* z, void* out, int V, int h, int w, int ldo, hipStream_t s, const float* drop = nullptr) const;
  int run_gemm(const void* in, void* z, int V, int h, int w, hipStream_t s) const;
  int combine(const void* z, void* out, int V, int h, int w, int ldo, hipStream_t s, const float* drop = nullptr) const;
};

struct UpConvFinal {
  DevBuf wz;
  DevBuf wf;
  DevBuf wf_h;
  DevBuf bias;
  DevBuf biasf;
  float slope = 0.f;
  int dtype = 0;
  bool ready() const { return (bool)wz; }
  bool f16_ready() const { return (bool)wf_h; }
  int init(int dtype, const float* w3, const float* b3, float slope, const float* wfin, const float* bfin);
  int run(const void* in, void* out, int out_kind, int V, int h, int w, hipStream_t s) const;
};

bool weights_fit_f16(const std::vector<float>& w);
int upload_packed(const std::vector<float>& w, int dtype, DevBuf& dev);
int upload_f32(const float* host, size_t n, DevBuf& dev);

}
```

Measured before the change: 5836.

## Skip out-of-bounds filter taps by grouping border pixels into tap-range classes

```diff
diff --git a/include/rgbm.h b/include/rgbm.h
--- a/include/rgbm.h
+++ b/include/rgbm.h
@@ -243,6 +243,11 @@
 int rgbm_conv_plan(int dtype, int N, int D, int H, int W, int Cin, int Cin_pad, int Cout, int Cout_pad, int KD, int KH, int KW,
                    int stride_d, int stride_hw, int pad_d, int pad_hw, int dil_hw, int transposed, int has_bias, int res_mode, int act,
                    int cls, int n_cu, int32_t* plan);
+#define RGBM_BORDER_HEAD_INTS 10
+int rgbm_conv_border_plan(int dtype, int N, int H, int W, int Cin, int Cout, int K, int stride, int pad, int dil, int res_mode, int n_cu,
+                          int32_t* head, int32_t* classes, int cap_classes, int32_t* tiles, int32_t* order, int cap_tiles, int32_t* wg_off,
+                          int cap_wg, int32_t* rows, int64_t cap_rows);
+int rgbm_conv_border_launches(int64_t* count);
 int rgbm_bn_per_sample_scratch_bytes(int V, size_t* bytes);
 int rgbm_bn_per_sample(int dtype, void* y_dev, const void* res_dev, const float* gamma_dev, const float* beta_dev, void* scratch_dev,
                        int V, int64_t nvox, int C, int relu, void* stream);
diff --git a/rgbmanip_amd/_lib.py b/rgbmanip_amd/_lib.py
--- a/rgbmanip_amd/_lib.py
+++ b/rgbmanip_amd/_lib.py
@@ -155,6 +155,9 @@
     "rgbm_conv_nd": (_i, [_i, _vp, _i, _i, _i, _i, _i, _i, _vp, _i, _i, _i, _i, _i, _i, _i, _i, _i, _i, _i, _vp, _vp, _vp,
                           _vp, _i, _i, _f, _vp, _vp]),
     "rgbm_conv_plan": (_i, [_i] * 23 + [C.POINTER(C.c_int32)]),
+    "rgbm_conv_border_plan": (_i, [_i] * 12 + [C.POINTER(C.c_int32)] * 2 + [_i] + [C.POINTER(C.c_int32)] * 2 + [_i, C.POINTER(C.c_int32), _i,
+                                   C.POINTER(C.c_int32), _i64]),
+    "rgbm_conv_border_launches": (_i, [C.POINTER(C.c_int64)]),
     "rgbm_bn_per_sample_scratch_bytes": (_i, [_i, C.POINTER(_sz)]),
     "rgbm_bn_per_sample": (_i, [_i, _vp, _vp, _vp, _vp, _vp, _i, _i64, _i, _i, _vp]),
     "rgbm_conv3d_tile": (_i, [_i, _i, _vp, _i, _i, _i, _i, _vp, _vp, _vp, _vp, _vp, _vp]),
diff --git a/rgbmanip_amd/csrc/capi.cpp b/rgbmanip_amd/csrc/capi.cpp
--- a/rgbmanip_amd/csrc/capi.cpp
+++ b/rgbmanip_amd/csrc/capi.cpp
@@ -615,6 +615,63 @@
   return 0;
 }
 
+int rgbm_conv_border_plan(int dtype, int N, int H, int W, int Cin, int Cout, int K, int stride, int pad, int dil, int res_mode, int n_cu,
+                          int32_t* head, int32_t* classes, int cap_classes, int32_t* tiles, int32_t* order, int cap_tiles, int32_t* wg_off,
+                          int cap_wg, int32_t* rows, int64_t cap_rows) {
+  RGBM_REQUIRE(head && n_cu >= 0 && dtype >= F32 && dtype <= BF16X3 && N > 0 && H > 0 && W > 0 && K > 0, "conv_border_plan arguments");
+  const ConvGeom g = conv_nd_geom(Cin, Cout, 1, K, K, 1, stride, 0, pad, dil, 0, ACT_RELU, 0.f);
+  PackedConv pc;
+  const int E = dtype_chunk(dtype);
+  const int Cin_pad = (Cin + E - 1) / E * E, Cout_pad = (Cout + 3) / 4 * 4;
+  if (int rc = conv_pack_geom(g, dtype, Cin_pad, Cout_pad, 0, &pc)) return rc;
+  ConvDesc d;
+  conv_desc_geom(d, g, pc, Cin_pad, Cout_pad, N, 1, H, W, Cout_pad, 0);
+  alignas(16) static const float buffer[4] = {};
+  d.in = d.wgt = buffer; d.out = const_cast<float*>(buffer);
+  d.res = res_mode != RES_NONE ? buffer : nullptr;
+  d.res_mode = res_mode;
+  d.w_finite = 1;
+  ConvTuning t;
+  ConvPlan p;
+  if (int rc = conv_tuning(n_cu, &t)) return rc;
+  if (int rc = plan_conv(d, dtype, t, &p)) return rc;
+  memset(head, 0, RGBM_BORDER_HEAD_INTS * sizeof(int32_t));
+  BorderPlan bp;
+  if (p.kernel != CONV_M32 || !p.border || !plan_border(d, dtype, t.flags, p.main_rows, t.n_cu, &bp)) return 0;
+  const int32_t h[RGBM_BORDER_HEAD_INTS] = {1, (int32_t)bp.classes.size(), (int32_t)bp.tiles.size(), bp.n_wg, (int32_t)bp.rows.size(),
+                                             (int32_t)bp.max_wg_steps, (int32_t)bp.total_steps, (int32_t)bp.parent_steps, bp.steps_per_tap, bp.kr};
+  memcpy(head, h, sizeof(h));
+  if (classes) {
+    RGBM_REQUIRE((int)bp.classes.size() <= cap_classes, "conv_border_plan: cap_classes too small");
+    for (size_t c = 0; c < bp.classes.size(); ++c) {
+      classes[3 * c] = bp.classes[c].n_pix; classes[3 * c + 1] = bp.classes[c].mask; classes[3 * c + 2] = (int32_t)bp.classes[c].row0;
+    }
+  }
+  if (tiles || order) RGBM_REQUIRE((int)bp.tiles.size() <= cap_tiles, "conv_border_plan: cap_tiles too small");
+  if (tiles)
+    for (size_t i = 0; i < bp.tiles.size(); ++i) {
+      const BorderTile& bt = bp.tiles[i];
+      const int32_t v[5] = {bt.cls, bt.ch, bt.mask, bt.steps, (int32_t)bt.row0};
+      memcpy(tiles + 5 * i, v, sizeof(v));
+    }
+  if (order) memcpy(order, bp.order.data(), bp.order.size() * sizeof(int32_t));
+  if (wg_off) {
+    RGBM_REQUIRE(bp.n_wg + 1 <= cap_wg, "conv_border_plan: cap_wg too small");
+    memcpy(wg_off, bp.wg_off.data(), bp.wg_off.size() * sizeof(int32_t));
+  }
+  if (rows) {
+    RGBM_REQUIRE((int64_t)bp.rows.size() <= cap_rows, "conv_border_plan: cap_rows too small");
+    memcpy(rows, bp.rows.data(), bp.rows.size() * sizeof(int32_t));
+  }
+  return 0;
+}
+
+int rgbm_conv_border_launches(int64_t* count) {
+  RGBM_REQUIRE(count, "conv_border_launches arguments");
+  *count = border_launch_count();
+  return 0;
+}
+
 int rgbm_upsample_conv3x3(int dtype, const void* in_dev, int V, int h, int w, int Cin, const float* w_host, int Cout,
                           const float* bias_host, int act, float slope, void* z_scratch_dev, void* out_dev, void* stream) {
   RGBM_REQUIRE(in_dev && w_host && z_scratch_dev && out_dev, "upsample_conv3x3 arguments");
diff --git a/rgbmanip_amd/csrc/common.h b/rgbmanip_amd/csrc/common.h
--- a/rgbmanip_amd/csrc/common.h
+++ b/rgbmanip_amd/csrc/common.h
@@ -238,6 +238,7 @@
   double algo_flops, algo_bytes;
   int out_f32;
   int ksplit; float* kscratch; unsigned* kcount;
+  int w_finite; const int* btab; int b_nwg, b_ent, b_rows;
 };
 
 int launch_conv(const ConvDesc& d, int dtype, hipStream_t s);
diff --git a/rgbmanip_amd/csrc/conv_igemm_glds.hip b/rgbmanip_amd/csrc/conv_igemm_glds.hip
--- a/rgbmanip_amd/csrc/conv_igemm_glds.hip
+++ b/rgbmanip_amd/csrc/conv_igemm_glds.hip
@@ -1,3 +1,4 @@
+#include <atomic>
 #include <map>
 #include <mutex>
 #include <type_traits>
diff --git a/rgbmanip_amd/csrc/conv_igemm_m32.inc b/rgbmanip_amd/csrc/conv_igemm_m32.inc
--- a/rgbmanip_amd/csrc/conv_igemm_m32.inc
+++ b/rgbmanip_amd/csrc/conv_igemm_m32.inc
@@ -60,9 +60,20 @@
   const bool res_in_acc = d.ident != nullptr && d.res_mode == RES_PRE_ACT;
   const int KR = (res_in_acc && part == nsp - 1) ? BCH / BK : 0;
   const int KTT = KT + KR;
-  const int n_my = vtile >= 0 ? 1 : ((int)d.n_tiles - (int)blockIdx.x + (int)gridDim.x - 1) / (int)gridDim.x;
-  const int total = n_my * KTT;
+  const bool bm = STAGED && !X3 && d.btab != nullptr;
+  const int* __restrict__ bent = d.btab;
+  int n_my = vtile >= 0 ? 1 : ((int)d.n_tiles - (int)blockIdx.x + (int)gridDim.x - 1) / (int)gridDim.x;
+  int total = n_my * KTT;
+  if (bm) {
+    const int be0 = d.btab[blockIdx.x];
+    n_my = d.btab[blockIdx.x + 1] - be0;
+    bent = d.btab + d.b_ent + 4 * be0;
+    total = 0;
+    for (int k = 0; k < n_my; ++k) total += bent[4 * k + 1] + KR;
+  }
+  auto bsteps = [&](int k) { return bm ? __builtin_amdgcn_readfirstlane(bent[4 * k + 1]) : KT; };
   auto tile_of = [&](int k, int& pix_tile, int& ch_tile) {
+    if (bm) { pix_tile = 0; ch_tile = __builtin_amdgcn_readfirstlane(bent[4 * k + 2]) >> 16; return; }
     const int v = vtile >= 0 ? vtile : (int)blockIdx.x + k * (int)gridDim.x;
     const int nblk = d.n_tiles, bq = nblk >> 3, br = nblk & 7, xcd = v & 7, bidx = v >> 3;
     const int lid = (xcd < br ? xcd * (bq + 1) : br * (bq + 1) + (xcd - br) * bq) + bidx;
@@ -100,17 +111,15 @@
     long long mybase = 0;
     unsigned mymask = 0;
     int my_ch_tile = 0, my_pix_tile = 0;
-    auto prepare_tile = [&](int k) {
-      int pix_tile, ch_tile;
-      tile_of(k, pix_tile, ch_tile);
-      my_ch_tile = ch_tile;
-      my_pix_tile = pix_tile;
+    int ikt = 0, itile = 0;
+    int KTc = KT, KTTc = KTT, bkh0 = 0, bkh1 = 0, bkw0 = 0, bkw1 = 0, mym = -1;
+    int* lrow = reinterpret_cast<int*>(lbias + 2560);
+    auto decode_my = [&](long long m) {
       mybase = 0;
       mymask = 0;
       if (j < XR) {
-        const long long m = d.m0 + (long long)pix_tile * BPIX + r0 + 32 * j;
         int xn = 0, xd0 = -(1 << 20), xh0 = 0, xw0 = 0;
-        if (m < d.M) {
+        if (m >= 0 && m < d.M) {
           unsigned n, qd, qh, qw;
           decode_row(d, (unsigned)m, n, qd, qh, qw);
           xn = (int)n * d.Di;
@@ -121,19 +130,41 @@
         for (int kk = 0; kk < d.KD; ++kk) mymask |= (unsigned)((unsigned)(xd0 + kk * d.dild) < (unsigned)d.Di) << kk;
         for (int kk = 0; kk < d.KH; ++kk) mymask |= (unsigned)((unsigned)(xh0 + kk * d.dilh) < (unsigned)d.Hi) << (8 + kk);
         for (int kk = 0; kk < d.KW; ++kk) mymask |= (unsigned)((unsigned)(xw0 + kk * d.dilw) < (unsigned)d.Wi) << (16 + kk);
+        if (bm) mymask = m >= 0 ? 0x00ffffffu : 0u;
         const long long pix0 = ((long long)(xn + xd0) * d.Hi + xh0) * d.Wi + xw0;
         mybase = pix0 * d.Cin * (long long)sizeof(T);
       }
+    };
+    auto prepare_tile = [&](int k) {
+      int pix_tile, ch_tile;
+      tile_of(k, pix_tile, ch_tile);
+      my_ch_tile = ch_tile;
+      my_pix_tile = pix_tile;
+      if (bm) {
+        const int tr = __builtin_amdgcn_readfirstlane(bent[4 * k + 2]);
+        KTc = bsteps(k);
+        KTTc = KTc + KR;
+        bkh0 = tr & 15; bkh1 = (tr >> 4) & 15; bkw0 = (tr >> 8) & 15; bkw1 = (tr >> 12) & 15;
+        mym = j < XR ? d.btab[d.b_rows + __builtin_amdgcn_readfirstlane(bent[4 * k]) + r0 + 32 * j] : -1;
+        return;
+      }
+      decode_my(d.m0 + (long long)pix_tile * BPIX + r0 + 32 * j);
     };
     auto enter_tile = [&]() {
       const int grp = (tp & 63) & 56;
+      if (bm) {
+        decode_my(mym);
+        if (j < XR) lrow[(itile & 1) * 256 + r0 + 32 * j] = mym;
+        asm volatile("s_waitcnt lgkmcnt(0)" ::: "memory");
+      }
 #pragma unroll
       for (int i = 0; i < XR; ++i) {
         const long long b = __shfl(mybase, grp | i, 64);
         rmask[i] = (unsigned)__shfl((int)mymask, grp | i, 64);
         xoff[i] = (unsigned)(b + xbias + (long long)(js * E) * (long long)sizeof(T));
         if (KR) {
-          const long long m = d.m0 + (long long)my_pix_tile * BPIX + r0 + 32 * i;
+          long long m = d.m0 + (long long)my_pix_tile * BPIX + r0 + 32 * i;
+          if (bm) { m = __shfl(mym, grp | i, 64); if (m < 0) m = d.M; }
           roff[i] = m < d.M ? (unsigned)((m * d.ldo + my_ch_tile * BCH + js * E) * (long long)sizeof(T)) : 0xffffffffu;
         }
       }
@@ -144,6 +175,10 @@
       }
       tkd = tkh = tkw = tc = 0;
       wko = 0;
+      if (bm) {
+        tkh = bkh0; tkw = bkw0;
+        wko = (unsigned)((tkh * d.KW + tkw) * d.Cin) * (unsigned)sizeof(T);
+      }
       if (kt0 > 0) {
         if (d.korder && d.lcin >= 0) {
           const int tap = kt0 % d.ntaps, cb = kt0 / d.ntaps;
@@ -163,15 +198,14 @@
       }
     };
 
-    int ikt = 0, itile = 0;
     auto issue = [&](int stage) {
       if (ikt == 0) enter_tile();
       const unsigned sbase = lds0 + (unsigned)stage * (STAGE * 16);
       const unsigned sel = (1u << tkd) | (256u << tkh) | (65536u << tkw);
       const unsigned soff = (unsigned)(((long long)((tkd * d.dild * d.Hi + tkh * d.dilh) * d.Wi + tkw * d.dilw) * d.Cin + tc) * (long long)sizeof(T));
       const bool cok = tkd < d.KD && tc + js * E < d.Cin;
-      if (ikt >= KT) {
-        const unsigned ro = (unsigned)(ikt - KT) * (unsigned)(BK * sizeof(T));
+      if (ikt >= KTc) {
+        const unsigned ro = (unsigned)(ikt - KTc) * (unsigned)(BK * sizeof(T));
 #pragma unroll
         for (int i = 0; i < XR; ++i) blds16(roff[i], rsrc_r, ro, sbase + (BCH * 8 + i * 256) * 16);
         if (!BIG) {
@@ -187,7 +221,10 @@
 #pragma unroll
         for (int i = 0; i < WL; ++i) blds16(woff[i], rsrc_w, wko, sbase + (i * 256) * 16);
       }
-      if (ikt >= KT) {
+      if (ikt >= KTc) {
+      } else if (bm) {
+        if (++tkw == bkw1) { tkw = bkw0; if (++tkh == bkh1) { tkh = bkh0; tc += BK; } }
+        wko = (unsigned)((tkh * d.KW + tkw) * d.Cin + tc) * (unsigned)sizeof(T);
       } else if (d.korder && d.lcin >= 0) {
         wko += (unsigned)d.Cin * (unsigned)sizeof(T);
         if (++tkw == d.KW) { tkw = 0; if (++tkh == d.KH) { tkh = 0; if (++tkd == d.KD) { tkd = 0; tc += BK; wko = (unsigned)tc * (unsigned)sizeof(T); } } }
@@ -199,13 +236,14 @@
           if (++tkw == d.KW) { tkw = 0; if (++tkh == d.KH) { tkh = 0; ++tkd; } }
         }
       }
-      if (++ikt == KTT) { ikt = 0; ++itile; if (itile < n_my) prepare_tile(itile); }
+      if (++ikt == KTTc) { ikt = 0; ++itile; if (itile < n_my) prepare_tile(itile); }
     };
 
     if (total > 0) prepare_tile(0);
     if (total > 0) issue(0);
     if (NST == 3 && total > 1) issue(1);
-    int st = 0, gk = 0;
+    int st = 0, gk = 0, gtile = 0;
+    int gKTT = total > 0 ? bsteps(0) + KR : KTT;
     for (int g = 0; g < total; ++g) {
       if (NST == 2 || g + 1 >= total) asm volatile("s_waitcnt vmcnt(0)" ::: "memory");
       else asm volatile("s_waitcnt vmcnt(%0)" :: "n"(NP) : "memory");
@@ -213,7 +251,7 @@
       if (NST == 3) { if (g + 2 < total) issue(st == 0 ? 2 : st - 1); }
       else { if (g + 1 < total) issue(st ^ 1); }
       st = st == NST - 1 ? 0 : st + 1;
-      if (STAGED) { if (++gk == KTT) { gk = 0; RGBM_BARRIER(); } }
+      if (STAGED) { if (++gk == gKTT) { gk = 0; RGBM_BARRIER(); if (++gtile < n_my) gKTT = bsteps(gtile) + KR; } }
     }
     return;
   }
@@ -257,10 +295,12 @@
   T* __restrict__ out = reinterpret_cast<T*>(d.out);
   const T* __restrict__ res = reinterpret_cast<const T*>(d.res);
   auto tile_interior = [&](int pix_tile, int ch_tile) {
+    if (bm) return true;
     return (d.bias == nullptr || bias_lds) && d.m0 + (long long)(pix_tile + 1) * BPIX <= d.M && (ch_tile + 1) * BCH <= d.Cout && d.act != ACT_TANH;
   };
   int st = 0;
   for (int k = 0; k < n_my; ++k) {
+    const int KTk = BIG ? bsteps(k) : KT;
     {
       int pt, ct;
       tile_of(k, pt, ct);
@@ -296,7 +336,7 @@
         hi = make_uint4(c0.x, c0.y, c1.x, c1.y);
         lo = make_uint4(c0.z, c0.w, c1.z, c1.w);
       };
-      const int KTM = BIG ? KT : KTT;
+      const int KTM = BIG ? KTk : KTT;
       for (int kt = 0; kt < KTM; ++kt) {
         asm volatile("s_waitcnt lgkmcnt(0)" ::: "memory");
         RGBM_BARRIER();
@@ -388,7 +428,7 @@
 #pragma unroll
       for (int a = 0; a < FA; ++a) ldAs(st, 0, a);
       __builtin_amdgcn_sched_barrier(0);
-      for (int kt = 0; kt + 1 < KT; ++kt) {
+      for (int kt = 0; kt + 1 < KTk; ++kt) {
         first3();
         if (M32_SHIFT) {
           asm volatile("s_waitcnt lgkmcnt(0)" ::: "memory");
@@ -606,6 +646,17 @@
 #pragma unroll
               for (int q = 0; q < NQ; ++q)
                 *reinterpret_cast<uint4*>(stg + (wofs ^ (unsigned)((a * 2 * NQ + q) << 4))) = pk[a][q];
+            if (bm) {
+              const int* lrow = reinterpret_cast<const int*>(lbias + 2560) + (k & 1) * 256 + wpix + b * 32 + (lane >> 4);
+              char* oc = reinterpret_cast<char*>(out + ch0 + ar * AR * 32) + (lane & 15) * 16;
+#pragma unroll
+              for (int t = 0; t < 8; ++t) {
+                const int m = lrow[4 * t];
+                const uint4 v = *reinterpret_cast<const uint4*>(stg + t * 1024 + (rofs ^ (unsigned)(((4 * t) & 15) << 4)));
+                if (m >= 0) *reinterpret_cast<uint4*>(oc + (long long)m * d.ldo * (long long)sizeof(T)) = v;
+              }
+              return;
+            }
             char* ob = reinterpret_cast<char*>(out + (mrow + b * 32) * d.ldo + ch0 + ar * AR * 32);
 #pragma unroll
             for (int t = 0; t < 8; ++t) {
@@ -685,10 +736,13 @@
   }
 }
 
+static std::atomic<long long> g_border_launches{0};
+long long border_launch_count() { return g_border_launches.load(std::memory_order_relaxed); }
+
 template <typename T, int BPIX, int BCH = 256>
 static int launch_m32_range(ConvDesc d, hipStream_t s) {
   constexpr int NST = BPIX == 256 ? 2 : 3;
-  constexpr size_t LDS = ((size_t)NST * (BCH + BPIX) * 8) * sizeof(uint4) + 2560 * sizeof(float);
+  constexpr size_t LDS = ((size_t)NST * (BCH + BPIX) * 8) * sizeof(uint4) + 2560 * sizeof(float) + (BPIX == 256 && BCH == 256 ? 2 * 256 * sizeof(int) : 0);
   d.n_pix_tiles = (int)((d.M - d.m0 + BPIX - 1) / BPIX);
   d.n_ch_tiles = (d.Cout + BCH - 1) / BCH;
   const long long ntiles = (long long)d.n_pix_tiles * d.n_ch_tiles;
@@ -702,6 +756,8 @@
   if (int rc = persistent_grid_cus(&n_cu)) return rc;
   RGBM_REQUIRE(d.ksplit <= 1 || (BPIX == 128 && BCH <= 128 && ntiles * d.ksplit <= 4096 && d.kscratch && d.kcount), "K split: 64 / 128-channel x 128-pixel tiles, one workgroup per (tile, part)");
   const int grid = d.ksplit > 1 ? (int)(ntiles * d.ksplit) : ntiles < n_cu ? (int)ntiles : n_cu;
+  RGBM_REQUIRE(d.btab == nullptr || (BPIX == 256 && BCH == 256 && d.m0 == 0 && grid == d.b_nwg), "border-class table: made for another grid");
+  if (d.btab) g_border_launches.fetch_add(1, std::memory_order_relaxed);
   prof_begin_launch(s, BPIX == 256 && BCH == 256 ? (std::is_same<T, bx3_t>::value ? 33 : 31) : (std::is_same<T, bx3_t>::value ? 41 : 40), d.algo_flops, d.algo_bytes);
   hipLaunchKernelGGL((conv_igemm_m32_kernel<T, BPIX, BCH>), dim3((unsigned)grid), dim3(BPIX == 256 ? 768 : 512), LDS, s, d);
   prof_end_launch(s);
@@ -776,12 +832,14 @@
 template <typename T>
 static int launch_m32_small(ConvDesc d, const ConvPlan& p, hipStream_t s) {
   if (int rc = m32_setup<T>(d, p, s)) return rc;
+  d.btab = nullptr;
   return launch_m32_tiles128<T>(d, p.bch, s);
 }
 
 template <typename T>
 static int launch_m32(ConvDesc d, const ConvPlan& p, hipStream_t s) {
   if (int rc = m32_setup<T>(d, p, s)) return rc;
+  if (!p.border) d.btab = nullptr;
   if (p.main_rows > 0) {
     ConvDesc m = d;
     m.M = p.main_rows;
@@ -789,6 +847,7 @@
     m.algo_flops = d.algo_flops * frac; m.algo_bytes = d.algo_bytes * frac;
     if (int rc = launch_m32_range<T, 256, 256>(m, s)) return rc;
     d.m0 = m.M;
+    d.btab = nullptr;
     d.algo_flops *= 1.0 - frac; d.algo_bytes *= 1.0 - frac;
   }
   return p.tail_bch ? launch_m32_tiles128<T>(d, p.tail_bch, s) : 0;
diff --git a/rgbmanip_amd/csrc/conv_plan.cpp b/rgbmanip_amd/csrc/conv_plan.cpp
--- a/rgbmanip_amd/csrc/conv_plan.cpp
+++ b/rgbmanip_amd/csrc/conv_plan.cpp
@@ -1,4 +1,9 @@
 #include "conv_plan.h"
+
+#include <algorithm>
+#include <functional>
+#include <queue>
+#include <utility>
 
 #include "kernels.h"
 
@@ -55,6 +60,157 @@
   return n;
 }
 
+void tap_range(int q, int pad, int dil, int K, int n, int& k0, int& k1) {
+  k0 = K; k1 = 0;
+  for (int k = 0; k < K; ++k) {
+    const int x = q - pad + k * dil;
+    if (x >= 0 && x < n) { if (k < k0) k0 = k; k1 = k + 1; }
+  }
+  if (k0 > k1) k0 = k1 = 0;
+}
+
+struct AxisClasses {
+  std::vector<int> k0, k1, count, cls;
+};
+bool axis_classes(int nq, int pad, int dil, int K, int n, AxisClasses* a) {
+  a->cls.resize(nq);
+  for (int q = 0; q < nq; ++q) {
+    int k0, k1;
+    tap_range(q, pad, dil, K, n, k0, k1);
+    if (k1 == k0) return false;
+    for (int k = k0; k < k1; ++k) {
+      const int x = q - pad + k * dil;
+      if (x < 0 || x >= n) return false;
+    }
+    size_t c = 0;
+    while (c < a->k0.size() && !(a->k0[c] == k0 && a->k1[c] == k1)) ++c;
+    if (c == a->k0.size()) { a->k0.push_back(k0); a->k1.push_back(k1); a->count.push_back(0); }
+    a->count[c] += 1;
+    a->cls[q] = (int)c;
+  }
+  return true;
+}
+
+bool border_shape_ok(const ConvDesc& d, int dtype) {
+  return (dtype == BF16 || dtype == F16) && d.w_finite && d.KD == 1 && d.Di == 1 && d.Dq == 1 && d.pd == 0 && d.sd == 1 && d.sh == 1 && d.sw == 1 &&
+         d.KH * d.KW > 1 && d.KH <= 4 && d.KW <= 4 && d.lcin >= 0 && d.Cin % conv_bk(dtype) == 0 && d.Cout % 256 == 0 && d.ph >= 0 && d.pw >= 0 &&
+         d.dilh >= 1 && d.dilw >= 1 && d.N > 0 && d.M == (long long)d.N * d.Hq * d.Wq;
+}
+
+int popcount_int(int v) { int n = 0; for (; v; v &= v - 1) ++n; return n; }
+
+}
+
+static long long class_live_rows(const ConvDesc& d, const AxisClasses& ah, const AxisClasses& aw, long long main_rows, int i, int j) {
+  const long long hw = (long long)d.Hq * d.Wq, whole = main_rows / hw, rem = main_rows % hw;
+  const int hr = (int)(rem / d.Wq), wr = (int)(rem % d.Wq);
+  long long h_below = 0, w_below = 0;
+  for (int h = 0; h < hr; ++h) h_below += ah.cls[h] == i;
+  for (int w = 0; w < wr; ++w) w_below += aw.cls[w] == j;
+  return whole * ah.count[i] * aw.count[j] + h_below * aw.count[j] + (ah.cls[hr < d.Hq ? hr : 0] == i && hr < d.Hq ? w_below : 0);
+}
+
+bool border_applies(const ConvDesc& d, int dtype, int flags, long long main_rows) {
+  if ((flags & (DBG_NO_BORDER_TILES | DBG_KORDER_TAPS_OUTER)) || !border_shape_ok(d, dtype)) return false;
+  if (main_rows <= 0 || main_rows > d.M || main_rows % 256) return false;
+  AxisClasses ah, aw;
+  if (!axis_classes(d.Hq, d.ph, d.dilh, d.KH, d.Hi, &ah) || !axis_classes(d.Wq, d.pw, d.dilw, d.KW, d.Wi, &aw)) return false;
+  long long tiles = 0, taps = 0;
+  for (size_t i = 0; i < ah.k0.size(); ++i)
+    for (size_t j = 0; j < aw.k0.size(); ++j) {
+      const long long t = (class_live_rows(d, ah, aw, main_rows, (int)i, (int)j) + 255) / 256;
+      tiles += t;
+      taps += t * (ah.k1[i] - ah.k0[i]) * (aw.k1[j] - aw.k0[j]);
+    }
+  return taps < (main_rows / 256) * (long long)d.ntaps && tiles < (1ll << 20);
+}
+
+bool plan_border(const ConvDesc& d, int dtype, int flags, long long main_rows, int n_wg, BorderPlan* out) {
+  if (n_wg <= 0 || !border_applies(d, dtype, flags, main_rows)) return false;
+  AxisClasses ah, aw;
+  axis_classes(d.Hq, d.ph, d.dilh, d.KH, d.Hi, &ah);
+  axis_classes(d.Wq, d.pw, d.dilw, d.KW, d.Wi, &aw);
+  BorderPlan p;
+  p.n_wg = n_wg;
+  p.n_ch = d.Cout / 256;
+  p.steps_per_tap = d.Cin / conv_bk(dtype);
+  const bool dense_out = d.osd == 1 && d.osh == 1 && d.osw == 1 && d.opd == 0 && d.oph == 0 && d.opw == 0 && d.Dq == d.Do && d.Hq == d.Ho && d.Wq == d.Wo;
+  p.kr = (dense_out && d.res_mode == RES_PRE_ACT && d.res != nullptr) ? 256 / conv_bk(dtype) : 0;
+  const int nw = (int)aw.k0.size();
+  std::vector<int> of_class(ah.k0.size() * nw, -1);
+  for (int h = 0; h < d.Hq; ++h)
+    for (int w = 0; w < d.Wq; ++w) {
+      int& c = of_class[ah.cls[h] * nw + aw.cls[w]];
+      if (c < 0) {
+        c = (int)p.classes.size();
+        BorderClass bc = {};
+        bc.kh0 = ah.k0[ah.cls[h]]; bc.kh1 = ah.k1[ah.cls[h]]; bc.kw0 = aw.k0[aw.cls[w]]; bc.kw1 = aw.k1[aw.cls[w]];
+        for (int kh = bc.kh0; kh < bc.kh1; ++kh)
+          for (int kw = bc.kw0; kw < bc.kw1; ++kw) bc.mask |= 1 << (kh * d.KW + kw);
+        bc.n_pix = ah.count[ah.cls[h]] * aw.count[aw.cls[w]];
+        p.classes.push_back(bc);
+      }
+    }
+  int pix0 = 0;
+  for (BorderClass& bc : p.classes) { bc.pix0 = pix0; pix0 += bc.n_pix; }
+  p.pix.assign((size_t)d.Hq * d.Wq, 0);
+  {
+    std::vector<int> fill(p.classes.size(), 0);
+    for (int h = 0; h < d.Hq; ++h)
+      for (int w = 0; w < d.Wq; ++w) {
+        const int c = of_class[ah.cls[h] * nw + aw.cls[w]];
+        p.pix[p.classes[c].pix0 + fill[c]++] = h * d.Wq + w;
+      }
+  }
+  const long long hw = (long long)d.Hq * d.Wq;
+  p.total_steps = 0;
+  for (size_t c = 0; c < p.classes.size(); ++c) {
+    BorderClass& bc = p.classes[c];
+    bc.row0 = (long long)p.rows.size();
+    for (long long v = 0; v * hw < main_rows; ++v)
+      for (int i = 0; i < bc.n_pix; ++i) {
+        const long long m = v * hw + p.pix[bc.pix0 + i];
+        if (m < main_rows) p.rows.push_back((int)m);
+      }
+    const long long live = (long long)p.rows.size() - bc.row0;
+    p.rows.resize((size_t)(bc.row0 + (live + 255) / 256 * 256), -1);
+    if (p.rows.size() >= (1u << 30)) return false;
+    const int steps = popcount_int(bc.mask) * p.steps_per_tap + p.kr;
+    for (long long t = 0; t < (live + 255) / 256; ++t)
+      for (int ch = 0; ch < p.n_ch; ++ch) {
+        p.tiles.push_back(BorderTile{(int)c, ch, bc.mask, steps, bc.row0 + t * 256});
+        p.total_steps += steps;
+      }
+  }
+  p.parent_steps = (main_rows / 256) * p.n_ch * (long long)(d.ntaps * p.steps_per_tap + p.kr);
+  std::vector<int> by_steps(p.tiles.size());
+  for (size_t i = 0; i < by_steps.size(); ++i) by_steps[i] = (int)i;
+  auto mid_view = [&](int i) { const BorderClass& bc = p.classes[p.tiles[i].cls]; return (double)(p.tiles[i].row0 - bc.row0 + 128) / bc.n_pix; };
+  std::stable_sort(by_steps.begin(), by_steps.end(), [&](int a, int b) { return mid_view(a) < mid_view(b); });
+  if ((int)by_steps.size() > n_wg)
+    std::stable_sort(by_steps.end() - n_wg, by_steps.end(), [&](int a, int b) { return p.tiles[a].steps > p.tiles[b].steps; });
+  typedef std::pair<long long, std::pair<int, int>> Load;
+  std::priority_queue<Load, std::vector<Load>, std::greater<Load>> q;
+  const int per_xcd = (n_wg + 7) / 8;
+  for (int b = 0; b < n_wg; ++b) q.push(Load(0, std::make_pair((b & 7) * per_xcd + (b >> 3), b)));
+  std::vector<std::vector<int>> mine(n_wg);
+  for (int i : by_steps) {
+    Load l = q.top();
+    q.pop();
+    mine[l.second.second].push_back(i);
+    l.first += p.tiles[i].steps;
+    q.push(l);
+  }
+  p.max_wg_steps = 0;
+  p.wg_off.assign(1, 0);
+  for (int b = 0; b < n_wg; ++b) {
+    long long s = 0;
+    for (int i : mine[b]) { p.order.push_back(i); s += p.tiles[i].steps; }
+    p.wg_off.push_back((int)p.order.size());
+    if (s > p.max_wg_steps) p.max_wg_steps = s;
+  }
+  *out = std::move(p);
+  return true;
 }
 
 int plan_conv(const ConvDesc& d, int dtype, const ConvTuning& t, ConvPlan* out) {
@@ -127,6 +283,7 @@
       }
       p.main_rows = Pm * 256;
       p.identity_residual = ident_ok;
+      p.border = p.main_rows > 0 && p.korder == 1 && uni && border_applies(d, dtype, f, p.main_rows);
       p.tail_bch = p.main_rows == d.M ? 0 : 256;
       const long long pt = (d.M - p.main_rows + 127) / 128;
       if (p.tail_bch && t.gemm_kernel != 1 && !(f & DBG_M32_TAILS_R5)) {
diff --git a/rgbmanip_amd/csrc/conv_plan.h b/rgbmanip_amd/csrc/conv_plan.h
--- a/rgbmanip_amd/csrc/conv_plan.h
+++ b/rgbmanip_amd/csrc/conv_plan.h
@@ -1,4 +1,6 @@
 #pragma once
+#include <vector>
+
 #include "common.h"
 
 namespace rgbm {
@@ -31,7 +33,34 @@
   int ksplit;
   bool identity_residual;
   int korder, buf_ok;
+  bool border;
 };
+
+struct BorderClass {
+  int kh0, kh1, kw0, kw1;
+  int mask;
+  int n_pix;
+  int pix0;
+  long long row0;
+};
+struct BorderTile {
+  int cls, ch;
+  int mask;
+  int steps;
+  long long row0;
+};
+struct BorderPlan {
+  int n_wg, n_ch, kr, steps_per_tap;
+  std::vector<BorderClass> classes;
+  std::vector<int> pix;
+  std::vector<BorderTile> tiles;
+  std::vector<int> order;
+  std::vector<int> wg_off;
+  std::vector<int> rows;
+  long long total_steps, parent_steps, max_wg_steps;
+};
+bool border_applies(const ConvDesc& d, int dtype, int flags, long long main_rows);
+bool plan_border(const ConvDesc& d, int dtype, int flags, long long main_rows, int n_wg, BorderPlan* out);
 
 constexpr size_t kM32SplitFloats = 8u << 20, kM32SplitCounters = 16384;
 
diff --git a/rgbmanip_amd/csrc/kernels.h b/rgbmanip_amd/csrc/kernels.h
--- a/rgbmanip_amd/csrc/kernels.h
+++ b/rgbmanip_amd/csrc/kernels.h
@@ -135,9 +135,10 @@
   DBG_PSP_STAGE_R5 = 1024, DBG_POINT_MLP_R5 = 2048, DBG_TILE_CONV0 = 4096, DBG_NO_KSPLIT = 16384, DBG_L2_SLIM_TILE = 32768,
   DBG_WS_128x256 = 65536, DBG_NO_SLIM64 = 262144, DBG_KORDER_TAPS_OUTER = 1 << 20, DBG_SWEEP_ALT_BLEND = 1 << 21, DBG_SWEEP_DOT2 = 1 << 22,
   DBG_PP_ONE_KERNEL = 1 << 23, DBG_NO_SLIM_SMALL = 1 << 24, DBG_PP_GENERIC_SELECT = 1 << 25, DBG_PP_GUARD = 1 << 26, DBG_GLOBAL_ADDR = 1 << 27,
-  DBG_SWEEP_PER_TILE = 1 << 28, DBG_SPARSE_TAIL_R5 = 1 << 29, DBG_M32_TAILS_R5 = 1 << 30, DBG_POSE_MLP_R6 = 1 << 19,
+  DBG_SWEEP_PER_TILE = 1 << 28, DBG_SPARSE_TAIL_R5 = 1 << 29, DBG_M32_TAILS_R5 = 1 << 30, DBG_POSE_MLP_R6 = 1 << 19, DBG_NO_BORDER_TILES = 32,
 };
 extern int g_debug_flags;
+long long border_launch_count();
 extern long long g_ws_min_rows;
 extern int g_tuning_version;
 extern int g_gemm_kernel;
diff --git a/rgbmanip_amd/csrc/layers.cpp b/rgbmanip_amd/csrc/layers.cpp
--- a/rgbmanip_amd/csrc/layers.cpp
+++ b/rgbmanip_amd/csrc/layers.cpp
@@ -1,8 +1,10 @@
 #include "layers.h"
+#include "conv_plan.h"
 #include "kernels.h"
 
 #include <string.h>
 
+#include <array>
 #include <map>
 #include <mutex>
 #include <utility>
@@ -124,6 +126,12 @@
   return 0;
 }
 
+struct BorderTables {
+  struct Entry { DevBuf buf; int n_wg = 0, b_ent = 0, b_rows = 0; };
+  std::mutex mu;
+  std::map<std::array<long long, 7>, Entry> per_shape;
+};
+
 int ConvLayer::init(int dtype_, const ConvGeom& g_, const float* w, const float* bias_h, const float* bn_scale,
                     const float* bn_shift, int Cin_pad_, int Cout_pad_) {
   g = g_;
@@ -161,6 +169,10 @@
         for (int t = 0; t < pc.ntaps; ++t)
           packed[(size_t)o * pc.Kpad + (size_t)t * Cin_pad + c] = w[((long long)o * g.Cin + c) * kvol + t] * sc;
     }
+    w_finite = true;
+    for (float v : packed)
+      if (!((v < 0.f ? -v : v) <= 3.3895313892515355e38f)) { w_finite = false; break; }
+    border = std::make_shared<BorderTables>();
     return finish(pc, packed);
   }
 
@@ -232,10 +244,51 @@
   d.bias_stride = bias_override ? bias_stride : 0;
   d.res_mode = res ? res_mode : RES_NONE;
   d.out_f32 = (out_plain_f32 && dtype == BF16X3) ? 1 : 0;
+  d.w_finite = w_finite ? 1 : 0;
   d.algo_flops = 2.0 * (double)d.M * g.Cout * (double)pc.ntaps * g.Cin;
   d.algo_bytes = ((double)d.M * g.Cout + (cls == 0 ? (double)N * Di * Hi * Wi * g.Cin : 0.0) +
                   (res ? (double)d.M * g.Cout : 0.0)) * (double)dtype_size(dtype) +
                  (double)g.Cout * pc.ntaps * g.Cin * (double)dtype_size(dtype);
+  return 0;
+}
+
+int ConvLayer::attach_border(ConvDesc& d, hipStream_t s) const {
+  if (!border || !w_finite || g.transposed || dtype == F32 || g.KH * g.KW == 1) return 0;
+  ConvTuning t;
+  ConvPlan p;
+  if (int rc = conv_tuning(0, &t)) return rc;
+  if (int rc = plan_conv(d, dtype, t, &p)) return rc;
+  if (p.kernel != CONV_M32 || !p.border) return 0;
+  int dev = 0;
+  RGBM_CHECK_HIP(hipGetDevice(&dev));
+  const std::array<long long, 7> key = {dev, d.N, d.Hi, d.Wi, t.n_cu, p.identity_residual ? 1 : 0, p.main_rows};
+  std::lock_guard<std::mutex> lock(border->mu);
+  auto it = border->per_shape.find(key);
+  if (it == border->per_shape.end()) {
+    hipStreamCaptureStatus cs = hipStreamCaptureStatusNone;
+    if (hipStreamIsCapturing(s, &cs) == hipSuccess && cs != hipStreamCaptureStatusNone) return 0;
+    BorderPlan bp;
+    if (!plan_border(d, dtype, t.flags, p.main_rows, t.n_cu, &bp)) return 0;
+    std::vector<int> tab(bp.wg_off);
+    BorderTables::Entry e;
+    e.n_wg = bp.n_wg;
+    e.b_ent = (int)tab.size();
+    for (int i : bp.order) {
+      const BorderTile& bt = bp.tiles[i];
+      const BorderClass& bc = bp.classes[bt.cls];
+      tab.push_back((int)bt.row0);
+      tab.push_back(bt.steps - bp.kr);
+      tab.push_back(bc.kh0 | bc.kh1 << 4 | bc.kw0 << 8 | bc.kw1 << 12 | bt.ch << 16);
+      tab.push_back(0);
+    }
+    e.b_rows = (int)tab.size();
+    tab.insert(tab.end(), bp.rows.begin(), bp.rows.end());
+    RGBM_CHECK_HIP(hipMalloc(e.buf.out(), tab.size() * sizeof(int)));
+    RGBM_CHECK_HIP(hipMemcpy(e.buf.get(), tab.data(), tab.size() * sizeof(int), hipMemcpyHostToDevice));
+    it = border->per_shape.emplace(key, std::move(e)).first;
+  }
+  d.btab = it->second.buf.get<int>();
+  d.b_nwg = it->second.n_wg; d.b_ent = it->second.b_ent; d.b_rows = it->second.b_rows;
   return 0;
 }
 
@@ -245,6 +298,7 @@
   for (int cls = 0; cls < nclass; ++cls) {
     ConvDesc d;
     if (int rc = build_desc(d, in, out, N, Di, Hi, Wi, ldo, res, res_mode, bias_override, bias_stride, cls, out_plain_f32)) return rc;
+    if (int rc = attach_border(d, s)) return rc;
     if (int rc = launch_conv(d, dtype, s)) return rc;
   }
   return 0;
diff --git a/rgbmanip_amd/csrc/layers.h b/rgbmanip_amd/csrc/layers.h
--- a/rgbmanip_amd/csrc/layers.h
+++ b/rgbmanip_amd/csrc/layers.h
@@ -1,5 +1,6 @@
 #pragma once
 #include <map>
+#include <memory>
 #include <string>
 #include <vector>
 
@@ -58,6 +59,8 @@
 void conv_desc_geom(ConvDesc& d, const ConvGeom& g, const PackedConv& pc, int Cin_pad, int Cout_pad, int N, int Di, int Hi, int Wi,
                     int ldo, int cls);
 
+struct BorderTables;
+
 struct ConvLayer {
   ConvGeom g;
   int dtype = F32;
@@ -65,6 +68,8 @@
   int Cout_pad = 0;
   DevBuf bias;
   std::vector<PackedConv> packs;
+  bool w_finite = false;
+  std::shared_ptr<BorderTables> border;
 
   int init(int dtype, const ConvGeom& g, const float* w, const float* bias, const float* bn_scale, const float* bn_shift,
            int Cin_pad, int Cout_pad);
@@ -76,6 +81,7 @@
                    bool allow_fuse, bool* fused, hipStream_t s, bool out2_plain_f32 = false) const;
   int build_desc(ConvDesc& d, const void* in, void* out, int N, int Di, int Hi, int Wi, int ldo, const void* res, int res_mode,
                  const float* bias_override, int bias_stride, int cls, bool out_plain_f32 = false) const;
+  int attach_border(ConvDesc& d, hipStream_t s) const;
 };
 
 struct UpConvLayer {
```

New measurement: 5937, median of 6. 1.7% higher.
